# sair-lab/AirSLAM

Measured on AMD Instinct MI355X. Metric: stereo detect+match pairs/sec (2x PLNet @512x512 internal: points + lines, junctions on the left + LightGlue match), higher is better.
Workload: dtype fp16

## Files before the change

### airslam_amd/_lib.py

```python
from __future__ import annotations

import ctypes as C
import os

_HERE = os.path.dirname(os.path.abspath(__file__))
LIB_PATH = os.path.join(_HERE, "libairfe.so")


class Tuning(C.Structure):
    _fields_ = [(n, C.c_int) for n in (
        "fuse_lg_block", "gemm_small_max_m", "gemm8_min_m", "gemmr_min_m", "gemmr_wgs", "qkv_pair", "block_min_m", "lgb_tokens", "sg_kenc_gemm",
        "fold_qkv", "overlap_lines", "kf_graph", "kf_spec_rows", "fuse_dec", "assign_fused", "fold_out_proj", "desc_gather_stream", "copy_wgs")] + [("reserved", C.c_int * 5)]


class Cfg(C.Structure):
    _fields_ = [
        ("device", C.c_int), ("precision", C.c_int), ("max_batch", C.c_int), ("enc_chunk", C.c_int),
        ("max_keypoints", C.c_int), ("keypoint_threshold", C.c_float), ("remove_borders", C.c_int),
        ("nms_radius", C.c_int), ("line_threshold", C.c_float), ("line_length_threshold", C.c_float),
        ("matcher", C.c_int), ("image_width", C.c_int), ("image_height", C.c_int), ("sinkhorn_iters", C.c_int),
        ("superpoint_pack", C.c_char_p), ("plnet_s1_pack", C.c_char_p), ("lightglue_pack", C.c_char_p),
        ("superglue_pack", C.c_char_p), ("matcher_precision", C.c_int), ("line_precision", C.c_int), ("check_launches", C.c_int),
        ("tuning", C.POINTER(Tuning)),
    ]


class Stage0(C.Structure):
    _fields_ = [(n, C.c_void_p) for n in (
        "juncs_pred", "lines_pred", "iskeep", "idx_junc_to_end_min", "idx_junc_to_end_max",
        "loi_features", "loi_features_thin", "loi_features_aux")]


class BowdbFilter(C.Structure):
    _fields_ = [("ratio", C.c_float), ("min_words", C.c_int), ("d_max_index", C.c_void_p), ("d_exclude", C.c_void_p), ("exclude_words", C.c_int)]


class RelocCfg(C.Structure):
    _fields_ = [("ratio", C.c_float), ("min_words", C.c_int), ("K", C.c_int), ("outlier_rejection", C.c_int), ("min_inlier", C.c_int),
                ("pose_refinement", C.c_int), ("cam", C.c_double * 5), ("thr", C.c_double * 2)]


class LoopCfg(C.Structure):
    _fields_ = [("ratio", C.c_float), ("min_words", C.c_int), ("K", C.c_int), ("outlier_rejection", C.c_int), ("distance_rate", C.c_double),
                ("min_matches", C.c_int), ("min_points", C.c_int), ("min_inliers", C.c_int), ("cam", C.c_double * 5), ("thr", C.c_double * 2)]


class SeqPolicy(C.Structure):
    _fields_ = [("min_init_stereo_feature", C.c_int), ("min_num_match", C.c_int), ("max_num_match", C.c_int), ("tracking_point_rate", C.c_float),
                ("tracking_parallax_rate", C.c_float), ("min_x_diff", C.c_double), ("max_x_diff", C.c_double), ("max_y_diff", C.c_double),
                ("image_width", C.c_int), ("image_height", C.c_int)]


class SeqFrame(C.Structure):
    _fields_ = ([(n, C.c_int) for n in ("frame_type", "candidate", "promoted", "dropped", "enough_match", "good_stereo_point", "n_left", "n_right", "n_lines_left",
                                        "n_lines_right", "n_junctions", "n_stereo", "n_matches")] + [("_pad", C.c_int)]
                + [(n, C.c_void_p) for n in ("features_left", "features_right", "lines_left", "lines_right", "junctions", "stereo_idx", "stereo_score", "matches_idx",
                                             "matches_score")])


class DebugLinearArgs(C.Structure):
    _fields_ = ([(n, C.c_int) for n in ("prec", "M", "K", "K1", "N")] + [(n, C.c_void_p) for n in ("x1", "x2", "w", "b")]
                + [("epi", C.c_int), ("act", C.c_int), ("rowidx", C.c_void_p), ("src_rows", C.c_int), ("rot_cos", C.c_void_p), ("rot_sin", C.c_void_p),
                   ("Np", C.c_int), ("H", C.c_int), ("x32", C.c_void_p), ("d2s_hc", C.c_int), ("d2s_wc", C.c_int), ("flag", C.c_void_p),
                   ("kernel", C.c_int), ("gr_wgs", C.c_int), ("out", C.c_void_p), ("out2", C.c_void_p)])


class DebugLgBlockArgs(C.Structure):
    _fields_ = ([("prec", C.c_int), ("M", C.c_int)] + [(n, C.c_void_p) for n in ("attn", "x32", "xb", "wo", "bo", "w1", "b1", "gamma", "beta", "w2", "b2")]
                + [(n, C.c_int) for n in ("relu", "tokens_per_wg", "mixed", "nqk_n")]
                + [(n, C.c_void_p) for n in ("nqk_w", "nqk_b", "nv_w", "nv_b", "rot_cos", "rot_sin")]
                + [("Np", C.c_int)] + [(n, C.c_void_p) for n in ("q", "k", "vt")] + [("rows_past", C.c_int * 5)])


class DebugConvArgs(C.Structure):
    _fields_ = ([(n, C.c_void_p) for n in ("x", "img", "w1a", "b1a", "w", "b")] + [(n, C.c_int) for n in ("cin", "cout", "B", "H", "W", "pool", "out_pad", "relu", "wgs")]
                + [("y_words", C.c_size_t), ("y_raw", C.c_void_p)])


class DebugLgPrepareArgs(C.Structure):
    _fields_ = ([(n, C.c_int) for n in ("prec", "B", "cap", "ld", "kp_off", "normalize")] + [(n, C.c_float) for n in ("cx", "cy", "linv")]
                + [(n, C.c_void_p) for n in ("f0", "f1", "n0", "n1", "wr", "f0x", "f1x")] + [(n, C.c_int) for n in ("n0x", "n1x", "slack_rows", "rows")]
                + [(n, C.c_void_p) for n in ("x32", "xb", "rot_cos", "rot_sin", "lens")] + [("rows_past", C.c_int)])


class DebugLgAssignArgs(C.Structure):
    _fields_ = ([(n, C.c_int) for n in ("prec", "B", "n")] + [(n, C.c_void_p) for n in ("md", "x32", "w")] + [("b", C.c_float), ("lens", C.c_void_p), ("cap", C.c_int),
                ("thr", C.c_float), ("form", C.c_int)]
                + [(n, C.c_void_p) for n in ("pad", "z", "sim", "scores", "rowlse", "collse", "rowval", "rowarg", "colarg", "idx", "score", "nmatch")])


class DebugAttentionArgs(C.Structure):
    _fields_ = ([(n, C.c_int) for n in ("prec", "S", "H", "n", "cross")] + [(n, C.c_void_p) for n in ("q", "k", "v", "lens")]
                + [("canary", C.c_int), ("raw", C.c_int), ("out", C.c_void_p), ("Np", C.c_int), ("rows_past", C.c_int)])


class DebugDetectorTailArgs(C.Structure):
    _fields_ = ([(n, C.c_int) for n in ("B", "Bs", "h", "w", "cap")] + [(n, C.c_void_p) for n in ("heat", "act", "feat", "feat1", "n", "n1", "nms_map", "keep", "cand_cnt")]
                + [("nms_map_written", C.c_int)])


class DebugLinePostArgs(C.Structure):
    _fields_ = ([(n, C.c_int) for n in ("B", "nj", "ld", "h", "w", "capL", "capJ", "from_plane")]
                + [(n, C.c_void_p) for n in ("la", "sc", "m2", "heat", "lines", "nlines", "nfound", "junc", "njunc", "jfound", "jmap")])


class DebugJunctionTailArgs(C.Structure):
    _fields_ = ([(n, C.c_int) for n in ("B", "nj", "ld", "h", "w", "capL", "capJ")]
                + [(n, C.c_void_p) for n in ("la", "sc", "m2", "heat", "act", "lines", "nlines", "nfound", "junc", "njunc", "jfound")] + [("fused", C.c_int)])


class DebugLineMidArgs(C.Structure):
    _fields_ = ([(n, C.c_int) for n in ("B", "j2l", "s1_form", "wgs")]
                + [(n, C.c_void_p) for n in ("juncs_pred", "lines_pred", "thin", "aux", "loi", "iskeep_in", "idx_min_in", "idx_max_in", "iskeep", "idx_min", "idx_max", "counts",
                                             "keep", "pairs", "rep", "head4", "prop4", "ridx", "proj", "lines_adjusted", "scores_line", "table_dirty")])


class DebugS0DecodeArgs(C.Structure):
    _fields_ = ([(n, C.c_int) for n in ("B", "mode", "ld", "off", "want_ta8", "want_loi", "want_jnms", "prec", "wgs")] + [(n, C.c_void_p) for n in ("rows", "x", "w", "b")]
                + [("stage_floats", C.c_size_t)] + [(n, C.c_void_p) for n in ("stage", "jloc", "joff", "jnms", "ta8", "loi", "head_rows")])


SIGNATURES = {
    "airfe_copy_rows_dev": (C.c_int, [C.c_void_p, C.c_int, C.c_void_p, C.c_void_p, C.c_void_p, C.c_void_p, C.c_void_p, C.c_void_p]),
    "airfe_pack_rows_dev": (C.c_int, [C.c_void_p, C.c_int, C.c_void_p, C.c_void_p, C.c_void_p, C.c_void_p, C.c_void_p, C.c_void_p, C.c_void_p]),
    "airfe_seq_default_policy": (None, [C.POINTER(SeqPolicy)]),
    "airfe_seq_add_keyframe_check": (C.c_int, [C.POINTER(SeqPolicy), C.c_void_p, C.c_int, C.c_void_p, C.c_int, C.c_void_p, C.c_int]),
    "airfe_seq_good_stereo_points": (C.c_int, [C.POINTER(SeqPolicy), C.c_void_p, C.c_void_p, C.c_void_p, C.c_int]),
    "airfe_seq_create": (C.c_int, [C.c_void_p, C.c_void_p, C.c_int, C.POINTER(SeqPolicy), C.c_int, C.c_int, C.c_void_p, C.c_void_p, C.c_void_p, C.POINTER(C.c_void_p)]),
    "airfe_seq_destroy": (None, [C.c_void_p]),
    "airfe_seq_last_error": (C.c_char_p, [C.c_void_p]),
    "airfe_seq_begin": (C.c_int, [C.c_void_p, C.c_void_p, C.c_void_p, C.c_int, C.c_int, C.c_int, C.c_size_t]),
    "airfe_seq_end": (C.c_int, [C.c_void_p, C.POINTER(SeqFrame)]),
    "airfe_seq_step": (C.c_int, [C.c_void_p, C.c_void_p, C.c_void_p, C.c_int, C.c_int, C.c_int, C.c_size_t, C.POINTER(SeqFrame)]),
    "airfe_seq_stream": (C.c_void_p, [C.c_void_p]),
    "airfe_seq_set_outlier_rejection": (C.c_int, [C.c_void_p, C.c_int]),
    "airfe_seq_wall_split": (C.c_int, [C.c_void_p, C.POINTER(C.c_double), C.POINTER(C.c_double), C.POINTER(C.c_double), C.POINTER(C.c_int), C.POINTER(C.c_int)]),
    "airfe_default_cfg": (None, [C.POINTER(Cfg)]),
    "airfe_default_tuning": (None, [C.POINTER(Tuning)]),
    "airfe_debug_fail_next_launch": (C.c_int, [C.c_void_p, C.c_int]),
    "airfe_create": (C.c_int, [C.POINTER(Cfg), C.POINTER(C.c_void_p)]),
    "airfe_destroy": (None, [C.c_void_p]),
    "airfe_last_error": (C.c_char_p, [C.c_void_p]),
    "airfe_detect_points": (C.c_int, [C.c_void_p, C.c_void_p, C.c_int, C.c_int, C.c_int, C.c_void_p, C.c_int,
                                      C.POINTER(C.c_int)]),
    "airfe_has_line_branch": (C.c_int, [C.c_void_p]),
    "airfe_detect_plnet": (C.c_int, [C.c_void_p, C.c_void_p, C.c_int, C.c_int, C.c_int, C.POINTER(Stage0), C.c_void_p,
                                     C.c_int, C.POINTER(C.c_int), C.c_void_p, C.c_int, C.POINTER(C.c_int), C.c_void_p,
                                     C.c_int, C.POINTER(C.c_int), C.c_int]),
    "airfe_stereo_keyframe": (C.c_int, [C.c_void_p, C.c_void_p, C.c_void_p, C.c_int, C.c_int, C.c_int, C.c_void_p, C.c_void_p, C.c_int,
                                        C.POINTER(C.c_int), C.POINTER(C.c_int), C.c_void_p, C.c_void_p, C.c_int, C.POINTER(C.c_int),
                                        C.POINTER(C.c_int), C.c_void_p, C.c_int, C.POINTER(C.c_int), C.c_void_p, C.c_void_p, C.c_int,
                                        C.POINTER(C.c_int)]),
    "airfe_stereo_keyframe_tracked": (C.c_int, [C.c_void_p, C.c_void_p, C.c_void_p, C.c_int, C.c_int, C.c_int, C.c_void_p, C.c_void_p, C.c_int,
                                                C.POINTER(C.c_int), C.POINTER(C.c_int), C.c_void_p, C.c_void_p, C.c_int, C.POINTER(C.c_int),
                                                C.POINTER(C.c_int), C.c_void_p, C.c_int, C.POINTER(C.c_int), C.c_void_p, C.c_void_p, C.c_int,
                                                C.POINTER(C.c_int), C.c_void_p, C.c_int, C.c_void_p, C.c_void_p, C.POINTER(C.c_int)]),
    "airfe_track_frame": (C.c_int, [C.c_void_p, C.c_void_p, C.c_int, C.c_int, C.c_int, C.c_void_p, C.c_int, C.c_void_p, C.c_int, C.POINTER(C.c_int),
                                    C.c_void_p, C.c_void_p, C.c_int, C.POINTER(C.c_int)]),
    "airfe_promote_frame": (C.c_int, [C.c_void_p, C.c_void_p, C.c_int, C.c_int, C.c_int, C.c_void_p, C.c_int, C.POINTER(C.c_int), C.c_void_p, C.c_void_p, C.c_int,
# ... 60 lines not shown
    "airfe_bowdb_add_junction_frames_batch_dev": (C.c_int, [C.c_void_p, C.c_void_p, C.c_void_p, C.c_int, C.c_void_p, C.c_void_p] + [C.c_int] * 4 + [C.c_void_p]),
    "airfe_bowdb_query_stored_batch_dev": (C.c_int, [C.c_void_p, C.c_void_p, C.c_int, C.c_float, C.c_int, C.c_int] + [C.c_void_p] * 3 + [C.c_int] +
                                           [C.c_void_p] * 4),
    "airfe_loop_detect_batch_dev": (C.c_int, [C.c_void_p, C.c_void_p, C.POINTER(LoopCfg), C.c_void_p, C.c_int] + [C.c_void_p] * 10 + [C.c_int] +
                                    [C.c_void_p] * 3),
    "airfe_set_rectify_maps": (C.c_int, [C.c_void_p, C.c_int, C.c_void_p, C.c_void_p, C.c_int, C.c_int]),
    "airfe_rectify_detect_points": (C.c_int, [C.c_void_p, C.c_int, C.c_void_p, C.c_int, C.c_int, C.c_int, C.c_void_p, C.c_void_p, C.c_int,
                                              C.POINTER(C.c_int)]),
    "airfe_rectify_batch_dev": (C.c_int, [C.c_void_p, C.c_int, C.c_void_p, C.c_int, C.c_int, C.c_int, C.c_int, C.c_size_t, C.c_void_p,
                                          C.c_int, C.c_size_t, C.c_void_p]),
    "airfe_detect_points_batch_dev": (C.c_int, [C.c_void_p, C.c_void_p, C.c_int, C.c_int, C.c_int, C.c_int, C.c_size_t,
                                                C.c_void_p, C.c_int, C.c_void_p, C.c_void_p]),
    "airfe_match_lightglue_batch_dev": (C.c_int, [C.c_void_p, C.c_void_p, C.c_void_p, C.c_void_p, C.c_void_p, C.c_int,
                                                  C.c_int, C.c_void_p, C.c_void_p, C.c_int, C.c_void_p, C.c_void_p]),
    "airfe_match_superglue_batch_dev": (C.c_int, [C.c_void_p, C.c_void_p, C.c_void_p, C.c_void_p, C.c_void_p, C.c_int, C.c_int,
                                                  C.c_void_p, C.c_void_p, C.c_void_p, C.c_void_p, C.c_void_p]),
    "airfe_stereo_batch_dev": (C.c_int, [C.c_void_p, C.c_void_p, C.c_void_p, C.c_int, C.c_int, C.c_int, C.c_int,
                                         C.c_size_t, C.c_void_p, C.c_void_p, C.c_int, C.c_void_p, C.c_void_p, C.c_void_p,
                                         C.c_void_p, C.c_int, C.c_void_p, C.c_void_p]),
    "airfe_detect_plnet_batch_dev": (C.c_int, [C.c_void_p, C.c_void_p, C.c_int, C.c_int, C.c_int, C.c_int, C.c_size_t, C.c_void_p,
                                               C.c_int, C.c_void_p, C.c_void_p, C.c_int, C.c_void_p, C.c_void_p, C.c_int, C.c_void_p,
                                               C.c_int, C.c_void_p, C.c_void_p]),
    "airfe_stereo_plnet_batch_dev": (C.c_int, [C.c_void_p, C.c_void_p, C.c_void_p, C.c_int, C.c_int, C.c_int, C.c_int, C.c_size_t,
                                               C.c_void_p, C.c_void_p, C.c_int, C.c_void_p, C.c_void_p, C.c_void_p, C.c_int, C.c_void_p,
                                               C.c_void_p, C.c_int, C.c_void_p, C.c_void_p, C.c_void_p, C.c_void_p, C.c_int, C.c_void_p,
                                               C.c_void_p]),
    "airfe_debug_plnet_j2l": (C.c_int, [C.c_void_p, C.c_int, C.c_void_p, C.c_void_p, C.c_void_p]),
    "airfe_assign_points_to_lines_batch_dev": (C.c_int, [C.c_void_p, C.c_void_p, C.c_void_p, C.c_int, C.c_void_p, C.c_void_p, C.c_int, C.c_int,
                                                         C.c_void_p, C.c_void_p, C.c_void_p, C.c_int, C.c_void_p, C.c_void_p]),
    "airfe_match_lines_batch_dev": (C.c_int, [C.c_void_p] + [C.c_void_p] * 8 + [C.c_int, C.c_int, C.c_void_p, C.c_void_p, C.c_int, C.c_int,
                                              C.c_void_p, C.c_void_p, C.c_void_p, C.c_int, C.c_void_p, C.c_void_p]),
    "airfe_fundamental_ransac": (C.c_int, [C.c_void_p, C.c_void_p, C.c_int, C.c_void_p, C.c_int, C.c_void_p, C.c_void_p, C.c_int, C.POINTER(C.c_int)]),
    "airfe_fundamental_ransac_batch_dev": (C.c_int, [C.c_void_p, C.c_void_p, C.c_void_p, C.c_void_p, C.c_void_p, C.c_int, C.c_int, C.c_void_p, C.c_void_p,
                                                     C.c_int, C.c_void_p, C.c_void_p, C.c_void_p]),
    "airfe_set_outlier_rejection": (C.c_int, [C.c_void_p, C.c_int]),
    "airfe_pnp_ransac": (C.c_int, [C.c_void_p, C.c_void_p, C.c_void_p, C.c_int, C.c_void_p, C.c_void_p, C.c_void_p, C.c_void_p, C.POINTER(C.c_int)]),
    "airfe_pnp_ransac_batch_dev": (C.c_int, [C.c_void_p, C.c_void_p, C.c_void_p, C.c_void_p, C.c_int, C.c_int, C.c_void_p, C.c_void_p, C.c_void_p,
                                             C.c_void_p, C.c_void_p, C.c_void_p]),
    "airfe_stereo_points": (C.c_int, [C.c_void_p, C.c_void_p, C.c_void_p, C.c_int, C.c_void_p, C.c_int, C.c_void_p, C.c_int, C.c_void_p, C.c_void_p,
                                      C.c_void_p, C.POINTER(C.c_int)]),
    "airfe_stereo_points_batch_dev": (C.c_int, [C.c_void_p] * 6 + [C.c_int, C.c_int, C.c_void_p, C.c_void_p, C.c_int] + [C.c_void_p] * 5),
    "airfe_stereo_lines": (C.c_int, [C.c_void_p, C.c_void_p, C.c_void_p, C.c_int, C.c_void_p, C.c_int] + [C.c_void_p] * 8),
    "airfe_stereo_lines_batch_dev": (C.c_int, [C.c_void_p] * 6 + [C.c_int, C.c_void_p, C.c_void_p, C.c_int] + [C.c_void_p] * 7),
    "airfe_stereo_line_landmarks_batch_dev": (C.c_int, [C.c_void_p] * 6 + [C.c_int] + [C.c_void_p] * 4 + [C.c_int, C.c_void_p, C.c_void_p, C.c_int,
                                                        C.c_void_p, C.c_int] + [C.c_void_p] * 8 + [C.c_int] + [C.c_void_p] * 8),
    "airfe_track_pose_batch_dev": (C.c_int, [C.c_void_p, C.c_void_p, C.c_void_p, C.c_int, C.c_void_p, C.c_int, C.c_void_p, C.c_void_p, C.c_int, C.c_int,
                                             C.c_void_p, C.c_void_p, C.c_void_p, C.c_void_p, C.c_void_p]),
    "airfe_frame_optimize": (C.c_int, [C.c_void_p, C.c_void_p, C.c_void_p, C.c_int] + [C.c_void_p] * 7 + [C.POINTER(C.c_int)]),
    "airfe_frame_optimize_batch_dev": (C.c_int, [C.c_void_p, C.c_void_p, C.c_void_p, C.c_void_p, C.c_int, C.c_int] + [C.c_void_p] * 9),
    "airfe_track_pose_opt_batch_dev": (C.c_int, [C.c_void_p, C.c_void_p, C.c_void_p, C.c_int, C.c_void_p, C.c_int, C.c_void_p, C.c_int, C.c_void_p,
                                                 C.c_void_p, C.c_int, C.c_int] + [C.c_void_p] * 9),
    "airfe_sync": (C.c_int, [C.c_void_p]),
    "airfe_superglue_status": (C.c_int, [C.c_void_p, C.c_void_p]),
    "airfe_profile_enable": (C.c_int, [C.c_void_p, C.c_int]),
    "airfe_profile_stages": (C.c_int, []),
    "airfe_profile_stage_name": (C.c_char_p, [C.c_int]),
    "airfe_profile_read": (C.c_int, [C.c_void_p, C.c_void_p, C.c_void_p, C.c_void_p, C.c_void_p]),
    "airfe_debug_detector_maps": (C.c_int, [C.c_void_p, C.c_int, C.c_void_p, C.c_void_p, C.c_void_p]),
    "airfe_debug_lightglue_scores": (C.c_int, [C.c_void_p, C.c_void_p, C.c_int, C.c_void_p, C.c_int, C.c_void_p]),
    "airfe_debug_superglue_scores": (C.c_int, [C.c_void_p, C.c_void_p, C.c_int, C.c_void_p, C.c_int, C.c_void_p]),
    "airfe_debug_lg_filter": (C.c_int, [C.c_void_p, C.c_void_p, C.c_int, C.c_int, C.c_void_p, C.c_void_p, C.c_int, C.POINTER(C.c_int)]),
    "airfe_debug_sg_decode": (C.c_int, [C.c_void_p, C.c_void_p, C.c_int, C.c_int, C.c_void_p, C.c_void_p, C.c_void_p, C.c_void_p]),
    "airfe_debug_sg_sinkhorn": (C.c_int, [C.c_void_p, C.c_void_p, C.c_void_p, C.c_int, C.c_int, C.c_float, C.c_int, C.c_int, C.c_void_p, C.POINTER(C.c_int)]),
    "airfe_debug_detector_tail": (C.c_int, [C.c_void_p, C.POINTER(DebugDetectorTailArgs)]),
    "airfe_debug_line_post": (C.c_int, [C.c_void_p, C.POINTER(DebugLinePostArgs)]),
    "airfe_debug_junction_tail": (C.c_int, [C.c_void_p, C.POINTER(DebugJunctionTailArgs)]),
    "airfe_debug_junctions_topk": (C.c_int, [C.c_void_p, C.c_void_p, C.c_void_p, C.c_int, C.c_void_p]),
    "airfe_debug_line_mid": (C.c_int, [C.c_void_p, C.POINTER(DebugLineMidArgs)]),
    "airfe_debug_s0_decode": (C.c_int, [C.c_void_p, C.POINTER(DebugS0DecodeArgs)]),
    "airfe_debug_lg_prepare": (C.c_int, [C.c_void_p, C.POINTER(DebugLgPrepareArgs)]),
    "airfe_debug_lg_assign": (C.c_int, [C.c_void_p, C.POINTER(DebugLgAssignArgs)]),
    "airfe_debug_plnet_stage0": (C.c_int, [C.c_void_p] + [C.c_void_p] * 10),
    "airfe_debug_plnet_s1": (C.c_int, [C.c_void_p, C.POINTER(Stage0), C.c_void_p, C.c_void_p, C.c_int, C.POINTER(C.c_int)]),
    "airfe_debug_plnet_s1_last": (C.c_int, [C.c_void_p, C.c_void_p, C.c_void_p, C.c_int, C.POINTER(C.c_int)]),
    "airfe_debug_preprocess": (C.c_int, [C.c_void_p, C.c_void_p, C.c_int, C.c_int, C.c_int, C.c_void_p]),
    "airfe_debug_conv3x3": (C.c_int, [C.c_void_p, C.c_void_p, C.c_int, C.c_int, C.c_int, C.c_int, C.c_void_p, C.c_void_p,
                                      C.c_int, C.c_int, C.c_void_p]),
    "airfe_debug_conv": (C.c_int, [C.c_void_p, C.POINTER(DebugConvArgs)]),
    "airfe_debug_trace": (C.c_int, [C.c_void_p, C.c_int]),
    "airfe_debug_trace_stop": (C.c_int, [C.c_void_p, C.c_int]),
    "airfe_debug_trace_buffer": (C.c_int, [C.c_void_p, C.c_int, C.c_void_p, C.c_size_t]),
    "airfe_debug_trace_slots": (C.c_int, [C.c_void_p]),
    "airfe_debug_conv_order": (C.c_int, [C.c_int, C.POINTER(C.c_int)]),
    "airfe_debug_trace_slot": (C.c_int, [C.c_void_p, C.c_int, C.c_char_p, C.c_int, C.POINTER(C.c_uint), C.POINTER(C.c_uint), C.POINTER(C.c_uint)]),
    "airfe_debug_trace_read": (C.c_int, [C.c_void_p, C.c_void_p, C.c_void_p, C.c_void_p]),
    "airfe_debug_gemm": (C.c_int, [C.c_void_p, C.c_void_p, C.c_int, C.c_int, C.c_void_p, C.c_void_p, C.c_int, C.c_int,
                                   C.c_void_p]),
    "airfe_debug_linear": (C.c_int, [C.c_void_p, C.POINTER(DebugLinearArgs)]),
    "airfe_debug_qkv": (C.c_int, [C.c_void_p] + [C.c_int] * 3 + [C.c_void_p] * 3 + [C.c_int] + [C.c_void_p] * 4 + [C.c_int] * 2 + [C.c_void_p] * 3),
    "airfe_debug_lg_block": (C.c_int, [C.c_void_p, C.POINTER(DebugLgBlockArgs)]),
    "airfe_debug_ln_gelu": (C.c_int, [C.c_void_p, C.c_int, C.c_void_p, C.c_void_p, C.c_void_p, C.c_int]),
    "airfe_debug_attention_args": (C.c_int, [C.c_void_p, C.POINTER(DebugAttentionArgs)]),
    "airfe_debug_attention": (C.c_int, [C.c_void_p, C.c_void_p, C.c_void_p, C.c_void_p, C.c_void_p, C.c_int, C.c_int, C.c_int, C.c_int, C.c_void_p]),
}

_lib = None


def lib() -> C.CDLL:
    global _lib
    if _lib is None:
        if not os.path.exists(LIB_PATH):
            raise RuntimeError(
                f"{LIB_PATH} is missing: build it with `python -m airslam_amd.build` "
                "(hipcc, gfx950).  airslam_amd has no CPU fallback.")
        try:
            import torch
        except Exception:
            pass
        l = C.CDLL(LIB_PATH)
        for name, (res, args) in SIGNATURES.items():
            fn = getattr(l, name)
            fn.restype = res
            fn.argtypes = args
        _lib = l
    return _lib
```

### airslam_amd/api.py

```python
from __future__ import annotations

import ctypes as C
import os
import tempfile
from typing import Dict, Optional

import numpy as np

from . import _lib, weights as W

FEAT = 259


def _pack_arg(x, tmpfiles) -> Optional[bytes]:
    if x is None:
        return None
    if isinstance(x, (str, bytes, os.PathLike)):
        return os.fsencode(x)
    f = tempfile.NamedTemporaryFile(suffix=".airfe", delete=False)
    f.close()
    W.save_pack(f.name, x)
    tmpfiles.append(f.name)
    return f.name.encode()


class AirfeError(RuntimeError):
    pass


def conv_tile_order(order: int) -> int:
    prev = C.c_int()
    if _lib.lib().airfe_debug_conv_order(int(order), C.byref(prev)) != 0:
        raise AirfeError((_lib.lib().airfe_last_error(None) or b"airfe_debug_conv_order failed").decode())
    return prev.value


class Context:

    def __init__(self, superpoint=None, lightglue=None, superglue=None, plnet_s1=None, tuning=None, **cfg):
        self._l = _lib.lib()
        c = _lib.Cfg()
        self._l.airfe_default_cfg(C.byref(c))
        t = None
        if tuning and "conv_order" in tuning:
            tuning = dict(tuning)
            conv_tile_order(int(tuning.pop("conv_order")))
        if tuning:
            t = _lib.Tuning()
            self._l.airfe_default_tuning(C.byref(t))
            for k, v in tuning.items():
                if k == "reserved" or not hasattr(t, k):
                    raise TypeError(f"unknown airfe_tuning field {k!r}")
                setattr(t, k, int(v))
            c.tuning = C.pointer(t)
        for k, v in cfg.items():
            if not hasattr(c, k):
                raise TypeError(f"unknown airfe_cfg field {k!r}")
            setattr(c, k, v)
        tmp = []
        try:
            c.superpoint_pack = _pack_arg(superpoint, tmp)
            c.lightglue_pack = _pack_arg(lightglue, tmp)
            c.superglue_pack = _pack_arg(superglue, tmp)
            c.plnet_s1_pack = _pack_arg(plnet_s1, tmp)
            h = C.c_void_p()
            rc = self._l.airfe_create(C.byref(c), C.byref(h))
            if rc != 0:
                raise AirfeError((self._l.airfe_last_error(None) or b"airfe_create failed").decode())
        finally:
            for t in tmp:
                os.unlink(t)
        self._h = h
        c.tuning = None
        self.cfg = c
        self.max_keypoints = c.max_keypoints
        self.np_rows = (c.max_keypoints + 15) // 16 * 16

    def close(self):
        if getattr(self, "_h", None):
            self._l.airfe_destroy(self._h)
            self._h = None

    def __del__(self):
        try:
            self.close()
        except Exception:
            pass

    def _chk(self, rc, what):
        if rc != 0:
            raise AirfeError(f"{what}: {(self._l.airfe_last_error(self._h) or b'').decode()}")

    @staticmethod
    def _image(img, wrong_type=None):
        img = np.asarray(img)
        if img.ndim != 2 or img.dtype != np.uint8:
            raise wrong_type if wrong_type is not None else AirfeError("empty image")
        if img.size == 0:
            raise AirfeError("empty image")
        if img.strides[1] != 1 or img.strides[0] < img.shape[1]:
            img = np.ascontiguousarray(img)
        return img

    def detect_points(self, gray: np.ndarray) -> np.ndarray:
        gray = self._image(gray, TypeError("expected a 2-D uint8 image"))
        cap = self.np_rows
        feat = np.empty((cap, FEAT), dtype=np.float32)
        n = C.c_int(0)
        self._chk(self._l.airfe_detect_points(self._h, gray.ctypes.data, gray.shape[0], gray.shape[1], gray.strides[0],
                                              feat.ctypes.data, cap, C.byref(n)), "airfe_detect_points")
        return feat[:n.value].copy()

    def bow_load(self, voc: dict):
        d = np.ascontiguousarray(voc["desc"], np.float32); fc = np.ascontiguousarray(voc["first_child"], np.int32)
        nc = np.ascontiguousarray(voc["n_children"], np.int32); wi = np.ascontiguousarray(voc["word_id"], np.int32)
        w = np.ascontiguousarray(voc["weight"], np.float64)
        self._chk(self._l.airfe_bow_load(self._h, d.ctypes.data, fc.ctypes.data, nc.ctypes.data, wi.ctypes.data, w.ctypes.data, d.shape[0]),
                  "airfe_bow_load")

    def bow_transform(self, feat_rows: np.ndarray):
        f = np.ascontiguousarray(feat_rows, np.float32).reshape(-1, FEAT)
        wid = np.empty((f.shape[0],), np.uint32); w = np.empty((f.shape[0],), np.float64)
        self._chk(self._l.airfe_bow_transform(self._h, f.ctypes.data, f.shape[0], wid.ctypes.data, w.ctypes.data), "airfe_bow_transform")
        return wid, w

    def set_rectify_maps(self, side: int, mapx: np.ndarray, mapy: np.ndarray):
        mx = np.ascontiguousarray(mapx, np.float32); my = np.ascontiguousarray(mapy, np.float32)
        if mx.shape != my.shape or mx.ndim != 2:
            raise TypeError("maps must be two 2-D arrays of one shape")
# ... 355 lines not shown
        for name, x in zip(("iskeep_in", "idx_min_in", "idx_max_in"), ins):
            if x is not None:
                assert x.shape == (b, n)
                setattr(a, name, x.ctypes.data)
        self._chk(self._l.airfe_debug_line_mid(self._h, C.byref(a)), "airfe_debug_line_mid")
        return out

    S0_STAGE = {"lines_pred": (600, 3 * 16384 * 4), "thin": (600 + 7 * 3 * 16384, 4 * 16384), "aux": (600 + 7 * 3 * 16384 + 4 * 16384, 4 * 16384)}
    S0_STAGE_FLOATS = (600 + 7 * 3 * 16384 + 8 * 16384 + 63) // 64 * 64

    def debug_s0_decode(self, rows=None, ld=160, off=128, ta8=True, loi=False, jnms=True, x=None, w=None, b=None, prec=1, wgs=0, two_pass=False):
        f = lambda t: np.ascontiguousarray(t, np.float32)
        npx, sf = 128 * 128, self.S0_STAGE_FLOATS
        a = _lib.DebugS0DecodeArgs(want_ta8=int(bool(ta8)), want_loi=int(bool(loi)), want_jnms=int(bool(jnms)), prec=int(prec), wgs=int(wgs), stage_floats=sf)
        if rows is not None:
            assert x is None and not two_pass
            rows = f(rows)
            bb = rows.shape[0]
            assert rows.shape == (bb, npx, ld)
            a.mode, a.ld, a.off, a.rows = 0, int(ld), int(off), rows.ctypes.data
        else:
            x, w, b = f(x), f(w), f(b)
            bb = x.shape[0] // npx
            assert x.shape == (bb * npx, 128) and w.shape == (17, 128) and b.shape == (17,)
            a.mode, a.x, a.w, a.b = (2 if two_pass else 1), x.ctypes.data, w.ctypes.data, b.ctypes.data
        poison = lambda *shape: np.full(shape, -1, np.int32).view(np.float32)
        out = {"stage": poison(bb, sf), "jloc": poison(bb, 128, 128), "joff": poison(bb, 2, 128, 128), "jnms": poison(bb, 128, 128), "ta8": poison(bb, npx, 8),
               "loi": poison(128, 128, 128)}
        if two_pass:
            out["head_rows"] = poison(bb, npx, 32)
        a.B = bb
        for k, v in out.items():
            setattr(a, k, v.ctypes.data)
        self._chk(self._l.airfe_debug_s0_decode(self._h, C.byref(a)), "airfe_debug_s0_decode")
        for k, (o, n) in self.S0_STAGE.items():
            v = out["stage"][:, o:o + n]
            out[k] = v.reshape(bb, 3 * npx, 4) if k == "lines_pred" else v.reshape(bb, 4, 128, 128)
        return out

    def debug_junctions_topk(self, jloc, joff):
        jloc, joff = np.ascontiguousarray(jloc, np.float32), np.ascontiguousarray(joff, np.float32)
        b = jloc.shape[0]
        assert jloc.shape == (b, 128, 128) and joff.shape == (b, 2, 128, 128)
        out = np.full((b, 300, 2), np.nan, np.float32)
        self._chk(self._l.airfe_debug_junctions_topk(self._h, jloc.ctypes.data, joff.ctypes.data, b, out.ctypes.data), "airfe_debug_junctions_topk")
        return out

    def debug_preprocess(self, gray):
        gray = np.ascontiguousarray(gray, np.uint8)
        out = np.empty((512, 512), np.float32)
        self._chk(self._l.airfe_debug_preprocess(self._h, gray.ctypes.data, gray.shape[0], gray.shape[1], gray.strides[0],
                                                 out.ctypes.data), "airfe_debug_preprocess")
        return out

    def debug_conv3x3(self, x, w, b, pool=False):
        x = np.ascontiguousarray(x, np.float32); w = np.ascontiguousarray(w, np.float32); b = np.ascontiguousarray(b, np.float32)
        bb, cin, hh, ww = x.shape
        cout = w.shape[0]
        ho, wo = (hh // 2, ww // 2) if pool else (hh, ww)
        y = np.empty((bb, cout, ho, wo), np.float32)
        self._chk(self._l.airfe_debug_conv3x3(self._h, x.ctypes.data, bb, cin, hh, ww, w.ctypes.data, b.ctypes.data, cout,
                                              int(pool), y.ctypes.data), "airfe_debug_conv3x3")
        return y

    def debug_conv(self, w, b, prec, x=None, img=None, w1a=None, b1a=None, pool=False, out_pad=1, relu=True, wgs=256):
        f32 = lambda t: None if t is None else np.ascontiguousarray(t, np.float32)
        x, img, w1a, b1a, w, b = map(f32, (x, img, w1a, b1a, w, b))
        src = x if x is not None else img
        bb, hh, ww = src.shape[0], src.shape[-2], src.shape[-1]
        cout, cin = w.shape[0], w.shape[1]
        p = int(out_pad)
        ho, wo = (hh // 2, ww // 2) if pool else (hh, ww)
        guard = (wo + 2 * p) * cout
        words = bb * (ho + 2 * p) * guard
        raw = np.zeros(words + 2 * guard, np.uint16)
        ptr = lambda t: None if t is None else t.ctypes.data
        a = _lib.DebugConvArgs(x=ptr(x), img=ptr(img), w1a=ptr(w1a), b1a=ptr(b1a), w=ptr(w), b=ptr(b), cin=cin, cout=cout, B=bb, H=hh, W=ww, pool=int(pool), out_pad=p,
                               relu=int(relu), wgs=int(wgs), y_words=raw.size, y_raw=ptr(raw))
        self._chk(self._l.airfe_debug_conv(self._h, C.byref(a)), "airfe_debug_conv")
        buf = raw[guard:guard + words].reshape(bb, ho + 2 * p, wo + 2 * p, cout)
        inner = np.ascontiguousarray(buf[:, p:p + ho, p:p + wo, :])
        y = inner.view(np.float16).astype(np.float32) if prec == 1 else (inner.astype(np.uint32) << 16).view(np.float32)
        return {"raw": buf, "guard_lo": raw[:guard], "guard_hi": raw[guard + words:], "y": np.ascontiguousarray(y.transpose(0, 3, 1, 2))}

    def debug_gemm(self, x, w, b, relu=False):
        x = np.ascontiguousarray(x, np.float32); w = np.ascontiguousarray(w, np.float32); b = np.ascontiguousarray(b, np.float32)
        m, k = x.shape
        n = w.shape[0]
        y = np.empty((m, n), np.float32)
        self._chk(self._l.airfe_debug_gemm(self._h, x.ctypes.data, m, k, w.ctypes.data, b.ctypes.data, n, int(relu),
                                           y.ctypes.data), "airfe_debug_gemm")
        return y

    DEBUG_KERNELS = {"dispatch": 0, "small": 1, "tiled": 2, "gemm8": 3, "gemmr": 4, "gemmr_gather": 5, "gemmr_gather128": 6}

    def debug_linear(self, x1, w, b, prec, epi=0, act=0, x2=None, rowidx=None, rot=None, Np=0, x32=None, d2s=None, kernel="dispatch", gr_wgs=0):
        f32 = lambda t: None if t is None else np.ascontiguousarray(t, np.float32)
        x1, w, b, x2, x32 = f32(x1), f32(w), f32(b), f32(x2), (None if x32 is None else np.array(x32, np.float32, copy=True))
        n, k = w.shape
        m = len(rowidx) if rowidx is not None else x1.shape[0]
        a = _lib.DebugLinearArgs(prec=prec, M=m, K=k, K1=x1.shape[1], N=n, x1=x1.ctypes.data, w=w.ctypes.data, b=b.ctypes.data, epi=epi, act=act, Np=Np, H=4,
                                 kernel=self.DEBUG_KERNELS[kernel], gr_wgs=gr_wgs)
        keep = []
        if x2 is not None:
            a.x2 = x2.ctypes.data
        if rowidx is not None:
            ri = np.ascontiguousarray(rowidx, np.int32)
            keep.append(ri)
            a.rowidx, a.src_rows = ri.ctypes.data, x1.shape[0]
        if rot is not None:
            rc, rs = f32(rot[0]), f32(rot[1])
            keep += [rc, rs]
            a.rot_cos, a.rot_sin = rc.ctypes.data, rs.ctypes.data
        if x32 is not None:
            a.x32 = x32.ctypes.data
        flag = np.zeros(1, np.int32)
        out2 = None
        if epi == 5:
            hc, wc = d2s
            a.d2s_hc, a.d2s_wc, a.flag = hc, wc, flag.ctypes.data
            out = np.empty((m // (hc * wc), 8 * hc, 8 * wc), np.float32)
        elif epi in (3, 4):
            s = m // Np
            out = np.empty((s, 4, Np, 64) if epi == 3 else (s, 4, 64, Np), np.float32)
            if epi == 3 and n == 512:
                out2 = np.empty_like(out)
                a.out2 = out2.ctypes.data
        else:
            out = np.empty((m, n), np.float32)
        a.out = out.ctypes.data
        self._chk(self._l.airfe_debug_linear(self._h, C.byref(a)), "airfe_debug_linear")
        if epi == 5:
            return out, int(flag[0])
        if epi == 2:
            return out, x32
        return (out, out2) if out2 is not None else out

    def debug_qkv(self, x, wqk, bqk, wv, bv, prec, Np, rot=None, pair=True, gr_wgs=0):
        f32 = lambda t: np.ascontiguousarray(t, np.float32)
        x, wqk, bqk, wv, bv = f32(x), f32(wqk), f32(bqk), f32(wv), f32(bv)
        m, nqk, s = x.shape[0], wqk.shape[0], x.shape[0] // Np
        q = np.empty((s, 4, Np, 64), np.float32)
        k = np.empty_like(q) if nqk == 512 else None
        vt = np.empty((s, 4, 64, Np), np.float32)
        rc, rs = (f32(rot[0]), f32(rot[1])) if rot is not None else (None, None)
        ptr = lambda t: None if t is None else t.ctypes.data
        self._chk(self._l.airfe_debug_qkv(self._h, prec, m, Np, ptr(x), ptr(wqk), ptr(bqk), nqk, ptr(wv), ptr(bv), ptr(rc), ptr(rs), int(pair), gr_wgs, ptr(q),
                                          ptr(k), ptr(vt)), "airfe_debug_qkv")
        return q, k, vt

    def debug_lg_block(self, attn, x32, w1, b1, w2, b2, prec, gamma=None, beta=None, wo=None, bo=None, relu=False, tokens_per_wg=128, mixed=False,
                       nqk=None, nv=None, rot=None, Np=0):
        f32 = lambda t: None if t is None else np.ascontiguousarray(t, np.float32)
        m = attn.shape[0]
        attn, w1, b1, w2, b2, gamma, beta, wo, bo = map(f32, (attn, w1, b1, w2, b2, gamma, beta, wo, bo))
        x32 = np.array(x32, np.float32, copy=True)
        xb = np.empty_like(x32)
        ptr = lambda t: None if t is None else t.ctypes.data
        a = _lib.DebugLgBlockArgs(prec=prec, M=m, attn=ptr(attn), x32=ptr(x32), xb=ptr(xb), wo=ptr(wo), bo=ptr(bo), w1=ptr(w1), b1=ptr(b1), gamma=ptr(gamma),
                                  beta=ptr(beta), w2=ptr(w2), b2=ptr(b2), relu=int(relu), tokens_per_wg=tokens_per_wg, mixed=int(mixed), Np=Np)
        q = k = vt = None
        keep = []
        if nqk is not None:
            (qw, qb), (vw, vb) = map(lambda p: (f32(p[0]), f32(p[1])), (nqk, nv))
            keep += [qw, qb, vw, vb]
            s = m // Np
# ... 707 lines not shown
```

### airslam_amd/csrc/airfe_debug.hip

```cpp
#include "airfe_host.h"

#include <memory>

struct HookStage {
  enum { OWN_TEXT = 1, SATURATION = 2, DEVICE_WIDE = 4 };
  HookStage(airfe_ctx* c_, const std::string& who_, int pack_prec = 0) : c(c_), who(who_), st(c_->stream) { mem.pack_prec = pack_prec; }
  HookStage(const HookStage&) = delete;
  ~HookStage() {
    if (queued) (void)hipStreamSynchronize(st);
    for (void* p : mem.allocs) (void)hipFree(p);
  }
  int status() const { return rc; }
  hipStream_t stream() { queued = true; return st; }
  int refuse(const std::string& m) { return rc ? rc : rc = fail(c, who + ": " + m); }
  void step(int r) { queued = true; if (r) rc = 1; }
  template <class T> T* fresh(size_t n, int byte) {
    T* p = raw<T>(n);
    fill(p, byte, std::max<size_t>(n, 1) * sizeof(T));
    return p;
  }
  template <class T> T* up(std::vector<T> v) { T* p = raw<T>(v.size()); put(p, std::move(v)); return p; }
  template <class T> T* up(const T* src, size_t n) { return up(std::vector<T>(src, src + n)); }
  bool linear(const float* W, const float* b, int K, int N, LinW& out) { if (!rc && !make_linear(&mem, W, b, K, N, out)) refuse("allocation failed"); return !rc; }
  void fill(void* p, int byte, size_t bytes) { if (!rc && bytes) hip(hipMemsetAsync(p, byte, bytes, stream()), "hipMemsetAsync"); }
// ... 110 lines not shown
  s.wait();
  const std::vector<uint16_t> yo = s.get<uint16_t>(a.Y, ywords);
  for (int bb = 0; bb < B; ++bb)
    for (int co = 0; co < cout; ++co)
      for (int yy = 0; yy < Ho; ++yy)
        for (int xx = 0; xx < Wo; ++xx)
          y[(((size_t)bb * cout + co) * Ho + yy) * Wo + xx] = back2(yo[(((size_t)bb * (Ho + 2) + yy + 1) * (Wo + 2) + xx + 1) * cout + co], prec);
  return s.status();
} AIRFE_CATCH(c)

int airfe_debug_fail_next_launch(airfe_ctx* c, int stage) try {
  AIRFE_ENTER(c);
  if (stage < -1 || stage >= ST_COUNT) return fail(c, "debug_fail_next_launch: no such stage");
  c->fail_stage = stage;
  return 0;
} AIRFE_CATCH(c)

int airfe_debug_gemm(airfe_ctx* c, const float* x, int M, int K, const float* w, const float* b, int N, int relu, float* y) try {
  AIRFE_ENTER(c);
  if (K != 128 && K != 256 && K != 512) return fail(c, "debug_gemm: K must be 128, 256 or 512");
  const int prec = c->prec, Mp = (M + 127) / 128 * 128, Np8 = (N + 7) / 8 * 8;
  HookStage s(c, "debug_gemm", prec);
  LinW lw;
  s.linear(w, b, K, N, lw);
  GemmArgs g;
  g.X1 = s.up(dbg_rows2(x, M, K, Mp, prec)); g.ld1 = K; g.K1 = K; g.Wp = lw.w; g.bias = lw.b; g.M = Mp; g.N = N; g.cb_total = lw.cbt;
  g.epi = EPI_STORE_F32; g.act = relu ? ACT_RELU : ACT_NONE; g.out = s.fresh<float>((size_t)Mp * Np8, 0); g.ldo = Np8;
  dbg_gemm_dispatch(c, g, 0);
  if (s.status()) return 1;
  launch_gemm(prec, K, false, g, s.stream());
  s.wait(HookStage::OWN_TEXT);
  const std::vector<float> yo = s.get<float>(g.out, (size_t)Mp * Np8);
  for (int m = 0; m < M; ++m)
    for (int n = 0; n < N; ++n) y[(size_t)m * N + n] = yo[(size_t)m * Np8 + n];
  return s.status();
} AIRFE_CATCH(c)

int airfe_debug_conv(airfe_ctx* c, airfe_debug_conv_args* a) try {
  AIRFE_ENTER(c);
  if (!a || !a->w || !a->b || !a->y_raw) return fail(c, "debug_conv: null argument");
  const bool fused = a->img != nullptr;
  if (fused == (a->x != nullptr)) return fail(c, "debug_conv: exactly one of x (plain form) and img (fused conv1a -> conv1b) must be given");
  const int cin = a->cin, cout = a->cout, B = a->B, H = a->H, W = a->W, pool = a->pool, opad = a->out_pad, prec = c->prec;
  if (prec != 0 && prec != 1) return fail(c, "debug_conv: the context's precision must be fp16 or bf16");
  if (a->wgs < 1 || a->wgs > 256) return fail(c, "debug_conv: wgs must lie in 1 .. 256");
  if (cin != 64 && cin != 128) return fail(c, "debug_conv: cin must be 64 or 128");
  if (cout < 64 || cout % 64 || (cin == 128 && cout % 128)) return fail(c, "debug_conv: cout must be a multiple of 64 (of 128 when cin is 128)");
  if (B < 1 || H < 16 || W < 16 || H % 16 || W % 16) return fail(c, "debug_conv: B >= 1, H and W multiples of 16");
  if ((pool != 0 && pool != 1) || (opad != 0 && opad != 1) || (a->relu != 0 && a->relu != 1)) return fail(c, "debug_conv: pool, out_pad and relu are 0 or 1");
  if (pool && !opad) return fail(c, "debug_conv: a pooled layer always feeds another conv (out_pad = 1); pool with out_pad = 0 is no form of the arena");
  if (fused && (cin != 64 || cout != 64 || !pool || !opad || !a->relu || !a->w1a || !a->b1a))
    return fail(c, "debug_conv: the fused form is conv1a -> conv1b: cin = cout = 64, pool = 1, out_pad = 1, relu = 1, w1a and b1a given");
  const int Ho = pool ? H / 2 : H, Wo = pool ? W / 2 : W;
  const size_t guard = (size_t)(Wo + 2 * opad) * cout, words = (size_t)B * (Ho + 2 * opad) * guard, total = words + 2 * guard;
  if (a->y_words != total) return fail(c, "debug_conv: y_words must be (B (Ho + 2 out_pad) + 2) (Wo + 2 out_pad) cout");
  HookStage s(c, "debug_conv");
  ConvArgs g;
  if (fused) {
    std::vector<float> im((size_t)B * (H + 2) * (W + 2), 0.f);
    for (int bb = 0; bb < B; ++bb)
      for (int yy = 0; yy < H; ++yy) memcpy(&im[((size_t)bb * (H + 2) + yy + 1) * (W + 2) + 1], a->img + ((size_t)bb * H + yy) * W, (size_t)W * sizeof(float));
    g.img = s.up(std::move(im));
    g.w1a = s.up(a->w1a, (size_t)64 * 9);
    g.b1a = s.up(a->b1a, (size_t)64);
  } else {
    g.X = s.up(dbg_conv_x(a->x, B, cin, H, W, prec));
  }
  g.Wp = s.up(dbg_conv_slabs(a->w, cin, cout, prec));
  g.bias = s.up(a->b, (size_t)cout);
  uint16_t* dy = s.fresh<uint16_t>(total, 0xFF);
  if (s.status()) return 1;
  g.Y = dy + guard;
  g.B = B; g.H = H; g.W = W; g.CIN = cin; g.COUT = cout; g.pool = pool; g.out_pad = opad; g.relu = a->relu; g.wgs = a->wgs;
  if (fused) launch_conv64r(prec, g, s.stream());
  else launch_conv3x3(prec, g, s.stream());
  s.wait(HookStage::OWN_TEXT);
  s.get(a->y_raw, dy, total * 2);
  return s.status();
} AIRFE_CATCH(c)

int airfe_debug_conv_order(int order, int* previous) try {
  if (order < -1 || order > CONV_ORDER_DEFAULT) return fail(nullptr, "debug_conv_order: order must lie in -1 .. 3");
  const int before = conv_tile_order_switch(order);
  if (previous) *previous = before;
  return 0;
} AIRFE_CATCH(nullptr)

int airfe_debug_linear(airfe_ctx* c, const airfe_debug_linear_args* a) try {
  AIRFE_ENTER(c);
  if (!a || !a->x1 || !a->w || !a->b || !a->out) return fail(c, "debug_linear: null argument");
  const int prec = a->prec, M = a->M, K = a->K, N = a->N, epi = a->epi, kern = a->kernel, K1 = a->x2 ? a->K1 : K;
  if ((prec != 0 && prec != 1) || M < 1 || N < 1 || (K != 128 && K != 256 && K != 512) || K1 < 32 || K1 % 32 || K1 > K || (a->x2 && K1 == K) ||
      epi < EPI_STORE || epi > EPI_SOFTMAX_D2S || kern < AIRFE_DEBUG_KERNEL_DISPATCH || kern > AIRFE_DEBUG_KERNEL_GEMMR_GATHER128 || (a->act != ACT_NONE && a->act != ACT_RELU))
    return fail(c, "debug_linear: bad argument");
  const bool trans = epi == EPI_HEADS_T, heads = epi == EPI_HEADS || trans, d2s = epi == EPI_SOFTMAX_D2S;
  if (heads && ((a->H != 4 && a->H != 0) || a->Np < 16 || a->Np % 16 || M % a->Np || (epi == EPI_HEADS ? (N != 256 && N != 512) || (N == 512 && !a->out2) : N != 256)))
    return fail(c, "debug_linear: head layouts need H = 4, M = S * Np with Np a multiple of 16, N = 256 (or 512 with out2 for EPI_HEADS)");
  if ((a->rot_cos || a->rot_sin) && (epi != EPI_HEADS || !a->rot_cos || !a->rot_sin)) return fail(c, "debug_linear: rotary is an EPI_HEADS form");
  if (epi == EPI_RESID && (!a->x32 || N % 64)) return fail(c, "debug_linear: EPI_RESID needs x32 and N a multiple of 64");
  if (d2s && (K != 256 || N != 65 || a->x2 || a->rowidx || a->act || a->d2s_hc < 1 || a->d2s_wc < 1 || M % (a->d2s_hc * a->d2s_wc) || M % 16 ||
              (kern != AIRFE_DEBUG_KERNEL_DISPATCH && kern != AIRFE_DEBUG_KERNEL_GEMM8)))
    return fail(c, "debug_linear: EPI_SOFTMAX_D2S is launch_gemm8's head kernel: K = 256, N = 65, dense rows, M = B * hc * wc, M % 16 == 0");
  if (a->rowidx) {
    if (kern != AIRFE_DEBUG_KERNEL_GEMM8 && kern != AIRFE_DEBUG_KERNEL_GEMMR_GATHER && kern != AIRFE_DEBUG_KERNEL_GEMMR_GATHER128)
      return fail(c, "debug_linear: a row gather runs in gemm8, gemmr_gather or gemmr_gather128 only");
    if (a->src_rows < 1) return fail(c, "debug_linear: rowidx needs src_rows");
    for (int r = 0; r < M; ++r)
      if (a->rowidx[r] < 0 || a->rowidx[r] >= a->src_rows) return fail(c, "debug_linear: rowidx entry outside 0 .. src_rows - 1");
  }
  static const int row_tile[7] = {128, 32, 128, 256, 32, 32, 64};
  const int Mp = d2s ? M : (M + row_tile[kern] - 1) / row_tile[kern] * row_tile[kern];
  const int xrows = a->rowidx ? a->src_rows : Mp;
  const int ldo = (epi == EPI_STORE || epi == EPI_STORE_F32) ? (N + 7) / 8 * 8 : N;
  const int Sg = heads ? (Mp + a->Np - 1) / a->Np : 0, S = heads ? M / a->Np : 0;
  const bool f32 = epi == EPI_STORE_F32 || d2s, two = epi == EPI_HEADS && N == 512;
  const size_t out_elems = d2s ? (size_t)M * 64 : heads ? (size_t)Sg * 4 * a->Np * 64 : (size_t)Mp * ldo, out_bytes = out_elems * (f32 ? 4 : 2);
  HookStage s(c, "debug_linear", prec);
  LinW lw;
  s.linear(a->w, a->b, K, N, lw);
  GemmArgs g;
  g.X1 = s.up(dbg_rows2(a->x1, a->rowidx ? a->src_rows : M, K1, xrows, prec)); g.ld1 = K1; g.K1 = K1;
  if (a->x2) { g.X2 = s.up(dbg_rows2(a->x2, M, K - K1, Mp, prec)); g.ld2 = K - K1; }
  g.Wp = lw.w; g.bias = lw.b; g.M = Mp; g.N = N; g.cb_total = lw.cbt; g.epi = epi; g.act = a->act; g.ldo = ldo; g.Np = a->Np; g.H = 4;
  dbg_gemm_dispatch(c, g, a->gr_wgs);
  if (a->rot_cos) { g.rot_cos = s.up(dbg_rows4(a->rot_cos, M, 32, Mp)); g.rot_sin = s.up(dbg_rows4(a->rot_sin, M, 32, Mp)); }
  if (a->rowidx) { std::vector<int> ri(Mp, 0); memcpy(ri.data(), a->rowidx, (size_t)M * sizeof(int)); g.rowidx = s.up(std::move(ri)); }
  g.out = s.fresh<uint8_t>(out_bytes, 0xFF);
  if (two) g.out2 = s.fresh<uint8_t>(out_bytes, 0xFF);
  if (epi == EPI_RESID) g.x32 = s.up(dbg_rows4(a->x32, M, N, Mp));
  if (d2s) { g.d2s_hc = a->d2s_hc; g.d2s_wc = a->d2s_wc; g.flag = s.fresh<int>(1, 0); }
  if (s.status()) return 1;
  const char* refused = nullptr;
  hipStream_t st = s.stream();
  switch (kern) {
    case AIRFE_DEBUG_KERNEL_DISPATCH:
      if (d2s) launch_gemm8(prec, K, false, g, st);
      else launch_gemm(prec, K, trans, g, st);
      break;
    case AIRFE_DEBUG_KERNEL_SMALL:
      if (d2s || a->rowidx) refused = "gemm_small";
      else { g.small_max = 1 << 30; g.g8_min = 1 << 30; g.gr_min = 1 << 30; launch_gemm(prec, K, trans, g, st); }
      break;
    case AIRFE_DEBUG_KERNEL_TILED:
      if (d2s || a->rowidx || K1 % 64) refused = "gemm_kernel";
      else { g.small_max = -1; g.g8_min = 1 << 30; g.gr_min = 1 << 30; launch_gemm(prec, K, trans, g, st); }
      break;
    case AIRFE_DEBUG_KERNEL_GEMM8:
      if (K1 % 64) refused = "gemm8";
      else launch_gemm8(prec, K, trans, g, st);
      break;
    case AIRFE_DEBUG_KERNEL_GEMMR:
      if (a->rowidx || !gemmr_applicable(K, trans, g)) refused = "gemmr";
      else launch_gemmr(prec, trans, g, st);
      break;
    case AIRFE_DEBUG_KERNEL_GEMMR_GATHER:
      if (!gemmr_gather_applicable(K, g)) refused = "gemmr_gather";
      else launch_gemmr_gather(prec, g, st);
      break;
    default:
      if (!gemmr_gather128_applicable(g)) refused = "gemmr_gather128";
      else launch_gemmr_gather128(prec, g, st);
      break;
  }
  if (refused) return s.refuse(std::string(refused) + " does not apply to this form");
  s.wait(HookStage::OWN_TEXT);
  if (f32) {
// ... 825 lines not shown
```

### airslam_amd/csrc/airfe_detect.hip

```cpp
#include "airfe_host.h"

namespace airfe_host {

int ensure_tables(airfe_ctx* c, int h, int w) {
  if (c->tab_w == w && c->tab_h == h) return 0;
  const auto xt = resize_table(AIRFE_INTERNAL_SIZE, w), yt = resize_table(AIRFE_INTERNAL_SIZE, h);
  if (c->tab_w != -1) HIPCHK(c, hipDeviceSynchronize());
  HIPCHK(c, hipMemcpyAsync(c->xtab, xt.data(), xt.size() * 4, hipMemcpyHostToDevice, c->stream));
  HIPCHK(c, hipMemcpyAsync(c->ytab, yt.data(), yt.size() * 4, hipMemcpyHostToDevice, c->stream));
  HIPCHK(c, hipStreamSynchronize(c->stream));
  c->tab_w = w;
  c->tab_h = h;
  return 0;
}

int run_conv(airfe_ctx* c, const ConvW& w, const uint16_t* x, uint16_t* y, int B, int H, int W, int pool, int out_pad,
             hipStream_t st) {
  ConvArgs a;
  a.X = x; a.Wp = w.w; a.bias = w.b; a.Y = y;
  a.B = B; a.H = H; a.W = W; a.CIN = w.cin; a.COUT = w.cout;
  a.pool = pool; a.out_pad = out_pad; a.relu = 1;
  const double px = (double)B * H * W;
  const double ob = px / (pool ? 4 : 1) * w.cout * 2;
  {
    ProfScope ps(c, w.cin == 64 ? ST_CONV3X3_C64 : ST_CONV3X3_C128, st, 2.0 * px * w.cin * w.cout * 9,
                 px * w.cin * 2 + ob + 9.0 * w.cin * w.cout * 2);
    launch_conv3x3(c->prec, a, st);
  }
  return c->cfg.check_launches ? launch_status(c) : 0;
}

void f32_conv(const airfe_ctx::F32Conv& w, const float* x, float* y, int B, int H, int W, int opad, hipStream_t st) {
  launch_conv3x3_f32(x, w.w, w.b, y, B, H, W, w.cin, w.cout, opad, st);
}
int encode_f32(airfe_ctx* c, const uint8_t* d_gray, int B, int h, int w, int stride, size_t img_stride, hipStream_t st) {
  const int R = AIRFE_INTERNAL_SIZE;
  for (int c0 = 0; c0 < B; c0 += c->f_B) {
    const int cb = std::min(c->f_B, B - c0);
    launch_preprocess(d_gray + (size_t)c0 * img_stride, cb, h, w, stride, img_stride, c->xtab, c->ytab, c->lut, c->img32, R, R, st);
    launch_conv1a_f32(c->img32, c->c1a_w, c->c1a_b, c->f1a, cb, R, R, st);
    f32_conv(c->f_c1b, c->f1a, c->f1b, cb, R, R, 1, st);
    launch_maxpool2_f32(c->f1b, c->fp1, cb, R, R, 64, st);
    f32_conv(c->f_c2a, c->fp1, c->f2a, cb, R / 2, R / 2, 1, st);
    f32_conv(c->f_c2b, c->f2a, c->f2b, cb, R / 2, R / 2, 1, st);
    launch_maxpool2_f32(c->f2b, c->fp2, cb, R / 2, R / 2, 64, st);
    f32_conv(c->f_c3a, c->fp2, c->f3a, cb, R / 4, R / 4, 1, st);
    f32_conv(c->f_c3b, c->f3a, c->f3b, cb, R / 4, R / 4, 1, st);
    launch_maxpool2_f32(c->f3b, c->fp3, cb, R / 4, R / 4, 128, st);
    f32_conv(c->f_c4a, c->fp3, c->f4a, cb, R / 8, R / 8, 1, st);
    f32_conv(c->f_c4b, c->f4a, c->f4b, cb, R / 8, R / 8, 1, st);
    f32_conv(c->f_cPa, c->f4b, c->fPa, cb, R / 8, R / 8, 0, st);
    f32_conv(c->f_cDa, c->f4b, c->fDa, cb, R / 8, R / 8, 0, st);
    const int cells = cb * (R / 8) * (R / 8);
    const size_t cell0 = (size_t)c0 * (R / 8) * (R / 8);
    GemmF32Args g;
    g.X1 = c->fPa; g.ld1 = 256; g.K1 = 256; g.K = 256; g.W = c->f_cPb.w; g.bias = c->f_cPb.b; g.M = cells; g.N = 65;
    g.Y = c->logits + cell0 * 72; g.ldy = 72;
    launch_gemm_f32(g, st);
    g.X1 = c->fDa; g.W = c->f_cDb.w; g.bias = c->f_cDb.b; g.N = 256; g.Y = c->desc + cell0 * 256; g.ldy = 256;
    launch_gemm_f32(g, st);
  }
  launch_softmax_d2s(c->logits, 72, c->heat, B, R / 8, R / 8, st);
  c->desc_normalised = false;
  return launch_status(c);
}

int dense_desc_head(airfe_ctx* c, int B, hipStream_t st) {
  const int R = AIRFE_INTERNAL_SIZE, cells = B * (R / 8) * (R / 8);
  GemmArgs g;
  g.X1 = c->aDa; g.ld1 = 256; g.K1 = 256; g.Wp = c->cDb.w; g.bias = c->cDb.b;
  g.M = cells; g.N = 256; g.cb_total = c->cDb.cbt; g.epi = EPI_STORE_F32; g.out = c->desc; g.ldo = 256;
  g.small_max = c->gemm_small_max; g.g8_min = c->gemm8_min; g.gr_min = c->gemmr_min; g.gr_wgs = c->gemmr_wgs;
  {
    ProfScope ps(c, ST_HEAD_GEMM, st, 2.0 * cells * 256 * 256, (double)cells * (512 + 1024));
    if (c->desc_gather_stream && cells >= c->gemmr_min && gemmr_gather_applicable(256, g)) launch_gemmr_gather(c->prec, g, st);
    else launch_gemm(c->prec, 256, false, g, st);
  }
  c->desc_normalised = false;
  return c->cfg.check_launches ? launch_status(c) : 0;
}

int point_desc_head(airfe_ctx* c, int B, int cap, hipStream_t st, bool& sparse) {
  const int R = AIRFE_INTERNAL_SIZE;
  sparse = B > 2 && cap * 4 <= (R / 8) * (R / 8) && cap <= 1024;
  if (!sparse && dense_desc_head(c, B, st)) return 1;
  c->desc_dense_valid = !sparse;
  c->last_B = B;
  return 0;
}

int detect_tail_dev(airfe_ctx* c, int B, int Bs, bool two, bool sparse_desc, int h, int w, float* d_feat, float* d_feat1, int cap, int* d_n, int* d_n1,
                    hipStream_t st) {
  const int R = AIRFE_INTERNAL_SIZE;
  const int ccap = R * R;
  {
    ProfScope ps(c, ST_NMS, st, 0, (double)B * R * R * 8);
    if (c->cfg.nms_radius == 4) {
      c->nms_map_valid = B <= 2;
      launch_nms512_candidates(c->heat, c->nms_map_valid ? c->heat_nms : nullptr, c->nms_mask, B, c->cfg.keypoint_threshold,
                               c->cfg.remove_borders, c->cand, c->cand_cnt, ccap, st);
    } else if (c->cfg.nms_radius > 0) {
      c->nms_map_valid = true;
      launch_simple_nms(c->heat, c->heat_nms, c->nms_tmp, B, R, R, c->cfg.nms_radius, st);
      launch_candidates(c->heat_nms, B, R, R, c->cfg.keypoint_threshold, c->cfg.remove_borders, c->cand, c->cand_cnt, ccap, st);
    } else {
      launch_candidates(c->heat, B, R, R, c->cfg.keypoint_threshold, c->cfg.remove_borders, c->cand, c->cand_cnt, ccap, st);
    }
  }
  const int M = B * cap * 4, Mp = (M + 255) / 256 * 256;
  {
    ProfScope ps(c, ST_SELECT, st, 0, (double)B * 8192 * 8);
    SelectExtra ex;
    if (two) { ex.feat1 = d_feat1; ex.n_out1 = d_n1; ex.Bs = Bs; }
    if (sparse_desc) { ex.desc_idx = c->desc_idx; ex.HC = R / 8; ex.WC = R / 8; }
    launch_select_list(c->cand, c->cand_cnt, ccap, B, R, c->cfg.max_keypoints, cap, d_feat, d_n, st, &ex);
  }
  bool sampled = false;
  if (sparse_desc) {
    if (Mp > M) HIPCHK(c, hipMemsetAsync(c->desc_idx + M, 0, (size_t)(Mp - M) * 4, st));
    GemmArgs g;
    g.X1 = c->aDa; g.ld1 = 256; g.K1 = 256; g.Wp = c->cDb.w; g.bias = c->cDb.b; g.rowidx = c->desc_idx;
    g.M = Mp; g.N = 256; g.cb_total = c->cDb.cbt; g.epi = EPI_STORE_F32; g.out = c->desc; g.ldo = 256;
    g.gr_wgs = c->gemmr_wgs;
    const bool stream = c->desc_gather_stream && Mp >= c->gemmr_min && gemmr_gather_applicable(256, g);
    if (stream && gemmr_gather_sample_applicable(g)) {
      ProfScope ps(c, ST_HEAD_GEMM, st, 2.0 * Mp * 256 * 256, (double)Mp * 512 + (double)B * c->cfg.max_keypoints * 1036);
      DescSample ds;
      ds.feat = d_feat; ds.n = d_n; ds.feat1 = two ? d_feat1 : nullptr; ds.n1 = two ? d_n1 : nullptr; ds.Bs = two ? Bs : B; ds.B = B; ds.cap = cap;
      ds.HC = R / 8; ds.WC = R / 8; ds.w_scale = (float)w / (float)R; ds.h_scale = (float)h / (float)R; ds.flag = c->sat_flag;
      launch_gemmr_gather_sample(c->prec, g, ds, st);
      sampled = true;
    } else {
      ProfScope ps(c, ST_HEAD_GEMM, st, 2.0 * Mp * 256 * 256, (double)Mp * (512 + 1024));
      if (stream) launch_gemmr_gather(c->prec, g, st);
      else launch_gemm8(c->prec, 256, false, g, st);
    }
  }
  if (!sampled) {
    ProfScope ps(c, ST_SAMPLE, st, 0, (double)B * c->cfg.max_keypoints * (4096 + 1036));
    launch_sample_desc(c->desc, B, R / 8, R / 8, d_feat, d_n, cap, (float)w / (float)R, (float)h / (float)R,
                       sparse_desc ? 1 : (c->desc_normalised ? 0 : 1), st, sparse_desc ? 1 : 0, c->sat_flag, two ? d_feat1 : nullptr, two ? d_n1 : nullptr, Bs);
  }
  return launch_status(c);
}

int detect_dev2(airfe_ctx* c, const uint8_t* d_gray, const uint8_t* d_gray1, int Bs, int h, int w, int stride, size_t img_stride,
                float* d_feat, float* d_feat1, int cap, int* d_n, int* d_n1, hipStream_t st) {
  if (!c->has_sp) return fail(c, "detector weights were not loaded (cfg.superpoint_pack)");
  const int B = d_gray1 ? 2 * Bs : Bs;
  if (Bs < 1 || Bs > c->Bmax || B > c->Dmax) return fail(c, "batch exceeds cfg.max_batch");
  if (h < 1 || w < 1) return fail(c, "empty image");
  if (cap < c->cfg.max_keypoints) return fail(c, "feature capacity < max_keypoints");
  if (ensure_tables(c, h, w)) return 1;
  const int R = AIRFE_INTERNAL_SIZE;
  bool sparse_desc = false;
  if (c->prec == 2) {
    if (d_gray1) return fail(c, "detect_dev2: the fp32 path takes one source");
    if (encode_f32(c, d_gray, B, h, w, stride, img_stride, st)) return 1;
  } else {
    for (int c0 = 0, cb = 0; c0 < B; c0 += cb) {
      cb = std::min(c->chunk, B - c0);
      {
        ProfScope ps(c, ST_PREPROCESS, st, 0, (double)cb * ((double)h * w + (double)R * R * 4));
        const int n0 = std::min(std::max(Bs - c0, 0), cb);
        const uint8_t* s0 = n0 > 0 ? d_gray + (size_t)c0 * img_stride : nullptr;
        const uint8_t* s1 = cb > n0 ? d_gray1 + (size_t)(c0 + n0 - Bs) * img_stride : nullptr;
        launch_preprocess(s0 ? s0 : s1, cb, h, w, stride, img_stride, c->xtab, c->ytab, c->lut, c->img32, R, R, st, s0 ? s1 : nullptr, n0);
      }
      {
        ConvArgs a;
        a.Wp = c->c1b.w; a.bias = c->c1b.b; a.Y = c->a1b; a.B = cb; a.H = R; a.W = R; a.CIN = 64; a.COUT = 64;
        a.pool = 1; a.out_pad = 1; a.relu = 1;
        a.img = c->img32; a.w1a = c->c1a_w; a.b1a = c->c1a_b;
        const double px = (double)cb * R * R;
        ProfScope ps(c, ST_CONV1_FUSED, st, 2.0 * px * 9 * 64 + 2.0 * px * 64 * 64 * 9, px * 4 + px / 4 * 128 + 9.0 * 64 * 64 * 2);
        launch_conv64r(c->prec, a, st);
      }
      if (run_conv(c, c->c2a, c->a1b, c->a2a, cb, R / 2, R / 2, 0, 1, st)) return 1;
      if (run_conv(c, c->c2b, c->a2a, c->a2b + (size_t)c0 * (R / 4 + 2) * (R / 4 + 2) * 64, cb, R / 2, R / 2, 1, 1, st)) return 1;
    }
    if (run_conv(c, c->c3a, c->a2b, c->a3a, B, R / 4, R / 4, 0, 1, st)) return 1;
    if (run_conv(c, c->c3b, c->a3a, c->a3b, B, R / 4, R / 4, 1, 1, st)) return 1;
    if (run_conv(c, c->c4a, c->a3b, c->a4a, B, R / 8, R / 8, 0, 1, st)) return 1;
    if (run_conv(c, c->c4b, c->a4a, c->a4b, B, R / 8, R / 8, 0, 1, st)) return 1;
    if (run_conv(c, c->cPa, c->a4b, c->aPa, B, R / 8, R / 8, 0, 0, st)) return 1;
    if (run_conv(c, c->cDa, c->a4b, c->aDa, B, R / 8, R / 8, 0, 0, st)) return 1;
    const int cells = B * (R / 8) * (R / 8);
    {
      GemmArgs g;
      g.X1 = c->aPa; g.ld1 = 256; g.K1 = 256; g.Wp = c->cPb.w; g.bias = c->cPb.b;
      g.M = cells; g.N = 65; g.cb_total = c->cPb.cbt; g.epi = EPI_STORE_F32; g.out = c->logits; g.ldo = 72;
      g.small_max = c->gemm_small_max; g.g8_min = c->gemm8_min; g.gr_min = c->gemmr_min; g.gr_wgs = c->gemmr_wgs;
      g.epi = EPI_SOFTMAX_D2S; g.out = c->heat; g.d2s_hc = R / 8; g.d2s_wc = R / 8; g.flag = c->sat_flag;
      ProfScope ps(c, ST_HEAD_GEMM, st, 2.0 * cells * 256 * 65, (double)cells * (512 + 256));
      launch_gemm8(c->prec, 256, false, g, st);
    }
    if (point_desc_head(c, B, cap, st, sparse_desc)) return 1;
  }
  return detect_tail_dev(c, B, Bs, d_gray1 != nullptr, sparse_desc, h, w, d_feat, d_feat1, cap, d_n, d_n1, st);
}

int detect_dev(airfe_ctx* c, const uint8_t* d_gray, int B, int h, int w, int stride, size_t img_stride, float* d_feat,
               int cap, int* d_n, hipStream_t st) {
  return detect_dev2(c, d_gray, nullptr, B, h, w, stride, img_stride, d_feat, nullptr, cap, d_n, nullptr, st);
}

}
```

### airslam_amd/csrc/airfe_host.h

```cpp
#pragma once
#include "../../include/airfe.h"
#include "../../include/airfe_debug.h"

#include <hip/hip_runtime.h>

#include <algorithm>
#include <cmath>
#include <cstdio>
#include <cstdlib>
#include <cstring>
#include <functional>
#include <map>
#include <string>
#include <vector>

#include "kernels.h"
#include "common.h"

using namespace airfe;


namespace airfe_host {

extern thread_local std::string g_err;
// ... 235 lines not shown
  ST_PREPROCESS = 0, ST_CONV1_FUSED , ST_CONV3X3_C64, ST_CONV3X3_C128, ST_HEAD_GEMM, ST_HEAD_ELTWISE, ST_NMS, ST_SELECT,
  ST_SAMPLE, ST_LG_PREPARE, ST_LG_GEMM, ST_LG_ATTENTION, ST_LG_LNGELU, ST_LG_ASSIGN, ST_PL_DECODE, ST_PL_STAGE1, ST_PL_FILTER, ST_LINE_ASSOC, ST_RECTIFY, ST_BOW, ST_COUNT
};
static const char* kStageNames[ST_COUNT] = {
  "preprocess", "conv1_fused", "conv3x3_cin64", "conv3x3_cin128", "head_gemm", "head_eltwise", "simple_nms", "select_topk",
  "sample_desc", "lg_prepare", "lg_gemm", "lg_attention", "lg_ln_gelu", "lg_assign", "plnet_s0_decode", "plnet_stage1", "plnet_filter", "line_assoc", "rectify", "bow"};

void note_launch(airfe_ctx* c, int stage);
void fail_launch_now(hipStream_t st);
struct ProfScope {
  airfe_ctx* c; hipStream_t st; bool on; int stage; airfe_ctx::Mark m;
  ProfScope(airfe_ctx* c_, int stage_, hipStream_t st_, double flops, double bytes) : c(c_), st(st_), on((c_->prof_mask >> stage_) & 1u), stage(stage_) {
    if (c->fail_stage == stage) { c->fail_stage = -1; fail_launch_now(st); if (c->cfg.check_launches) note_launch(c, stage); }
    if (!on) return;
    auto get = [&]() {
      hipEvent_t e;
      if (!c->ev_pool.empty()) { e = c->ev_pool.back(); c->ev_pool.pop_back(); }
      else (void)hipEventCreate(&e);
      return e;
    };
    m.stage = stage; m.flops = flops; m.bytes = bytes; m.a = get(); m.b = get();
    (void)hipEventRecord(m.a, st);
  }
  ~ProfScope() {
    if (c->cfg.check_launches) note_launch(c, stage);
    if (!on) return;
    (void)hipEventRecord(m.b, st);
    try { c->marks.push_back(m); } catch (...) { c->ev_pool.clear(); }
  }
};

namespace airfe_host {

#define HIPCHK(ctx, expr)                                                                         \
  do {                                                                                            \
    hipError_t e_ = (expr);                                                                       \
    if (e_ != hipSuccess) {                                                                       \
      (ctx)->err = std::string(#expr) + ": " + hipGetErrorString(e_);                             \
      g_err = (ctx)->err;                                                                         \
      return 1;                                                                                   \
    }                                                                                             \
  } while (0)

int fail(airfe_ctx* c, const std::string& m);
int fail_noexcept(airfe_ctx* c, const char* what, const char* detail) noexcept;
int launch_status(airfe_ctx* c);
int saturation_status(airfe_ctx* c);

template <class T>
T* dalloc(DevAllocs* c, size_t n, bool zero = true) {
  void* p = nullptr;
  if (hipMalloc(&p, std::max<size_t>(n, 1) * sizeof(T)) != hipSuccess) return nullptr;
  if (zero) (void)hipMemset(p, 0, std::max<size_t>(n, 1) * sizeof(T));
  c->allocs.push_back(p);
  return reinterpret_cast<T*>(p);
}
template <class T>
T* dupload(DevAllocs* c, const std::vector<T>& v) {
  T* p = dalloc<T>(c, v.size(), false);
  if (p && !v.empty()) (void)hipMemcpy(p, v.data(), v.size() * sizeof(T), hipMemcpyHostToDevice);
  return p;
}

int load_superpoint(airfe_ctx* c, const char* path);
int load_lightglue(airfe_ctx* c, const char* path);
int load_superglue(airfe_ctx* c, const char* path);
int load_plnet_s1(airfe_ctx* c, const char* path);
std::vector<int> resize_table(int dsize, int ssize);
std::vector<uint16_t> pack_slabs(int cbt, int nslab, int prec, const std::function<float(int, int, int)>& get);
uint16_t f2bf(float f);
uint16_t f2h(float f);
float h2f(uint16_t h);
inline uint16_t cvt2(float f, int prec) { return prec == 1 ? f2h(f) : f2bf(f); }
inline float back2(uint16_t v, int prec) {
  if (prec == 1) return h2f(v);
  uint32_t u = (uint32_t)v << 16;
  float f;
  memcpy(&f, &u, 4);
  return f;
}
bool make_linear(DevAllocs* c, const float* W, const float* bias, int K, int N, LinW& out, float scale = 1.f,
                 const std::function<int(int)>* src_row = nullptr, const std::function<int(int)>* src_col = nullptr);
int ensure_tables(airfe_ctx* c, int h, int w);
int run_conv(airfe_ctx* c, const ConvW& w, const uint16_t* x, uint16_t* y, int B, int H, int W, int pool, int out_pad, hipStream_t st);
int dense_desc_head(airfe_ctx* c, int B, hipStream_t st);
int detect_tail_dev(airfe_ctx* c, int B, int Bs, bool two, bool sparse_desc, int h, int w, float* d_feat, float* d_feat1, int cap, int* d_n, int* d_n1,
                    hipStream_t st);
int detect_dev2(airfe_ctx* c, const uint8_t* d_gray, const uint8_t* d_gray1, int Bs, int h, int w, int stride, size_t img_stride,
                float* d_feat, float* d_feat1, int cap, int* d_n, int* d_n1, hipStream_t st);
int detect_dev(airfe_ctx* c, const uint8_t* d_gray, int B, int h, int w, int stride, size_t img_stride, float* d_feat, int cap, int* d_n, hipStream_t st);
int point_desc_head(airfe_ctx* c, int B, int cap, hipStream_t st, bool& sparse);
void junctions_topk_dev(airfe_ctx* c, int nb, hipStream_t st);
void line_head_gemm(airfe_ctx* c, int nb, bool fused, int prec, const LinW& hw, hipStream_t st);
void line_head_decode(airfe_ctx* c, int nb, int prec, const LinW& hw, float* jnms, int wgs, hipStream_t st);
void line_decode_rows(airfe_ctx* c, int nb, const float* head, int ld, int off, float* jnms, bool ta8, bool loi_chw, hipStream_t st);
void line_match(airfe_ctx* c, int nb, bool exact_all, hipStream_t st);
void line_dedup(airfe_ctx* c, int nb, hipStream_t st);
int line_tap_rows(airfe_ctx* c, int nb, hipStream_t st);
void line_loi_rows(airfe_ctx* c, int nb, hipStream_t st);
enum S1Form { S1_CHW = 0, S1_HEAD = 1, S1_ROWS = 2, S1_ROWS_H = 3, S1_HEAD_H = 4 };
void line_stage1(airfe_ctx* c, int nb, int form, int wgs, hipStream_t st);
void junction_maps_clear(airfe_ctx* c, int nj, hipStream_t st);
void line_filter_maps(airfe_ctx* c, int nb, int nj, int h, int w, double* d_lines, int capL, int* d_nlines, int* d_lfound, hipStream_t st);
int junction_scan_maps(airfe_ctx* c, int i0, int nj, float* d_junc, int capJ, int* d_njunc, int* d_jfound, hipStream_t st);
int junction_desc_sample(airfe_ctx* c, int i0, int nj, int h, int w, float* d_junc, int capJ, const int* d_njunc, hipStream_t st);
int junction_dense_maps(airfe_ctx* c, int nj, int capJ, int phase, hipStream_t st, bool& partial);
int line_branch_dev(airfe_ctx* c, hipStream_t st, int i0, int nb, bool chw);
int line_tail_dev(airfe_ctx* c, int i0, int nb, bool host_s0, int h, int w, double* d_lines, int capL, int* d_nlines, int* d_lfound,
                  float* d_junc, int capJ, int* d_njunc, int* d_jfound, int nj, hipStream_t st, int phase = 3);
bool junction_tail_fused(airfe_ctx* c, int nj, int capJ);
int line_post_dev(airfe_ctx* c, int i0, int nb, int h, int w, double* d_lines, int capL, int* d_nlines, int* d_lfound, float* d_junc, int capJ, int* d_njunc,
                  int* d_jfound, int nj, hipStream_t st, int phase, bool fused);
void trace(airfe_ctx* c, hipStream_t st, const char* what, size_t li, const char* blk, const void* p, size_t words, unsigned unit_words);
int trace_finish(airfe_ctx* c, hipStream_t st);
int run_linear(airfe_ctx* c, const LinW& w, const uint16_t* x1, int ld1, int K1, const uint16_t* x2, int ld2, int M, int epi, int act, void* out,
                int ldo, hipStream_t st, bool trans = false, void* out2 = nullptr, float* x32 = nullptr, const float* rc = nullptr, const float* rs = nullptr);
void reset_slack_rows(airfe_ctx* c, int M, hipStream_t st);
struct LgSecondPair { const float *f0, *f1; const int *n0, *n1; };
int lightglue_dev(airfe_ctx* c, const float* f0, const int* n0, const float* f1, const int* n1, int B, int cap, int ld, int kp_off, int normalize,
                  int32_t* d_idx, float* d_score, int mcap, int* d_nmatch, float* scores_out, hipStream_t st, const LgSecondPair* x2 = nullptr);
int superglue_dev(airfe_ctx* c, const float* f0, const int* n0, const float* f1, const int* n1, int B, int cap, int normalize, hipStream_t st);
int sinkhorn_failed(airfe_ctx* c);

}

#define AIRFE_CATCH(c)                                                                                                   \
  catch (const std::exception& e_) { return airfe_host::fail_noexcept((c), __func__, e_.what()); }                       \
  catch (...) { return airfe_host::fail_noexcept((c), __func__, nullptr); }
inline int enter_device(airfe_ctx* c) {
  int d = -1;
  if (hipGetDevice(&d) == hipSuccess && d == c->cfg.device) return 0;
  if (hipSetDevice(c->cfg.device) != hipSuccess) return fail(c, "hipSetDevice(cfg.device) failed");
  return 0;
}
#define AIRFE_ENTER(c) do { if (!(c)) return 1; if (enter_device(c)) return 1; } while (0)
int ensure_pin(airfe_ctx* c, size_t bytes);
int upload_image(airfe_ctx* c, const uint8_t* gray, int h, int w, int stride);
inline void clear_saturation(airfe_ctx* c) {
  if (c->sat_host) c->sat_host[0] = c->sat_host[1] = 0;
}
struct DrainOnError {
  airfe_ctx* c; bool armed = false, ref_uploaded = false;
  explicit DrainOnError(airfe_ctx* c_, bool armed_ = false) : c(c_), armed(armed_) { clear_saturation(c_); }
  ~DrainOnError() {
    if (!armed) return;
    (void)hipStreamSynchronize(c->stream);
    (void)hipStreamSynchronize(c->stream2);
    if (ref_uploaded) c->ref_n = -1;
  }
};
inline int rows_out(const airfe_ctx* c, int img, float* feat) {
  const int Np = c->cfg.max_keypoints, n = std::min(reinterpret_cast<const int*>(c->pin)[img], Np);
  if (n > 0) memcpy(feat, c->pin + 64 + (size_t)img * Np * AIRFE_FEAT_DIM * 4, (size_t)n * AIRFE_FEAT_DIM * 4);
  return n;
}
inline void matches_out(const airfe_ctx* c, size_t off, size_t stride, int first, int nm, int32_t* idx, float* score) {
  if (nm < 1) return;
  memcpy(idx, c->pin + off + (size_t)first * 8, (size_t)nm * 8);
  memcpy(score, c->pin + off + stride + (size_t)first * 4, (size_t)nm * 4);
}
int upload_reference(airfe_ctx* c, DrainOnError& drain, size_t off, const float* ref_feat, int n_ref, hipStream_t st);
int rows_home(airfe_ctx* c, const DevBlock& blk, size_t bytes, hipStream_t s2);
struct RowsPart { const void* dev; void* host; size_t bytes; };
int rows_second_trip(airfe_ctx* c, std::initializer_list<RowsPart> parts, hipStream_t st);
int upload_stage0(airfe_ctx* c, const airfe_plnet_stage0* s0, hipStream_t st);
int fransac_queue(airfe_ctx* c, const float* d_f0, const float* d_f1, int B, int cap, int32_t* d_idx, float* d_score, int mcap, int* d_nmatch, double* d_F,
                  hipStream_t st);
// ... 8 lines not shown
```

### airslam_amd/csrc/airfe_lines.hip

```cpp
#include "airfe_host.h"

namespace airfe_host {

void junctions_topk_dev(airfe_ctx* c, int nb, hipStream_t st) {
  const int F = 128, ccap = F * F;
  launch_candidates_nms3(c->l_jloc, nb, F, F, 1e-30f, c->l_cand, c->l_cand_cnt, ccap, st);
  SelectExtra jx;
  jx.sort_all = 1;
  launch_select_list(c->l_cand, c->l_cand_cnt, ccap, nb, F, 300, 320, c->l_sel, c->l_nsel, st, &jx);
  launch_s0_juncs(c->l_sel, c->l_nsel, c->l_joff, c->s0_stage + SG_JUNCS, 300, 320, nb, SG_STRIDE, st);
}


void line_head_gemm(airfe_ctx* c, int nb, bool fused, int prec, const LinW& hw, hipStream_t st) {
  const int F = 128;
  GemmArgs g;
  g.X1 = c->l_feat; g.ld1 = 128; g.K1 = 128; g.Wp = hw.w; g.bias = hw.b;
  g.M = nb * F * F; g.N = hw.N; g.cb_total = hw.cbt; g.epi = EPI_STORE_F32; g.out = fused ? c->l_head : c->l_dec; g.ldo = fused ? 160 : 32;
  g.small_max = c->gemm_small_max; g.g8_min = c->gemm8_min; g.gr_min = c->gemmr_min; g.gr_wgs = c->gemmr_wgs;
  if (!fused) g.small_max = 1 << 30;
  ProfScope ps(c, ST_HEAD_GEMM, st, 2.0 * nb * F * F * 128 * hw.N, (double)nb * F * F * (256 + 4.0 * g.ldo));
  launch_gemm(prec, 128, false, g, st);
}

void line_head_decode(airfe_ctx* c, int nb, int prec, const LinW& hw, float* jnms, int wgs, hipStream_t st) {
  const int F = 128;
  ProfScope ps(c, ST_PL_DECODE, st, 2.0 * nb * F * F * 128 * 17, (double)nb * F * F * (256 + 92));
  launch_s0_head_decode(prec, c->l_feat, hw.w, hw.b, c->s0_stage + SG_LP, c->l_jloc, jnms, c->l_joff, c->l_ta8, nb, SG_STRIDE, st, wgs);
}

void line_decode_rows(airfe_ctx* c, int nb, const float* head, int ld, int off, float* jnms, bool ta8, bool loi_chw, hipStream_t st) {
  float* d = c->s0_stage;
  launch_s0_decode(head, ld, off, d + SG_LP, c->l_jloc, jnms, c->l_joff, d + SG_THIN, d + SG_AUX, loi_chw ? c->s0_loi : nullptr, ta8 ? c->l_ta8 : nullptr, nb,
                   SG_STRIDE, st);
}

void line_match(airfe_ctx* c, int nb, bool exact_all, hipStream_t st) {
  float* d = c->s0_stage;
  c->wf_counted = launch_s0_j2l(d + SG_LP, d + SG_JUNCS, 300, KEEP_CAP, 10.0f, d + SG_KEEP, d + SG_MIN, d + SG_MAX, c->wf_counts, nb, SG_STRIDE, exact_all ? 1 : 0, st);
}

void line_dedup(airfe_ctx* c, int nb, hipStream_t st) {
  float* d = c->s0_stage;
  launch_wireframe(d + SG_KEEP, d + SG_MIN, d + SG_MAX, KEEP_CAP, 300, c->wf_table, c->wf_keep, c->wf_pairs, c->wf_rep, KEEP_CAP, LINE_CAP,
                   c->wf_counts, c->wf_counted, d + SG_JUNCS, d + SG_LP, c->s1_la, c->wf_prop, nb, SG_STRIDE, st);
  c->wf_counted = false;
}

int line_tap_rows(airfe_ctx* c, int nb, hipStream_t st) {
  const int M = nb * 1200, Mp = (M + 255) / 256 * 256;
  launch_s1_junc_rows(c->s0_stage + SG_JUNCS, 300, c->l_ridx, nb, SG_STRIDE, st);
  if (Mp > M) HIPCHK(c, hipMemsetAsync(c->l_ridx + M, 0, (size_t)(Mp - M) * 4, st));
  return 0;
}

void line_loi_rows(airfe_ctx* c, int nb, hipStream_t st) {
  const int M = nb * 1200, Mp = (M + 255) / 256 * 256;
  GemmArgs g;
  g.X1 = c->l_feat; g.ld1 = 128; g.K1 = 128; g.Wp = c->cLh_loi.w; g.bias = c->cLh_loi.b; g.rowidx = c->l_ridx;
  g.M = Mp; g.N = 128; g.cb_total = c->cLh_loi.cbt; g.epi = EPI_STORE_F32; g.out = c->l_lrows; g.ldo = 128;
  g.gr_wgs = c->gemmr_wgs;
  if (c->desc_gather_stream && Mp >= c->gemmr_min && c->prec != 2 && gemmr_gather128_applicable(g)) launch_gemmr_gather128(c->prec, g, st);
  else launch_gemm8(c->prec, 128, false, g, st);
}

void line_stage1(airfe_ctx* c, int nb, int form, int wgs, hipStream_t st) {
  float* d = c->s0_stage;
  const bool chw = form == S1_CHW, rows = form == S1_ROWS || form == S1_ROWS_H, pairs = form == S1_ROWS_H || form == S1_HEAD_H;
  if (form == S1_ROWS_H) launch_s1h_junc_proj(d + SG_JUNCS, c->l_lrows, 300, c->s1_wsplit[4], c->s1_wsplit[5], c->s1_jfeat, nb, SG_STRIDE, st);
  else if (!chw)
    launch_s1_junc_proj(d + SG_JUNCS, rows ? nullptr : c->l_head, rows ? 0 : (size_t)128 * 128 * 160, rows ? 0 : 160, rows ? c->l_lrows : nullptr, 300, c->s1_w[0],
                        c->s1_jfeat, nb, SG_STRIDE, st);
  if (pairs)
    launch_plnet_s1h(c->wf_pairs, c->wf_counts, c->s1_jfeat, c->l_ta8, c->s1_wsplit, c->s1_w, c->s1_la, c->wf_prop, c->s1_sc, LINE_CAP, nb, st, wgs);
  else
    launch_plnet_s1(d + SG_JUNCS, d + SG_LP, c->wf_keep, c->wf_pairs, c->wf_rep, c->wf_counts, chw ? c->s0_loi : nullptr, 0, chw ? nullptr : c->s1_jfeat,
                    chw ? nullptr : c->l_ta8, d + SG_THIN, d + SG_AUX, c->s1_w, c->s1_la, c->s1_sc, KEEP_CAP, LINE_CAP, nb, SG_STRIDE, st, wgs);
}

int line_branch_dev(airfe_ctx* c, hipStream_t st, int i0, int nb, bool chw) {
  if (!c->has_s0) return fail(c, "the detector pack carries no line branch (line.* tensors)");
  if (!c->s0_stage) return fail(c, "the line path arena is not allocated (cfg.plnet_s1_pack)");
  if (nb < 1 || nb > c->Lmax || i0 < 0 || i0 + nb > c->Dmax) return fail(c, "line branch: image range outside the arena");
  const int F = 128;
  const bool fused = c->prec == 2 || chw;
  if (fused && (nb != 1 || i0 != 0)) return fail(c, "the fused line head (fp32 mode, inspection hook) runs one image at a time");
  c->line_sparse = !fused;
  bool head_done = false;
  if (c->prec == 2) {
    launch_conv3x3_f32(c->f3a, c->f_cL1.w, c->f_cL1.b, c->fL1, 1, F, F, 128, 128, 0, st);
    GemmF32Args g;
    g.X1 = c->fL1; g.ld1 = 128; g.K1 = 128; g.K = 128; g.W = c->f_cLh.w; g.bias = c->f_cLh.b; g.M = F * F; g.N = 145; g.Y = c->l_head; g.ldy = 160;
    launch_gemm_f32(g, st);
  } else {
    if (run_conv(c, c->cL1, c->a3a + (size_t)i0 * (F + 2) * (F + 2) * 128, c->l_feat, nb, F, F, 0, 0, st)) return 1;
    head_done = !fused && c->fuse_dec;
    if (head_done) line_head_decode(c, nb, c->prec, c->cLh_dec, nullptr, 0, st);
    else line_head_gemm(c, nb, fused, c->prec, fused ? c->cLh : c->cLh_dec, st);
  }
  {
    ProfScope ps(c, ST_PL_DECODE, st, 0, (double)nb * (128.0 * 128 * (17 * 4 + 3 * 16 + 11 * 4) + 3.0 * 49152 * (16 + 12)));
    if (!head_done) line_decode_rows(c, nb, fused ? c->l_head : c->l_dec, fused ? 160 : 32, fused ? 128 : 0, nullptr, true, chw, st);
    junctions_topk_dev(c, nb, st);
    line_match(c, nb, chw, st);
  }
  return launch_status(c);
}

static void junction_gemm_args(airfe_ctx* c, int i0, int nj, float* d_junc, int capJ, const int* d_njunc, int h, int w, GemmArgs& g, DescSample& ds) {
  const int R = AIRFE_INTERNAL_SIZE;
  g.X1 = c->aDa + (size_t)i0 * (R / 8) * (R / 8) * 256; g.ld1 = 256; g.K1 = 256; g.Wp = c->cDb.w; g.bias = c->cDb.b;
  g.M = (capJ + 7) / 8 * nj * 32; g.N = 256; g.cb_total = c->cDb.cbt; g.epi = EPI_STORE_F32; g.out = c->desc; g.ldo = 256;
  g.gr_wgs = c->gemmr_wgs;
  ds.feat = d_junc; ds.n = d_njunc; ds.Bs = nj; ds.B = nj; ds.cap = capJ; ds.HC = R / 8; ds.WC = R / 8;
  ds.w_scale = (float)w / (float)R; ds.h_scale = (float)h / (float)R; ds.flag = nullptr;
  ds.junc = 1;
}
bool junction_tail_fused(airfe_ctx* c, int nj, int capJ) {
  if (nj < 1 || capJ < 1 || c->prec == 2 || c->cfg.nms_radius != 4 || c->nms_map_valid || c->desc_dense_valid || !c->desc_gather_stream) return false;
  GemmArgs g;
  DescSample ds;
  junction_gemm_args(c, 0, nj, nullptr, capJ, nullptr, 1, 1, g, ds);
  return g.M >= c->gemmr_min && gemmr_gather_sample_junc_applicable(g, ds);
}

int line_tail_dev(airfe_ctx* c, int i0, int nb, bool host_s0, int h, int w, double* d_lines, int capL, int* d_nlines, int* d_lfound,
                  float* d_junc, int capJ, int* d_njunc, int* d_jfound, int nj, hipStream_t st, int phase) {
  if (!c->has_s1) return fail(c, "PLNet stage-1 weights were not loaded (cfg.plnet_s1_pack)");
  if (nb < 1 || nb > c->Lmax || nj < 0 || nj > nb) return fail(c, "line path: image range outside the arena");
  const bool fused = phase == 3 && junction_tail_fused(c, nj, capJ);
  if (phase & 1) {
    if (!fused) junction_maps_clear(c, nj, st);
    ProfScope ps(c, ST_PL_STAGE1, st, 0, (double)nb * 49152 * 12);
    line_dedup(c, nb, st);
    const int form = host_s0 ? S1_CHW : c->cfg.line_precision == 3 ? (c->line_sparse ? S1_ROWS_H : S1_HEAD_H) : (c->line_sparse ? S1_ROWS : S1_HEAD);
// ... 82 lines not shown
```

### airslam_amd/csrc/airfe_load.hip

```cpp
#include "airfe_host.h"

namespace airfe_host {

bool load_pack(const char* path, Pack& out, std::string& err) {
  FILE* f = fopen(path, "rb");
  if (!f) { err = std::string("cannot open weight pack ") + path; return false; }
  fseek(f, 0, SEEK_END);
  const long fsize = ftell(f);
  fseek(f, 0, SEEK_SET);
  char magic[8];
  uint32_t count = 0;
  bool ok = fread(magic, 1, 8, f) == 8 && memcmp(magic, "AIRFEPK1", 8) == 0 && fread(&count, 4, 1, f) == 1;
  for (uint32_t i = 0; ok && i < count; ++i) {
    uint32_t nl = 0, nd = 0;
    ok = fread(&nl, 4, 1, f) == 1 && nl < 4096;
    if (!ok) break;
    std::string name(nl, '\0');
    ok = fread(&name[0], 1, nl, f) == nl && fread(&nd, 4, 1, f) == 1 && nd <= 8;
    if (!ok) break;
    Tensor t;
    size_t n = 1;
    for (uint32_t d = 0; d < nd; ++d) {
      uint32_t v = 0;
      ok = ok && fread(&v, 4, 1, f) == 1;
// ... 10 lines not shown
  fclose(f);
  if (!ok) err = std::string("malformed weight pack ") + path;
  return ok;
}

uint16_t f2bf(float f) {
  uint32_t u;
  memcpy(&u, &f, 4);
  if ((u & 0x7F800000u) == 0x7F800000u) return (uint16_t)(u >> 16);
  u += 0x7FFFu + ((u >> 16) & 1u);
  return (uint16_t)(u >> 16);
}
uint16_t f2h(float f) {
  uint32_t x;
  memcpy(&x, &f, 4);
  const uint32_t sign = (x >> 16) & 0x8000u;
  int32_t e = (int32_t)((x >> 23) & 0xFF) - 127 + 15;
  uint32_t m = x & 0x7FFFFFu;
  if (((x >> 23) & 0xFF) == 0xFF) return (uint16_t)(sign | 0x7C00u | (m ? 0x200u : 0));
  if (e >= 31) return (uint16_t)(sign | 0x7C00u);
  if (e <= 0) {
    if (e < -10) return (uint16_t)sign;
    m |= 0x800000u;
    const int shift = 14 - e;
    uint32_t r = m >> shift;
    const uint32_t rem = m & ((1u << shift) - 1u), half = 1u << (shift - 1);
    if (rem > half || (rem == half && (r & 1u))) ++r;
    return (uint16_t)(sign | r);
  }
  uint32_t r = ((uint32_t)e << 10) | (m >> 13);
  const uint32_t rem = m & 0x1FFFu;
  if (rem > 0x1000u || (rem == 0x1000u && (r & 1u))) ++r;
  return (uint16_t)(sign | r);
}
float h2f(uint16_t h) {
  const uint32_t s = (uint32_t)(h & 0x8000u) << 16;
  int e = (h >> 10) & 31;
  uint32_t m = h & 0x3FFu;
  uint32_t u;
  if (e == 0) {
    if (!m) u = s;
    else {
      e = 1;
      while (!(m & 0x400u)) { m <<= 1; --e; }
      m &= 0x3FFu;
      u = s | ((uint32_t)(e + 112) << 23) | (m << 13);
    }
  } else if (e == 31) u = s | 0x7F800000u | (m << 13);
  else u = s | ((uint32_t)(e + 112) << 23) | (m << 13);
  float f;
  memcpy(&f, &u, 4);
  return f;
}

std::vector<uint16_t> pack_slabs(int cbt, int nslab, int prec, const std::function<float(int, int, int)>& get) {
  std::vector<uint16_t> out((size_t)cbt * nslab * 4096, 0);
  for (int cb = 0; cb < cbt; ++cb)
    for (int s = 0; s < nslab; ++s) {
      uint16_t* slab = out.data() + ((size_t)cb * nslab + s) * 4096;
      for (int rr = 0; rr < 64; ++rr) {
        const int feat = cb * 64 + slab_row_to_feature(rr);
        for (int k = 0; k < 64; ++k) {
          const int byte = rr * 128 + ((((k >> 3) ^ ((rr >> 1) & 7))) << 4) + (k & 7) * 2;
          slab[byte >> 1] = cvt2(get(feat, s, k), prec);
        }
      }
    }
  return out;
}

const Tensor* need(const Pack& p, const std::string& name, std::string& err) {
  auto it = p.find(name);
  if (it == p.end()) { err = "weight pack is missing tensor " + name; return nullptr; }
  return &it->second;
}
static bool need_linear(const Pack& p, const std::string& name, int K, int N, const Tensor*& w, const Tensor*& b, std::string& err) {
  w = need(p, name + ".weight", err);
  b = need(p, name + ".bias", err);
  if (!w || !b) return false;
  if ((int)w->data.size() != N * K || (int)b->data.size() != N) { err = name + ": unexpected shape"; return false; }
  return true;
}

bool make_conv(airfe_ctx* c, const Pack& p, const std::string& name, int cin, int cout, ConvW& out, std::string& err) {
  const Tensor* w = need(p, name + ".weight", err);
  const Tensor* b = need(p, name + ".bias", err);
  if (!w || !b) return false;
  if ((int)w->data.size() != cout * cin * 9 || (int)b->data.size() != cout) { err = name + ": unexpected shape"; return false; }
  const int nci = cin / 64;
  const float* wd = w->data.data();
  auto slabs = pack_slabs(cout / 64, 9 * nci, c->prec, [&](int feat, int s, int k) {
    const int tap = s / nci, cc = s % nci, ci = cc * 64 + k;
    return wd[((size_t)feat * cin + ci) * 9 + tap];
  });
  out.w = dupload(c, slabs);
  out.b = dupload(c, b->data);
  out.cin = cin;
  out.cout = cout;
  return out.w && out.b;
}

bool make_linear(DevAllocs* c, const float* W, const float* bias, int K, int N, LinW& out, float scale,
                 const std::function<int(int)>* src_row, const std::function<int(int)>* src_col) {
  const int Kp = (K + 63) / 64 * 64, cbt = (N + 63) / 64;
  const int cbp = (cbt + 3) & ~3;
  auto slabs = pack_slabs(cbp, Kp / 64, c->pack_prec, [&](int feat, int s, int k) {
    const int kk = s * 64 + k;
    if (feat >= N || kk >= K) return 0.f;
    const int r = src_row ? (*src_row)(feat) : feat;
    const int cc = src_col ? (*src_col)(kk) : kk;
    return W[(size_t)r * K + cc] * scale;
  });
  std::vector<float> bp((size_t)cbp * 64, 0.f);
  for (int f = 0; f < N; ++f) bp[f] = bias[src_row ? (*src_row)(f) : f] * scale;
  out.w = dupload(c, slabs);
  out.b = dupload(c, bp);
  out.K = Kp;
  out.N = N;
  out.cbt = cbt;
  {
    const int NS = Kp / 64;
    std::vector<uint16_t> fr(slabs.size());
    for (int T = 0; T < cbp * 4; ++T)
      for (int sl = 0; sl < NS; ++sl) {
        const uint16_t* slab = slabs.data() + ((size_t)(T >> 2) * NS + sl) * (SLAB_BYTES / 2);
        for (int h = 0; h < 2; ++h)
          for (int lane = 0; lane < 64; ++lane) {
            const int l15 = lane & 15, g = lane >> 4, rr = (T & 3) * 16 + l15;
            const int byte = rr * 128 + (((h * 4 + g) ^ ((rr >> 1) & 7)) << 4);
            uint16_t* dst = fr.data() + (((size_t)T * NS + sl) * 2 + h) * 512 + (size_t)lane * 8;
            for (int e = 0; e < 8; ++e) dst[e] = slab[(byte >> 1) + e];
          }
      }
    out.wf = dupload(c, fr);
  }
  return out.w && out.b && out.wf;
}

bool make_linear_named(airfe_ctx* c, const Pack& p, const std::string& name, int K, int N, LinW& out, std::string& err,
                       float scale = 1.f) {
  const Tensor *w, *b;
  return need_linear(p, name, K, N, w, b, err) && make_linear(c, w->data.data(), b->data.data(), K, N, out, scale);
}

bool make_ffn0_folded(airfe_ctx* c, const Tensor& w1, const Tensor& b1, const Tensor& wo, const Tensor& bo, LinW& out, std::string& err,
                      const std::function<int(int)>* wo_col = nullptr) {
  if (w1.data.size() != 512 * 512 || b1.data.size() != 512 || wo.data.size() != 256 * 256 || bo.data.size() != 256) { err = "fold_out_proj: unexpected shape"; return false; }
  std::vector<float> W((size_t)512 * 512), B(512);
  std::vector<double> row(256);
  for (int n = 0; n < 512; ++n) {
    const float* w1n = &w1.data[(size_t)n * 512];
    memcpy(&W[(size_t)n * 512], w1n, 256 * sizeof(float));
    std::fill(row.begin(), row.end(), 0.0);
    double bacc = b1.data[n];
    for (int j = 0; j < 256; ++j) {
      const double m = w1n[256 + j];
      bacc += m * bo.data[j];
      const float* woj = &wo.data[(size_t)j * 256];
      for (int k = 0; k < 256; ++k) row[k] += m * woj[k];
    }
    for (int k = 0; k < 256; ++k) W[(size_t)n * 512 + 256 + k] = (float)row[wo_col ? (*wo_col)(k) : k];
    B[n] = (float)bacc;
  }
  return make_linear(c, W.data(), B.data(), 512, 512, out, 1.f);
}

static const std::function<int(int)> hm = [](int f) { return (f & 63) * 4 + (f >> 6); };
static const std::function<int(int)> qkv_row = [](int f) { const int sel = f >> 8, hd = f & 255; return (hd >> 6) * 192 + (hd & 63) * 3 + sel; };
static const std::function<int(int)> v_row = [](int f) { return qkv_row(512 + f); };
struct BlockNames { std::string out, f0, f3, ln; };
static BlockNames lg_names(int i, const char* half, const char* out) {
  const std::string a = "transformers." + std::to_string(i) + half;
  return {a + out, a + ".ffn.0", a + ".ffn.3", a + ".ffn.1"};
}
static BlockNames sg_names(const std::string& g) { return {g + ".attn.merge", g + ".mlp.0", g + ".mlp.3", ""}; }

static bool load_block_tail(airfe_ctx* c, const Pack& p, const BlockNames& n, const std::function<int(int)>* wo_col, AttnBlock& b, std::string& err) {
  const Tensor *wo, *bo;
  bool ok = need_linear(p, n.out, 256, 256, wo, bo, err) && make_linear(c, wo->data.data(), bo->data.data(), 256, 256, b.out, 1.f, nullptr, wo_col);
  if (c->fold_out) {
    const Tensor *w1 = need(p, n.f0 + ".weight", err), *b1 = need(p, n.f0 + ".bias", err);
    ok = ok && w1 && b1 && make_ffn0_folded(c, *w1, *b1, *wo, *bo, b.ffn0, err, wo_col);
// ... 71 lines not shown
            f32_conv(c, p, "conv2b", 64, 64, c->f_c2b, err) && f32_conv(c, p, "conv3a", 64, 128, c->f_c3a, err) &&
            f32_conv(c, p, "conv3b", 128, 128, c->f_c3b, err) && f32_conv(c, p, "conv4a", 128, 128, c->f_c4a, err) &&
            f32_conv(c, p, "conv4b", 128, 128, c->f_c4b, err) && f32_conv(c, p, "convPa", 128, 256, c->f_cPa, err) &&
            f32_conv(c, p, "convDa", 128, 256, c->f_cDa, err) && f32_lin_named(c, p, "convPb", 256, 65, c->f_cPb, err) &&
            f32_lin_named(c, p, "convDb", 256, 256, c->f_cDb, err);
  if (ok && p.count("line.conv1.weight"))
    ok = f32_conv(c, p, "line.conv1", 128, 128, c->f_cL1, err) && f32_lin_named(c, p, "line.head", 128, 145, c->f_cLh, err);
  if (!ok) return fail(c, err.empty() ? "device allocation failed while loading fp32 detector weights" : err);
  const int R = AIRFE_INTERNAL_SIZE;
  const size_t FB = c->f_B = std::min(c->Bmax, 2);
  auto sq = [](size_t n) { return n * n; };
  c->f1a = dalloc<float>(c, FB * sq(R + 2) * 64); c->f1b = dalloc<float>(c, FB * sq(R + 2) * 64);
  c->fp1 = dalloc<float>(c, FB * sq(R / 2 + 2) * 64); c->f2a = dalloc<float>(c, FB * sq(R / 2 + 2) * 64); c->f2b = dalloc<float>(c, FB * sq(R / 2 + 2) * 64);
  c->fp2 = dalloc<float>(c, FB * sq(R / 4 + 2) * 64); c->f3a = dalloc<float>(c, FB * sq(R / 4 + 2) * 128); c->f3b = dalloc<float>(c, FB * sq(R / 4 + 2) * 128);
  c->fp3 = dalloc<float>(c, FB * sq(R / 8 + 2) * 128); c->f4a = dalloc<float>(c, FB * sq(R / 8 + 2) * 128); c->f4b = dalloc<float>(c, FB * sq(R / 8 + 2) * 128);
  c->fPa = dalloc<float>(c, FB * sq(R / 8) * 256); c->fDa = dalloc<float>(c, FB * sq(R / 8) * 256);
  c->fL1 = dalloc<float>(c, sq(R / 4) * 128);
  if (!c->f1a || !c->f1b || !c->fp1 || !c->f2a || !c->f2b || !c->fp2 || !c->f3a || !c->f3b || !c->fp3 || !c->f4a || !c->f4b || !c->fPa ||
      !c->fDa || !c->fL1)
    return fail(c, "device allocation failed (fp32 detector arena)");
  return 0;
}

int alloc_matcher_arena_f32(airfe_ctx* c);

int load_lightglue_f32(airfe_ctx* c, const Pack& p, int L) {
  std::string err;
  c->f_lg.resize(L);
  bool ok = true;
  for (int i = 0; i < L && ok; ++i) {
    auto& l = c->f_lg[i];
    const std::string s = "transformers." + std::to_string(i) + ".self_attn", x = "transformers." + std::to_string(i) + ".cross_attn";
    ok = f32_lin_named(c, p, s + ".Wqkv", 256, 768, l.self.qk, err, &qkv_row) && f32_block_tail(c, p, lg_names(i, ".self_attn", ".out_proj"), nullptr, l.self, err) &&
         f32_lin_named(c, p, x + ".to_qk", 256, 256, l.cross.qk, err) && f32_lin_named(c, p, x + ".to_v", 256, 256, l.cross.v, err) &&
         f32_block_tail(c, p, lg_names(i, ".cross_attn", ".to_out"), nullptr, l.cross, err);
  }
  ok = ok && f32_lin_named(c, p, "log_assignment." + std::to_string(L - 1) + ".final_proj", 256, 256, c->f_lgfinal, err);
  if (!ok) return fail(c, err.empty() ? "device allocation failed while loading fp32 LightGlue weights" : err);
  return alloc_matcher_arena_f32(c);
}

int alloc_matcher_arena_f32(airfe_ctx* c) {
  if (c->m_qkv) return 0;
  const size_t M = (size_t)(2 * c->Pmax + 2 + 128 / c->Np) * c->Np + 256;
  c->m_qkv = dalloc<float>(c, M * 768); c->m_ctx = dalloc<float>(c, M * 256); c->m_msg = dalloc<float>(c, M * 256);
  c->m_h = dalloc<float>(c, M * 512); c->m_md = dalloc<float>(c, M * 256);
  if (!c->m_qkv || !c->m_ctx || !c->m_msg || !c->m_h || !c->m_md) return fail(c, "device allocation failed (fp32 matcher arena)");
  return 0;
}

int load_superglue_f32(airfe_ctx* c, const Pack& p, int L) {
  std::string err;
  c->f_sg.resize(L);
  bool ok = true;
  for (int i = 0; i < L && ok; ++i) {
    auto& l = c->f_sg[i];
    const std::string g = "gnn.layers." + std::to_string(i);
    std::vector<float> wqkv((size_t)768 * 256), bqkv(768);
    for (int j = 0; j < 3 && ok; ++j) {
      const Tensor *w, *b;
      ok = need_linear(p, g + ".attn.proj." + std::to_string(j), 256, 256, w, b, err);
      for (int f = 0; ok && f < 256; ++f) {
        memcpy(&wqkv[((size_t)j * 256 + f) * 256], &w->data[(size_t)hm(f) * 256], 1024);
        bqkv[j * 256 + f] = b->data[hm(f)];
      }
    }
    ok = ok && f32_lin(c, wqkv.data(), bqkv.data(), 256, 768, l.qk) && f32_block_tail(c, p, sg_names(g), &hm, l, err);
  }
  ok = ok && f32_lin_named(c, p, "final_proj", 256, 256, c->f_sgfinal, err);
  if (!ok) return fail(c, err.empty() ? "SuperGlue (fp32): unexpected shapes or device allocation failed" : err);
  return alloc_matcher_arena_f32(c);
}

int load_superpoint(airfe_ctx* c, const char* path) {
  c->pack_prec = c->prec == 2 ? 1 : c->prec;
  Pack p;
  std::string err;
  if (!load_pack(path, p, err)) return fail(c, err);
  const Tensor* w1 = need(p, "conv1a.weight", err);
  const Tensor* b1 = need(p, "conv1a.bias", err);
  if (!w1 || !b1 || w1->data.size() != 64 * 9) return fail(c, err.empty() ? "conv1a: unexpected shape" : err);
  c->c1a_w = dupload(c, w1->data);
  c->c1a_b = dupload(c, b1->data);
  bool ok = make_conv(c, p, "conv1b", 64, 64, c->c1b, err) && make_conv(c, p, "conv2a", 64, 64, c->c2a, err) &&
            make_conv(c, p, "conv2b", 64, 64, c->c2b, err) && make_conv(c, p, "conv3a", 64, 128, c->c3a, err) &&
            make_conv(c, p, "conv3b", 128, 128, c->c3b, err) && make_conv(c, p, "conv4a", 128, 128, c->c4a, err) &&
            make_conv(c, p, "conv4b", 128, 128, c->c4b, err) && make_conv(c, p, "convPa", 128, 256, c->cPa, err) &&
            make_conv(c, p, "convDa", 128, 256, c->cDa, err) &&
            make_linear_named(c, p, "convPb", 256, 65, c->cPb, err) && make_linear_named(c, p, "convDb", 256, 256, c->cDb, err);
  if (!ok) return fail(c, err.empty() ? "device allocation failed while packing SuperPoint weights" : err);

  const int B = c->Dmax, ch = c->chunk, R = AIRFE_INTERNAL_SIZE;
  c->img32 = dalloc<float>(c, (size_t)ch * (R + 2) * (R + 2));
  c->a1b = dalloc<uint16_t>(c, (size_t)ch * (R / 2 + 2) * (R / 2 + 2) * 64);
  c->a2a = dalloc<uint16_t>(c, (size_t)ch * (R / 2 + 2) * (R / 2 + 2) * 64);
  c->a2b = dalloc<uint16_t>(c, (size_t)B * (R / 4 + 2) * (R / 4 + 2) * 64);
  c->a3a = dalloc<uint16_t>(c, (size_t)B * (R / 4 + 2) * (R / 4 + 2) * 128);
  c->a3b = dalloc<uint16_t>(c, (size_t)B * (R / 8 + 2) * (R / 8 + 2) * 128);
  c->a4a = dalloc<uint16_t>(c, (size_t)B * (R / 8 + 2) * (R / 8 + 2) * 128);
  c->a4b = dalloc<uint16_t>(c, (size_t)B * (R / 8 + 2) * (R / 8 + 2) * 128);
  const size_t cells = (size_t)B * (R / 8) * (R / 8);
  c->aPa = dalloc<uint16_t>(c, cells * 256);
  c->aDa = dalloc<uint16_t>(c, cells * 256);
  c->logits = dalloc<float>(c, cells * 72);
  c->desc = dalloc<float>(c, cells * 256);
  c->desc_idx = dalloc<int>(c, (size_t)B * 1024 * 4 + 256);
  c->heat = dalloc<float>(c, (size_t)B * R * R);
  c->heat_nms = dalloc<float>(c, (size_t)B * R * R);
  c->nms_mask = dalloc<unsigned char>(c, (size_t)2 * B * R * R);
  const bool multipass_nms = c->cfg.nms_radius > 0 && c->cfg.nms_radius != 4;
  c->nms_tmp = dalloc<float>(c, multipass_nms ? (size_t)4 * B * R * R : 1);
  c->cand = dalloc<unsigned long long>(c, (size_t)B * R * R, false);
  c->cand_cnt = dalloc<int>(c, B);
  c->xtab = dalloc<int>(c, (size_t)R * 4);
  c->ytab = dalloc<int>(c, (size_t)R * 4);
  std::vector<float> lut(256);
  for (int i = 0; i < 256; ++i) lut[i] = (float)((double)i / 255.0);
  c->lut = dupload(c, lut);
  if (!c->img32 || !c->a1b || !c->a2a || !c->a2b || !c->a3a || !c->a3b || !c->a4a || !c->a4b || !c->aPa ||
      !c->aDa || !c->logits || !c->desc || !c->heat || !c->heat_nms || !c->nms_tmp || !c->xtab || !c->ytab || !c->lut ||
      !c->cand || !c->cand_cnt)
    return fail(c, "device allocation failed (detector arena)");
  c->has_sp = true;
  if (p.count("line.conv1.weight")) {
    const Tensor *hw = need(p, "line.head.weight", err), *hb = need(p, "line.head.bias", err);
    if (!hw || !hb || hw->data.size() != 145 * 128 || hb->data.size() != 145) return fail(c, err.empty() ? "line.head: unexpected shape" : err);
    std::function<int(int)> dec_row = [](int f) { return 128 + f; };
    if (!make_conv(c, p, "line.conv1", 128, 128, c->cL1, err) || !make_linear(c, hw->data.data(), hb->data.data(), 128, 145, c->cLh) ||
        !make_linear(c, hw->data.data(), hb->data.data(), 128, 128, c->cLh_loi) ||
        !make_linear(c, hw->data.data(), hb->data.data(), 128, 17, c->cLh_dec, 1.f, &dec_row))
      return fail(c, err.empty() ? "device allocation failed while packing the line branch" : err);
    const size_t npx = (size_t)c->Lmax * 128 * 128;
    c->l_feat = dalloc<uint16_t>(c, npx * 128);
    c->l_head = dalloc<float>(c, (size_t)128 * 128 * 160);
    c->l_dec = dalloc<float>(c, npx * 32);
    c->l_ridx = dalloc<int>(c, (size_t)c->Lmax * 1200 + 256);
    c->l_lrows = dalloc<float>(c, ((size_t)c->Lmax * 1200 + 256) * 128);
    c->l_jloc = dalloc<float>(c, npx);
    c->l_joff = dalloc<float>(c, 2 * npx);
    c->l_ta8 = dalloc<float>(c, 8 * npx);
    c->l_sel = dalloc<float>(c, (size_t)c->Lmax * 320 * AIRFE_FEAT_DIM);
    c->l_nsel = dalloc<int>(c, c->Lmax);
    c->l_cand = dalloc<unsigned long long>(c, (size_t)c->Lmax * 128 * 128, false);
    c->l_cand_cnt = dalloc<int>(c, c->Lmax);
    if (!c->l_feat || !c->l_ta8 || !c->l_head || !c->l_dec || !c->l_ridx || !c->l_lrows || !c->l_jloc || !c->l_joff || !c->l_sel || !c->l_nsel || !c->l_cand || !c->l_cand_cnt)
      return fail(c, "device allocation failed (line branch arena)");
    c->has_s0 = true;
  }
  if (c->prec == 2 && load_superpoint_f32(c, p)) return 1;
  return 0;
}

int alloc_matcher_arena(airfe_ctx* c);

int load_lightglue(airfe_ctx* c, const char* path) {
  c->pack_prec = c->mprec == 2 ? 1 : c->mprec;
  Pack p;
  std::string err;
  if (!load_pack(path, p, err)) return fail(c, err);
  int L = 0;
  while (p.count("transformers." + std::to_string(L) + ".self_attn.Wqkv.weight")) ++L;
  if (L == 0) return fail(c, "LightGlue pack has no transformer layers");
  const Tensor* wr = need(p, "posenc.Wr.weight", err);
  if (!wr || wr->data.size() != 64) return fail(c, "posenc.Wr.weight missing or wrong shape");
  c->lg_wr = dupload(c, wr->data);
  c->lg.resize(L);
  bool ok = true;
  for (int i = 0; i < L && ok; ++i) {
    LgLayer& l = c->lg[i];
    const std::string s = "transformers." + std::to_string(i) + ".self_attn", x = "transformers." + std::to_string(i) + ".cross_attn";
    const Tensor *wqkv, *bqkv;
// ... 183 lines not shown
```

### airslam_amd/csrc/kernels.h

```cpp
#pragma once
#include <hip/hip_runtime.h>
#include <stdint.h>

namespace airfe {

enum Epi {
  EPI_STORE = 0,
  EPI_STORE_F32 = 1,
  EPI_RESID = 2,
  EPI_HEADS = 3,
  EPI_HEADS_T = 4,
  EPI_SOFTMAX_D2S = 5
};
enum Act { ACT_NONE = 0, ACT_RELU = 1 };

struct GemmArgs {
  const uint16_t* X1 = nullptr;
  const uint16_t* X2 = nullptr;
  int ld1 = 0, ld2 = 0, K1 = 0;
  const uint16_t* Wp = nullptr;
  const float* bias = nullptr;
  int M = 0;
  int N = 0;
  int cb_total = 0;
  int epi = EPI_STORE;
  int act = ACT_NONE;
  void* out = nullptr;
  void* out2 = nullptr;
  int ldo = 0;
  float* x32 = nullptr;
  const float* rot_cos = nullptr;
  const float* rot_sin = nullptr;
  int Np = 0, H = 4;
  int small_max = 4096, g8_min = 16000;
  int gr_min = 8192;
  int gr_wgs = 256;
  const int* rowidx = nullptr;
  int d2s_hc = 0, d2s_wc = 0;
  int* flag = nullptr;
};

void launch_gemm(int prec, int K, bool trans, const GemmArgs& a, hipStream_t st);
void launch_gemm8(int prec, int K, bool trans, const GemmArgs& a, hipStream_t st);
bool gemmr_applicable(int K, bool trans, const GemmArgs& a);
void launch_gemmr(int prec, bool trans, const GemmArgs& a, hipStream_t st);
bool gemmr_gather_applicable(int K, const GemmArgs& a);
void launch_gemmr_gather(int prec, const GemmArgs& a, hipStream_t st);
bool gemmr_gather128_applicable(const GemmArgs& a);
void launch_gemmr_gather128(int prec, const GemmArgs& a, hipStream_t st);
bool gemmr_pair_applicable(const GemmArgs& a, const GemmArgs& b);
void launch_gemmr_pair(int prec, const GemmArgs& a, const GemmArgs& b, hipStream_t st);

struct LgBlockFArgs {
  const uint16_t* attn;
  uint16_t* xb;
  float* x32;
  const uint16_t *wo, *w1, *w2;
  const float *bo, *b1, *gamma, *beta, *b2;
  int M;
  int tokens_per_wg = 128;
  int mixed = 0, n_cu = 0;
  int relu = 0;
  const uint16_t *nqk_w = nullptr, *nv_w = nullptr;
  const float *nqk_b = nullptr, *nv_b = nullptr, *rot_cos = nullptr, *rot_sin = nullptr;
  int nqk_n = 0, Np = 0, H = 4;
  uint16_t *q_out = nullptr, *k_out = nullptr, *vt_out = nullptr;
};
void launch_lg_blockf(int prec, const LgBlockFArgs& a, hipStream_t st);
bool lg_blockf_frag_weights();

struct ConvArgs {
  const uint16_t* X = nullptr;
  const uint16_t* Wp = nullptr;
  const float* bias = nullptr;
  uint16_t* Y = nullptr;
  int B = 0, H = 0, W = 0, CIN = 0, COUT = 0;
  int pool = 0;
  int out_pad = 1;
  int relu = 1;
  int wgs = 256;
  const float* img = nullptr;
  const float* w1a = nullptr;
  const float* b1a = nullptr;
};
void launch_conv3x3(int prec, const ConvArgs& a, hipStream_t st);
void launch_conv64r(int prec, const ConvArgs& a, hipStream_t st);
void launch_conv128r(int prec, const ConvArgs& a, hipStream_t st);
constexpr int CONV_ORDER_64R = 1, CONV_ORDER_128R = 2, CONV_ORDER_DEFAULT = CONV_ORDER_64R | CONV_ORDER_128R;
int conv_tile_order_switch();
int conv_tile_order_switch(int v);

void launch_preprocess(const uint8_t* src, int B, int h, int w, int stride, size_t img_stride,
                       const int* xtab , const int* ytab , const float* lut ,
                       float* out, int RH, int RW, hipStream_t st, const uint8_t* src1 = nullptr, int n0 = 0);

void launch_remap_linear(const uint8_t* src, int B, int h, int w, int stride, size_t img_stride, const float* mapx, const float* mapy,
                         uint8_t* dst, int dstride, size_t dimg_stride, hipStream_t st);

void launch_softmax_d2s(const float* logits, int ldl, float* heat, int B, int HC, int WC, hipStream_t st);
void launch_l2norm256(float* d, int rows, hipStream_t st);
void launch_simple_nms(const float* heat, float* out, float* tmp, int B, int H, int W, int radius, hipStream_t st);
void launch_nms512_candidates(const float* heat, float* out, void* planes, int B, float thr, int border, unsigned long long* cand,
                              int* cand_cnt, int cand_cap, hipStream_t st);
void launch_candidates(const float* heat, int B, int H, int W, float thr, int border, unsigned long long* cand,
                       int* cand_cnt, int cand_cap, hipStream_t st);
void launch_candidates_nms3(const float* heat, int B, int H, int W, float thr, unsigned long long* cand, int* cand_cnt, int cand_cap, hipStream_t st);
struct SelectExtra {
  float* feat1 = nullptr; int* n_out1 = nullptr; int Bs = 0;
  int* desc_idx = nullptr; int HC = 0, WC = 0;
  int sort_all = 0;
};
void launch_select_list(const unsigned long long* cand, const int* cand_cnt, int cand_cap, int B, int W, int topk, int cap,
                        float* feat, int* n_out, hipStream_t st, const SelectExtra* ex = nullptr);
void launch_sample_desc(const float* desc, int B, int HC, int WC, float* feat, const int* n, int cap,
                        float w_scale, float h_scale, int normalise, hipStream_t st, int compact = 0, int* flag = nullptr,
                        float* feat1 = nullptr, const int* n1 = nullptr, int Bs = 0);
struct DescSample {
  float* feat = nullptr; float* feat1 = nullptr;
  const int* n = nullptr; const int* n1 = nullptr;
  int Bs = 0, B = 0, cap = 0, HC = 0, WC = 0;
  float w_scale = 1.f, h_scale = 1.f;
  int* flag = nullptr;
  float sx = 0.f, bx = 0.f, sy = 0.f, by = 0.f;
  int junc = 0;
};
bool gemmr_gather_sample_applicable(const GemmArgs& a);
void launch_gemmr_gather_sample(int prec, const GemmArgs& a, const DescSample& ds, hipStream_t st);
bool gemmr_gather_sample_junc_applicable(const GemmArgs& a, const DescSample& ds);
void launch_gemmr_gather_sample_junc(int prec, const GemmArgs& a, const DescSample& ds, hipStream_t st);

struct LgPrepArgs {
  const float* f0; const float* f1;
  const int* n0; const int* n1;
  int ld, kp_off;
  int normalize;
  float cx, cy, linv;
  const float* wr;
  int B, cap, Np;
  float* x32; uint16_t* xb;
  float* rot_cos; float* rot_sin;
  int* lens;
  const float *f0x = nullptr, *f1x = nullptr; const int *n0x = nullptr, *n1x = nullptr;
  int slack_rows = 0;
};
void launch_lg_prepare(int prec, const LgPrepArgs& a, hipStream_t st);
void launch_attention32(int prec, const uint16_t* Q, const uint16_t* K, const uint16_t* Vt, uint16_t* O, const int* lens,
                        int S, int H, int Np, int cross, hipStream_t st);
void launch_ln_gelu(int prec, uint16_t* h, const float* gamma, const float* beta, int M, hipStream_t st);
void launch_rowdot256(const float* x32, const float* w, float b, float* z, int M, hipStream_t st);
void launch_sim(int prec, const uint16_t* md, float* sim, int B, int Np, hipStream_t st);
void launch_lg_assign(const float* sim, const float* z, const int* lens, int B, int Np, int cap, float thr,
                      float* rowlse, float* collse, float* scores_out, int* rowarg, float* rowval, int* colarg,
                      int32_t* idx, float* score, int* nmatch, hipStream_t st);

void launch_trace_hash(const void* p, unsigned unit_words, unsigned units, unsigned long long* out, hipStream_t st);
void launch_trace_digest(const unsigned long long* tab, const unsigned* off, int slots, unsigned long long* dig, hipStream_t st);
size_t lg_assign_part_floats(int B, int Np);
void launch_lg_assign_fused(int prec, const uint16_t* md, const float* z, const int* lens, int B, int Np, int cap, float thr, float* part, float* argpart,
                            float* rowlse, float* collse, float* sim_out, float* scores_out, int* rowarg, float* rowval, int* colarg, int32_t* idx,
                            float* score, int* nmatch, hipStream_t st);
void launch_lg_filter_scores(const float* scores, const int* lens, int B, int Np, int cap, float thr, int* rowarg, float* rowval,
                             int* colarg, int32_t* idx, float* score, int* nmatch, hipStream_t st);

constexpr int LINE_CNT_LD = 64;
constexpr int WF_WGS = 48;
void launch_wireframe(const float* iskeep, const float* imin, const float* imax, int n, int jn, int* table, int* keep,
                      int* pairs, int* rep, int cap, int line_cap, int* counts, bool counted, const float* juncs, const float* lines_pred, float* head4,
                      float* prop4, int B, size_t stage_stride, hipStream_t st);
constexpr int S1_WPAD = 128;
void launch_s1_junc_rows(const float* juncs, int jn, int* ridx, int B, size_t stage_stride, hipStream_t st);
void launch_s1_junc_proj(const float* juncs, const float* head, size_t head_img, int ps, const float* lrows, int jn, const float* w0t,
                         float* proj, int B, size_t stage_stride, hipStream_t st);
void launch_plnet_s1(const float* juncs, const float* lines_pred, const int* keep, const int* pairs, const int* rep,
                     const int* counts, const float* loi, size_t loi_img, const float* proj, const float* ta8, const float* thin,
                     const float* aux, const float* const* w, float* lines_adjusted, float* scores_line, int keep_cap, int line_cap, int B,
                     size_t stage_stride, hipStream_t st, int wgs = 0);
void launch_plnet_s1h(const int* pairs, const int* counts, const float* proj, const float* ta8, const uint16_t* const* wsplit, const float* const* w,
                      const float* lines_adjusted, const float* prop4, float* scores_line, int line_cap, int B, hipStream_t st, int wgs = 0);
void launch_s1h_junc_proj(const float* juncs, const float* lrows, int jn, const uint16_t* wa, const uint16_t* wb, float* proj, int B, size_t stage_stride,
                          hipStream_t st);
void launch_line_filter(const float* la, const float* sc, const int* counts, int border, float line_thr, float len_thr,
                        float w_scale, float h_scale, int R, unsigned char* jmap, int nj, double* lines_out, int capL, int* nlines, int* nfound,
                        int line_cap, int B, hipStream_t st);
void launch_zero16(void* p, size_t bytes, hipStream_t st);
void launch_junction_scan(const unsigned char* jmap, const float* heat, int R, int border, float* feat, int cap, int* n_kept, int* n_found,
                          int* wg_counts, int B, hipStream_t st, const unsigned long long* mask = nullptr);
void launch_line_filter_junc(const float* la, const float* sc, const int* counts, int border, float line_thr, float len_thr, float w_scale, float h_scale,
                             double* lines_out, int capL, int* nlines, int* nfound, int line_cap, int B, int nj, const float* heat, const unsigned long long* mask,
                             float* feat, int capJ, int* n_kept, int* n_jfound, hipStream_t st);

struct GemmF32Args {
  const float* X1 = nullptr; int ld1 = 0, K1 = 0;
  const float* X2 = nullptr; int ld2 = 0;
  const float* W = nullptr;
  const float* bias = nullptr;
  float* Y = nullptr; int ldy = 0;
  int M = 0, N = 0, K = 0;
  float scale = 1.f;
  int relu = 0, accumulate = 0;
};
void launch_conv1a_f32(const float* img, const float* w, const float* bias, float* out, int B, int H, int W, hipStream_t st);
void launch_conv3x3_f32(const float* X, const float* Wt, const float* bias, float* Y, int B, int H, int W, int CIN, int COUT, int opad,
                        hipStream_t st);
void launch_maxpool2_f32(const float* X, float* Y, int B, int H, int W, int C, hipStream_t st);
void launch_gemm_f32(const GemmF32Args& a, hipStream_t st);
void launch_rotary_f32(float* qk, int ld, const float* rc, const float* rs, int M, hipStream_t st);
void launch_attention_f32(const float* Q, int ldq, const float* K, int ldk, const float* V, int ldv, float* O, const int* lens, int S, int H,
                          int Np, int cross, float scale, hipStream_t st);
void launch_ln_gelu_f32(float* h, const float* gamma, const float* beta, int M, hipStream_t st);

void launch_s0_decode(const float* head, int ld, int off, float* lines_pred, float* jloc, float* jnms, float* joff, float* thin, float* aux,
                      float* loi, float* ta8, int B, size_t stage_stride, hipStream_t st);
void launch_s0_head_decode(int prec, const uint16_t* X, const uint16_t* Wp, const float* bias, float* lines_pred, float* jloc, float* jnms,
                           float* joff, float* ta8, int B, size_t stage_stride, hipStream_t st, int wgs = 0);
void launch_s0_juncs(const float* sel, const int* n_sel, const float* joff, float* juncs, int jn, int sel_cap, int B, size_t stage_stride,
                     hipStream_t st);
bool launch_s0_j2l(const float* lines_pred, const float* juncs, int jn, int n, float thr, float* iskeep, float* imin, float* imax, int* counts,
                   int B, size_t stage_stride, int exact_all, hipStream_t st);

void launch_sg_prepare(int prec, const float* f0, const float* f1, const int* n0, const int* n1, int ld, int normalize,
                       float cx, float cy, float linv, const float* const* w, int B, int cap, int Np, float* x32,
                       uint16_t* xb, int* lens, uint16_t* h128, hipStream_t st);
void launch_sg_sinkhorn(const float* sim, const int* lens, int B, int Np, int Lz, float alpha, int iters, float* u, float* v,
                        float* Z, unsigned* counters , unsigned* fail_flag , float* xch,
                        hipStream_t st, int form = 0 , int* form_ran = nullptr);
void launch_sg_decode(const float* Z, const int* lens, int B, int Np, int Lz, float thr, int* idx0, float* max0, int* idx1,
                      int32_t* out0, int32_t* out1, float* ms0, float* ms1, hipStream_t st);

void launch_bow_transform(const float* feat, int ld, int off, int N, const float* node_desc, const int* first_child,
                          const int* n_children, const int* word_id, const float* weight, unsigned* out_word, float* out_weight, int* out_node ,
                          hipStream_t st);

struct PlAssignArgs {
  const double* lines = nullptr;
  const int* nlines = nullptr;
  const float* feat = nullptr;
  const int* npts = nullptr;
  int capL = 0, cap = 0, capE = 0;
  int* counts = nullptr;
  int* row_ptr = nullptr;
  int* pt_idx = nullptr;
  double* pt_dist = nullptr;
  int* total = nullptr;
};
void launch_assign_points_to_lines(const PlAssignArgs& a, int B, hipStream_t st);
struct MlArgs {
  const int *row_ptr0 = nullptr, *pt_idx0 = nullptr, *nlines0 = nullptr, *npts0 = nullptr;
  const int *row_ptr1 = nullptr, *pt_idx1 = nullptr, *nlines1 = nullptr, *npts1 = nullptr;
  const int* matches = nullptr;
  const int* nmatch = nullptr;
  int capL = 0, capE = 0, mcap = 0, W = 0, cap = 0;
  int filter_on = 0;
  double min_x_diff = 0, max_x_diff = 0, max_y_diff = 0;
// ... 270 lines not shown
```

### airslam_amd/csrc/kernels_conv128r.hip

```cpp
#include "common.h"
#include "conv_tile_order.h"
#include "kernels.h"

namespace airfe {

typedef __attribute__((address_space(3))) void* las_ptr128r;

__device__ __forceinline__ void c128r_glds16(const void* gsrc, unsigned lds_off) {
  unsigned keep;
  asm volatile("s_mov_b32 %0, m0\n\ts_mov_b32 m0, %2\n\ts_nop 0\n\tglobal_load_lds_dwordx4 %1, off\n\ts_mov_b32 m0, %0"
               : "=&s"(keep)
               : "v"(gsrc), "s"(lds_off)
               : "memory");
}

constexpr int C128R_TILE_BYTES = 10 * 18 * 256;
constexpr int C128R_PIECES = 10 * 18 * 16;
constexpr int C128R_OUT_OFF = 2 * C128R_TILE_BYTES;
constexpr int C128R_LDS = C128R_OUT_OFF + 128 * 256;

template <class P, bool POOL, bool SHIFT>
__global__ __launch_bounds__(512, 1) void conv128r_kernel(ConvArgs a, ConvTileOrder o) {
  extern __shared__ __attribute__((aligned(16))) char smem[];
  const int tid = threadIdx.x, lane = tid & 63, l15 = lane & 15, g = lane >> 4;
  const int wave = __builtin_amdgcn_readfirstlane(tid >> 6);
  int tile, tstep, pass;
  conv_tile_first(o, blockIdx.x, gridDim.x, tile, tstep, pass);
  const int ntiles = o.ntiles, cb0 = 2 * pass;
  const int cb = cb0 + (wave >> 2), t = wave & 3;
  const int H = a.H, W = a.W, COUT = a.COUT;
  const size_t in_row = (size_t)(W + 2) * 256;
  const size_t in_img = (size_t)(H + 2) * in_row;
  const unsigned lds_base = __builtin_amdgcn_readfirstlane((unsigned)(size_t)(las_ptr128r)smem);

  typename P::vec8 wreg[9][2][2];
  {
    const char* wp = reinterpret_cast<const char*>(a.Wp) + (size_t)cb * 18 * SLAB_BYTES;
    const int rr = t * 16 + l15;
#pragma unroll
    for (int tap = 0; tap < 9; ++tap)
#pragma unroll
      for (int cc = 0; cc < 2; ++cc)
#pragma unroll
        for (int ks = 0; ks < 2; ++ks) {
          const uint4 u = *reinterpret_cast<const uint4*>(wp + (tap * 2 + cc) * SLAB_BYTES + rr * 128 + (((ks * 4 + g) ^ swz128(rr)) << 4));
          wreg[tap][cc][ks] = __builtin_bit_cast(typename P::vec8, u);
        }
  }
  const int f0 = (t >> 1) * 32 + g * 8 + (t & 1) * 4;
  const f32x4 bias = *reinterpret_cast<const f32x4*>(a.bias + cb * 64 + f0);

  int goff[6];
#pragma unroll
  for (int j = 0; j < 6; ++j) {
    const int q = min(j * 512 + tid, C128R_PIECES - 1);
    const int p = q >> 4;
    const int pr = p / 18, pc = p - pr * 18;
    const int c = (q & 15) ^ (pc & 15);
    goff[j] = pr * (int)in_row + pc * 256 + c * 16;
  }
  const bool last_piece = 5 * 512 + tid < C128R_PIECES;
  auto stage_tile = [&](int tile, int buf) {
    int b, ty, tx;
    if constexpr (SHIFT) conv_tile_decode_shift(o, tile, b, ty, tx); else conv_tile_decode_div(o, tile, b, ty, tx);
    const char* xin = reinterpret_cast<const char*>(a.X) + (size_t)b * in_img + (size_t)ty * 8 * in_row + (size_t)tx * 16 * 256;
    const unsigned dst = lds_base + buf * C128R_TILE_BYTES + wave * 1024;
#pragma unroll
    for (int j = 0; j < 5; ++j) c128r_glds16(xin + goff[j], dst + j * 8192);
    if (last_piece) c128r_glds16(xin + goff[5], dst + 5 * 8192);
  };
  int cbase[3];
#pragma unroll
  for (int dx = 0; dx < 3; ++dx) cbase[dx] = (l15 + dx) * 256 + ((g ^ ((l15 + dx) & 15)) << 4);

  const int Ho = POOL ? H / 2 : H, Wo = POOL ? W / 2 : W;
  const int opad = a.out_pad;
  const size_t orow = (size_t)(Wo + 2 * opad) * COUT;
  char* ost = smem + C128R_OUT_OFF;

  if (tile < ntiles) stage_tile(tile, 0);
  asm volatile("s_waitcnt vmcnt(0)" ::: "memory");
  __syncthreads();

  for (int i = 0; tile < ntiles; ++i, tile += tstep) {
    const int next = tile + tstep;
    if (next < ntiles) stage_tile(next, (i + 1) & 1);
    const int xoff = (i & 1) * C128R_TILE_BYTES;
    f32x4 acc[8];
#pragma unroll
    for (int m = 0; m < 8; ++m) acc[m] = bias;
#pragma unroll
    for (int c = 0; c < 12; ++c) {
      const int dx = c >> 2, cc = (c >> 1) & 1, ks = c & 1;
      typename P::vec8 bf[10];
      const char* fb = smem + ((cbase[dx] ^ (ks << 6) ^ (cc << 7)) + xoff);
#pragma unroll
      for (int r = 0; r < 10; ++r) bf[r] = lds_frag<P>(fb, r * (18 * 256));
#pragma unroll
      for (int dy = 0; dy < 3; ++dy)
#pragma unroll
        for (int m = 0; m < 8; ++m) acc[m] = P::mfma(wreg[dy * 3 + dx][cc][ks], bf[m + dy], acc[m]);
    }
    asm volatile("s_waitcnt vmcnt(0)" ::: "memory");
    __syncthreads();

    int b, ty, tx;
    if constexpr (SHIFT) conv_tile_decode_shift(o, tile, b, ty, tx); else conv_tile_decode_div(o, tile, b, ty, tx);
    uint16_t* ybase = a.Y + (size_t)b * (Ho + 2 * opad) * orow + cb0 * 64;
    const int fch = (wave >> 2) * 8 + (f0 >> 3);
    uint2 pk[8];
#pragma unroll
    for (int m = 0; m < 8; ++m) pk[m] = uint2{P::pack2(acc[m][0], acc[m][1]), P::pack2(acc[m][2], acc[m][3])};
    if constexpr (!POOL) {
#pragma unroll
      for (int m = 0; m < 8; ++m) {
        const int px = m * 16 + l15;
        uint2 v = pk[m];
        if (a.relu) { v.x = relu_packed(v.x); v.y = relu_packed(v.y); }
        *reinterpret_cast<uint2*>(ost + px * 256 + ((fch ^ (px & 15)) << 4) + (t & 1) * 8) = v;
      }
      __syncthreads();
#pragma unroll
      for (int j = 0; j < 4; ++j) {
        const int q = j * 512 + tid, px = q >> 4, c = q & 15;
        const uint4 v = *reinterpret_cast<const uint4*>(ost + px * 256 + ((c ^ (px & 15)) << 4));
        const int y = ty * 8 + (px >> 4), x = tx * 16 + (px & 15);
        *reinterpret_cast<uint4*>(ybase + (size_t)(y + opad) * orow + (size_t)(x + opad) * COUT + c * 8) = v;
      }
    } else {
#pragma unroll
      for (int mp = 0; mp < 4; ++mp) {
        uint2 v;
        v.x = max_packed_pre_relu(pk[2 * mp].x, pk[2 * mp + 1].x);
        v.y = max_packed_pre_relu(pk[2 * mp].y, pk[2 * mp + 1].y);
        v.x = max_packed_pre_relu(v.x, dpp_xor1(v.x));
        v.y = max_packed_pre_relu(v.y, dpp_xor1(v.y));
        if (a.relu) { v.x = relu_packed(v.x); v.y = relu_packed(v.y); }
        const int px = mp * 8 + (l15 >> 1);
        if (!(l15 & 1)) *reinterpret_cast<uint2*>(ost + px * 256 + ((fch ^ (px & 15)) << 4) + (t & 1) * 8) = v;
      }
      __syncthreads();
      {
        const int q = tid, px = q >> 4, c = q & 15;
        const uint4 v = *reinterpret_cast<const uint4*>(ost + px * 256 + ((c ^ (px & 15)) << 4));
        const int y = ty * 4 + (px >> 3), x = tx * 8 + (px & 7);
        *reinterpret_cast<uint4*>(ybase + (size_t)(y + opad) * orow + (size_t)(x + opad) * COUT + c * 8) = v;
      }
    }
  }
}

template <class P, bool POOL, bool SHIFT>
static void conv128r_launch_k(const ConvArgs& a, ConvTileOrder o, int grid, int launches, hipStream_t st) {
  static PerDeviceOnce attr_once;
  auto kfn = conv128r_kernel<P, POOL, SHIFT>;
  if (auto once_token = attr_once.first()) {
    (void)hipFuncSetAttribute(reinterpret_cast<const void*>(kfn), hipFuncAttributeMaxDynamicSharedMemorySize, C128R_LDS);
  }
  for (; o.pass0 < launches; ++o.pass0) hipLaunchKernelGGL(kfn, dim3(grid), dim3(512), C128R_LDS, st, a, o);
}

template <class P, bool POOL>
static void conv128r_launch_t(const ConvArgs& a, hipStream_t st) {
  const int tiles_x = a.W / 16, tiles_y = a.H / 8;
  const int ntiles = tiles_x * tiles_y * a.B;
  const int grid = ntiles < a.wgs ? ntiles : a.wgs;
  const int passes = a.COUT / 128;
  const ConvTileOrder o = conv_tile_order(conv_tile_order_switch() & CONV_ORDER_128R, grid, tiles_x, tiles_y, a.B, passes, 16, 8);
  const int launches = conv_tile_launches(o, passes);
  if (o.sh_img >= 0) conv128r_launch_k<P, POOL, true>(a, o, grid, launches, st);
  else conv128r_launch_k<P, POOL, false>(a, o, grid, launches, st);
}

void launch_conv128r(int prec, const ConvArgs& a, hipStream_t st) {
  if (prec == 1) {
    if (a.pool) conv128r_launch_t<PF16, true>(a, st); else conv128r_launch_t<PF16, false>(a, st);
  } else {
    if (a.pool) conv128r_launch_t<PBF16, true>(a, st); else conv128r_launch_t<PBF16, false>(a, st);
  }
}

}
```

### airslam_amd/csrc/kernels_ext.hip

```cpp
#include <float.h>
#include <algorithm>
#include <stdlib.h>

#include "common.h"
#include "kernels.h"

namespace airfe {

__device__ __forceinline__ unsigned block_excl_scan_1024(unsigned v, unsigned* wsum , unsigned* total) {
  const int tid = threadIdx.x, lane = tid & 63, wv = tid >> 6;
  unsigned incl = v;
#pragma unroll
  for (int o = 1; o < 64; o <<= 1) {
    const unsigned t = __shfl_up(incl, o);
    if (lane >= o) incl += t;
  }
  __syncthreads();
  if (lane == 63) wsum[wv] = incl;
  __syncthreads();
  unsigned off = 0, tot = 0;
  for (int w = 0; w < 16; ++w) {
    const unsigned t = wsum[w];
    if (w < wv) off += t;
    tot += t;
// ... 230 lines not shown
#pragma unroll
    for (int r = 0; r < 16; ++r) acc[r] = bias[f0 + 8 * (r >> 2) + 4 * kk + (r & 3)];
  }
  float wb[NB][U];
#pragma unroll
  for (int b = 0; b < NB; ++b)
#pragma unroll
    for (int u = 0; u < U; ++u) wb[b][u] = W.ld(lb, (unsigned)(b * 2 * U + 2 * u) * 512u);
#pragma unroll 1
  for (int t0 = 0; t0 < TRIPS; t0 += NB) {
#pragma unroll
    for (int b = 0; b < NB; ++b) {
      const int k0 = (t0 + b) * 2 * U;
      if (k0 < K) {
        float xb[U];
#pragma unroll
        for (int u = 0; u < U; ++u) xb[u] = xp[(k0 + 2 * u) * S1_LP];
#pragma unroll
        for (int u = 0; u < U; ++u) acc = mfma_32x32x2(wb[b][u], xb[u], acc);
        __builtin_amdgcn_sched_barrier(0);
        const unsigned nrow = (unsigned)__builtin_amdgcn_readfirstlane((k0 + NB * 2 * U) * 512);
#pragma unroll
        for (int u = 0; u < U; ++u) wb[b][u] = W.ld(lb, nrow + (unsigned)u * 1024u);
        __builtin_amdgcn_sched_barrier(0);
      }
    }
  }
}

#ifdef S1_TIMING
__device__ unsigned long long s1_dbg[16];
#define S1_T(i) if (tid == 0) { const long long now_ = wall_clock64(); tacc[i] += now_ - tp_; tp_ = now_; }
#else
#define S1_T(i)
#endif

struct S1Weights {
  const float *w0t, *b0, *w2t, *b2, *w4t, *b4, *wrt, *br, *wh, *bh, *tt;
};
struct S1Loi {
  const float* base;
  size_t img;
  int cs, ps;
  const float* jfeat;
  int jn;
  const float* ta8;
};

constexpr int S1_PJ = 8;
__global__ __launch_bounds__(256) void s1_junc_proj_kernel(const float* __restrict__ juncs, const float* __restrict__ head, size_t head_img,
                                                           int ps, const float* __restrict__ lrows, int jn,
                                                           const float* __restrict__ w0t ,
                                                           float* __restrict__ proj , size_t stage_stride) {
  __shared__ float fs[S1_PJ][128];
  const int t = threadIdx.x, n = t & 127, h = t >> 7, j0 = blockIdx.x * S1_PJ;
  const size_t img = blockIdx.y;
  const float* jp = juncs + img * stage_stride;
  for (int q = h; q < S1_PJ; q += 2) {
    const int j = min(j0 + q, jn - 1);
    if (lrows) {
      const BilTap bt = bil_setup(128, 128, jp[j * 2], jp[j * 2 + 1]);
      const float* r = lrows + ((img * jn + j) * 4) * 128 + n;
      fs[q][n] = bil_eval(r[0], r[128], r[256], r[384], bt);
    } else {
      fs[q][n] = bil_plane(head + img * head_img + n, 128, 128, ps, jp[j * 2], jp[j * 2 + 1]);
    }
  }
  __syncthreads();
  float acc[S1_PJ];
#pragma unroll
  for (int q = 0; q < S1_PJ; ++q) acc[q] = 0.f;
  const float* wp = w0t + (size_t)h * 128 * 128 + n;
#pragma unroll 8
  for (int k = 0; k < 128; ++k) {
    const float wv = wp[k * 128];
#pragma unroll
    for (int q = 0; q < S1_PJ; ++q) acc[q] = fmaf(wv, fs[q][k], acc[q]);
  }
#pragma unroll
  for (int q = 0; q < S1_PJ; ++q)
    if (j0 + q < jn) proj[((img * jn + j0 + q) * 2 + h) * 128 + n] = acc[q];
}

__global__ void s1_junc_rows_kernel(const float* __restrict__ juncs, int jn, int* __restrict__ ridx, size_t stage_stride) {
  const int j = blockIdx.x * blockDim.x + threadIdx.x;
  if (j >= jn) return;
  const size_t img = blockIdx.y;
  const float* jp = juncs + img * stage_stride + j * 2;
  const BilTap bt = bil_setup(128, 128, jp[0], jp[1]);
  int* o = ridx + (img * jn + j) * 4;
  const int base = (int)img * 128 * 128;
  o[0] = base + bt.i00; o[1] = base + bt.i10; o[2] = base + bt.i01; o[3] = base + bt.i11;
}
void launch_s1_junc_rows(const float* juncs, int jn, int* ridx, int B, size_t stage_stride, hipStream_t st) {
  hipLaunchKernelGGL(s1_junc_rows_kernel, dim3((jn + 63) / 64, B), dim3(64), 0, st, juncs, jn, ridx, stage_stride);
}
void launch_s1_junc_proj(const float* juncs, const float* head, size_t head_img, int ps, const float* lrows, int jn, const float* w0t,
                         float* proj, int B, size_t stage_stride, hipStream_t st) {
  hipLaunchKernelGGL(s1_junc_proj_kernel, dim3((jn + S1_PJ - 1) / S1_PJ, B), dim3(256), 0, st, juncs, head, head_img, ps, lrows, jn, w0t, proj,
                     stage_stride);
}

template <bool PRE>
__global__ __launch_bounds__(256, PRE ? 4 : 2) void plnet_s1_kernel(const float* __restrict__ juncs, const float* __restrict__ lines_pred,
                                                       const int* __restrict__ keep, const int* __restrict__ pairs,
                                                       const int* __restrict__ rep, const int* __restrict__ counts, S1Loi loi,
                                                       const float* __restrict__ thin, const float* __restrict__ aux, S1Weights w,
                                                       float* __restrict__ lines_adjusted, float* __restrict__ scores_line,
                                                       int keep_cap, int line_cap, size_t stage_stride) {
  constexpr int XR = PRE ? 256 : 496, XT = PRE ? 0 : 256;
  __shared__ float xs[XR * S1_LP];
  __shared__ __attribute__((aligned(16))) float la[S1_LT][4], li[S1_LT][4];
  __shared__ int lj[S1_LT][2];
  __shared__ float zh[S1_LT][2];
  __shared__ float tts[32];
  __shared__ float bs[4][128];
  __shared__ float whs[2][128];
  float* h0 = xs;
  float* h1 = xs + 128 * S1_LP;
  {
    const size_t img = blockIdx.y;
    juncs += img * stage_stride; lines_pred += img * stage_stride; thin += img * stage_stride; aux += img * stage_stride;
    keep += img * keep_cap; pairs += img * line_cap * 2; rep += img * line_cap; counts += img * LINE_CNT_LD;
    lines_adjusted += img * line_cap * 4; scores_line += img * line_cap;
    loi.base += img * loi.img;
    if constexpr (PRE) { loi.jfeat += img * loi.jn * 256; loi.ta8 += img * 128 * 128 * 8; }
  }
  const int m2 = counts[1];
  const int tid = threadIdx.x, n = tid & 127, g0 = (tid >> 7) * (S1_LT / 2);
  const int lane = tid & 63, f0 = (tid >> 6) * 32, col = lane & 31, rb = 4 * (lane >> 5);
  if (tid < 30) tts[tid] = w.tt[tid];
  if (tid < 128) { bs[0][tid] = w.b0[tid]; bs[1][tid] = w.br[tid]; bs[2][tid] = w.b2[tid]; bs[3][tid] = w.b4[tid]; whs[0][tid] = w.wh[tid]; whs[1][tid] = w.wh[128 + tid]; }
#ifdef S1_TIMING
  long long tacc[10] = {0}, tp_ = wall_clock64();
#endif
  const int hl = tid >> 2, hc = tid & 3;
  int h_j = 0, h_k = 0;
  float h_v = 0.f, h_li = 0.f;
  auto header_l1 = [&](int l0n) {
    if (tid < S1_LT * 4 && l0n < m2) {
      const int u = min(l0n + hl, m2 - 1);
      h_j = pairs[u * 2 + (hc >> 1)];
      h_k = rep[u];
    }
  };
  auto header_l2 = [&](int l0n) {
    if (tid < S1_LT * 4 && l0n < m2) {
      h_v = juncs[h_j * 2 + (hc & 1)];
      h_k = keep[h_k];
    }
  };
  auto header_l3 = [&](int l0n) {
    if (tid < S1_LT * 4 && l0n < m2) h_li = lines_pred[(size_t)h_k * 4 + hc];
  };
  auto header_put = [&](int l0n) {
    if (tid < S1_LT * 4 && l0n < m2) {
      la[hl][hc] = h_v;
      li[hl][hc] = h_li;
      if ((hc & 1) == 0) lj[hl][hc >> 1] = h_j;
      if (l0n + hl < m2) lines_adjusted[(size_t)(l0n + hl) * 4 + hc] = h_v;
    }
  };
  const int l_first = blockIdx.x * S1_LT, l_step = gridDim.x * S1_LT;
  header_l1(l_first); header_l2(l_first); header_l3(l_first);
  for (int l0 = l_first; l0 < m2; l0 += l_step) {
    __syncthreads();
    S1_T(0)
    header_put(l0);
    __syncthreads();
    header_l1(l0 + l_step);
    S1_T(1)
    if constexpr (PRE) {
      constexpr int ITEMS = (S1_LT / 2) * 60;
      constexpr int ROUNDS = (ITEMS + S1_SB * 128 - 1) / (S1_SB * 128);
#pragma unroll 1
      for (int rnd = 0; rnd < ROUNDS; ++rnd) {
        BilTap bt[S1_SB];
        float4 a00[S1_SB], a10[S1_SB], a01[S1_SB], a11[S1_SB];
// ... 1343 lines not shown
```

### airslam_amd/csrc/kernels_mm.hip

```cpp
#include <cstdlib>

#include "common.h"
#include "kernels.h"

namespace airfe {

template <int CIN>
__device__ __forceinline__ int swz_pix(int p) {
  if constexpr (CIN == 64) return swz128(p);
  else return swz256(p);
}

template <class P, int CIN, int MR, bool POOL>
__global__ __launch_bounds__(256) void conv3x3_kernel(ConvArgs a, int tiles_x, int tiles_y, int cb_per_block) {
  constexpr int TH = 4 * MR, TW = 16, PH = TH + 2, PW = TW + 2;
  constexpr int PIXB = CIN * 2, CPP = CIN / 8, NS = 9 * (CIN / 64);
  constexpr int TILE_BYTES = PH * PW * PIXB;
  extern __shared__ __attribute__((aligned(16))) char smem[];
  char* xs = smem;
  char* ws = smem + TILE_BYTES;

  const int tid = threadIdx.x, lane = tid & 63, wave = tid >> 6, l15 = lane & 15, g = lane >> 4;
  const int bid = blockIdx.x;
  const int tx = bid % tiles_x, ty = (bid / tiles_x) % tiles_y, b = bid / (tiles_x * tiles_y);
// ... 61 lines not shown
    }
    if (s == NS - 1) {
      const int cb = cb0 + it / NS;
      const size_t orow = (size_t)(Wo + 2 * opad) * COUT;
      uint16_t* ybase = a.Y + (size_t)b * (Ho + 2 * opad) * orow;
#pragma unroll
      for (int tp = 0; tp < 2; ++tp) {
        const int co0 = cb * 64 + tp * 32 + g * 8;
        float bias[8];
#pragma unroll
        for (int e = 0; e < 8; ++e) bias[e] = a.bias[co0 + e];
        if constexpr (!POOL) {
#pragma unroll
          for (int m = 0; m < MR; ++m) {
            float v[8];
#pragma unroll
            for (int e = 0; e < 4; ++e) {
              v[e] = acc[m][2 * tp][e] + bias[e];
              v[4 + e] = acc[m][2 * tp + 1][e] + bias[4 + e];
            }
            if (a.relu) {
#pragma unroll
              for (int e = 0; e < 8; ++e) v[e] = fmaxf(v[e], 0.f);
            }
            const int y = ty * TH + wave * MR + m, x = tx * TW + l15;
            *reinterpret_cast<uint4*>(ybase + (size_t)(y + opad) * orow + (size_t)(x + opad) * COUT + co0) = pack8<P>(v);
          }
        } else {
#pragma unroll
          for (int mp = 0; mp < MR / 2; ++mp) {
            float v[8];
#pragma unroll
            for (int e = 0; e < 4; ++e) {
              v[e] = fmaxf(acc[2 * mp][2 * tp][e], acc[2 * mp + 1][2 * tp][e]);
              v[4 + e] = fmaxf(acc[2 * mp][2 * tp + 1][e], acc[2 * mp + 1][2 * tp + 1][e]);
            }
#pragma unroll
            for (int e = 0; e < 8; ++e) {
              v[e] = fmaxf(v[e], __shfl_xor(v[e], 1));
              v[e] += bias[e];
              if (a.relu) v[e] = fmaxf(v[e], 0.f);
            }
            if ((l15 & 1) == 0) {
              const int y = (ty * TH + wave * MR) / 2 + mp, x = (tx * TW + l15) / 2;
              *reinterpret_cast<uint4*>(ybase + (size_t)(y + opad) * orow + (size_t)(x + opad) * COUT + co0) = pack8<P>(v);
            }
          }
        }
      }
    }
    __syncthreads();
  }
}

template <class P, int CIN, int MR, bool POOL>
static void conv_launch_t(const ConvArgs& a, hipStream_t st) {
  constexpr int TH = 4 * MR;
  constexpr int LDS = (TH + 2) * 18 * CIN * 2 + 2 * SLAB_BYTES;
  static PerDeviceOnce attr_once;
  auto kfn = conv3x3_kernel<P, CIN, MR, POOL>;
  if (auto once_token = attr_once.first()) {
    (void)hipFuncSetAttribute(reinterpret_cast<const void*>(kfn), hipFuncAttributeMaxDynamicSharedMemorySize, LDS);
  }
  const int tiles_x = a.W / 16, tiles_y = a.H / TH;
  const int cbt = a.COUT / 64;
  const long blocks = (long)tiles_x * tiles_y * a.B;
  const int gy = (blocks >= 2048) ? 1 : cbt;
  dim3 grid((unsigned)blocks, (unsigned)gy);
  hipLaunchKernelGGL(kfn, grid, dim3(256), LDS, st, a, tiles_x, tiles_y, cbt / gy);
}

template <class P>
static void conv_launch_p(const ConvArgs& a, hipStream_t st) {
  if (a.CIN == 64) {
    if (a.pool) conv_launch_t<P, 64, 4, true>(a, st); else conv_launch_t<P, 64, 4, false>(a, st);
  } else {
    if (a.pool) conv_launch_t<P, 128, 2, true>(a, st); else conv_launch_t<P, 128, 2, false>(a, st);
  }
}

static std::atomic<int> g_conv_order{CONV_ORDER_DEFAULT};
int conv_tile_order_switch() { return g_conv_order.load(std::memory_order_relaxed); }
int conv_tile_order_switch(int v) { return g_conv_order.exchange(v < 0 ? CONV_ORDER_DEFAULT : (v & CONV_ORDER_DEFAULT), std::memory_order_relaxed); }

void launch_conv3x3(int prec, const ConvArgs& a, hipStream_t st) {
  if (a.CIN == 64 && (a.COUT % 64) == 0 && a.relu && (a.H % 16) == 0 && (a.W % 16) == 0) {
    launch_conv64r(prec, a, st);
    return;
  }
  if (a.CIN == 128 && (a.COUT % 128) == 0 && a.relu && (a.H % 8) == 0 && (a.W % 16) == 0) {
    launch_conv128r(prec, a, st);
    return;
  }
  if (prec == 1) conv_launch_p<PF16>(a, st); else conv_launch_p<PBF16>(a, st);
}

template <class P>
__device__ __forceinline__ void gemm_store_run(const GemmArgs& a, int row, int co0, float* v) {
#pragma unroll
  for (int e = 0; e < 8; ++e) v[e] += a.bias[co0 + e];
  if (a.act == ACT_RELU) {
#pragma unroll
    for (int e = 0; e < 8; ++e) v[e] = fmaxf(v[e], 0.f);
  }
  switch (a.epi) {
    case EPI_STORE: {
      if (co0 < a.ldo)
        *reinterpret_cast<uint4*>(reinterpret_cast<uint16_t*>(a.out) + (size_t)row * a.ldo + co0) = pack8<P>(v);
      break;
    }
    case EPI_STORE_F32: {
      if (co0 < a.ldo) {
        float* o = reinterpret_cast<float*>(a.out) + (size_t)row * a.ldo + co0;
        *reinterpret_cast<float4*>(o) = make_float4(v[0], v[1], v[2], v[3]);
        *reinterpret_cast<float4*>(o + 4) = make_float4(v[4], v[5], v[6], v[7]);
      }
      break;
    }
    case EPI_RESID: {
      float* xr = a.x32 + (size_t)row * a.ldo + co0;
      float4 r0 = *reinterpret_cast<float4*>(xr), r1 = *reinterpret_cast<float4*>(xr + 4);
      v[0] += r0.x; v[1] += r0.y; v[2] += r0.z; v[3] += r0.w;
      v[4] += r1.x; v[5] += r1.y; v[6] += r1.z; v[7] += r1.w;
      *reinterpret_cast<float4*>(xr) = make_float4(v[0], v[1], v[2], v[3]);
      *reinterpret_cast<float4*>(xr + 4) = make_float4(v[4], v[5], v[6], v[7]);
      *reinterpret_cast<uint4*>(reinterpret_cast<uint16_t*>(a.out) + (size_t)row * a.ldo + co0) = pack8<P>(v);
      break;
    }
    case EPI_HEADS: {
      const int s = row / a.Np, n = row - s * a.Np;
      const int sel = co0 >> 8, cw = co0 & 255, h = cw >> 6, d = cw & 63;
      if (a.rot_cos) {
        const f32x4 c = *reinterpret_cast<const f32x4*>(a.rot_cos + (size_t)row * 32 + (d >> 1));
        const f32x4 sn = *reinterpret_cast<const f32x4*>(a.rot_sin + (size_t)row * 32 + (d >> 1));
        rotate_pairs(v, c, sn);
      }
      uint16_t* o = reinterpret_cast<uint16_t*>(sel ? a.out2 : a.out) + (((size_t)s * a.H + h) * a.Np + n) * 64 + d;
      *reinterpret_cast<uint4*>(o) = pack8<P>(v);
      break;
    }
    default: break;
  }
}

template <class P, bool TRANS>
__global__ __launch_bounds__(256, 2) void gemm_kernel(GemmArgs a, int K, int pairs_per_block) {
  constexpr int STAGE = 32768;
  extern __shared__ __attribute__((aligned(16))) char smem[];
  const int tid = threadIdx.x, lane = tid & 63, wave = tid >> 6, l15 = lane & 15, g = lane >> 4;
  const int wm = wave >> 1, wn = wave & 1;
  const int m0 = blockIdx.x * 128;
  const int NS = K >> 6;
  const int pair0 = blockIdx.y * pairs_per_block;
  const int total = pairs_per_block * NS;

  const int xr = tid >> 3, xc = tid & 7;
  const int xdst0 = xr * 128 + ((xc ^ swz128(xr)) << 4);
  const uint16_t* xp1 = a.X1 + (size_t)(m0 + xr) * a.ld1 + xc * 8;
  const uint16_t* xp2 = a.X2 ? a.X2 + (size_t)(m0 + xr) * a.ld2 + xc * 8 : xp1;
  uint4 px0, px1, px2, px3, pw0, pw1, pw2, pw3;
  const int K1 = a.K1, ld1 = a.ld1, ld2 = a.ld2;
  const uint4* wbase = reinterpret_cast<const uint4*>(a.Wp) + tid;
#define AIRFE_LOAD_CHUNK(IT)                                                                                  \
  {                                                                                                           \
    const int pr_ = pair0 + (IT) / NS, s_ = (IT) % NS, k0_ = s_ * 64;                                         \
    const bool first_ = k0_ < K1;                 \
// ... 200 lines not shown
```

### airslam_amd/csrc/kernels_nms512.hip

```cpp
#include "common.h"
#include "kernels.h"

namespace airfe {

typedef unsigned long long u64;

namespace {

constexpr int NR = 512, NBAND = NR / 8;

__device__ __forceinline__ u64 nms_key(float s, int idx) {
  return (1ull << 49) | ((u64)(__float_as_uint(s) & 0x7FFFFFFFu) << 18) | (u64)(0x3FFFF - idx);
}
__device__ __forceinline__ float vmax3f(float a, float b, float c) {
  float r;
  asm("v_max3_f32 %0, %1, %2, %3" : "=v"(r) : "v"(a), "v"(b), "v"(c));
  return r;
}
__device__ __forceinline__ void max9of16(const float* x, float* o) {
  float t[14];
#pragma unroll
  for (int i = 0; i < 14; ++i) t[i] = vmax3f(x[i], x[i + 1], x[i + 2]);
#pragma unroll
  for (int i = 0; i < 8; ++i) o[i] = vmax3f(t[i], t[i + 3], t[i + 6]);
// ... 50 lines not shown
                                                    int* __restrict__ cand_cnt, int cand_cap) {
  const int n = B * NBAND, per = n >> 3;
  int wid = blockIdx.x;
  if ((n & 7) == 0) wid = (wid & 7) * per + (wid >> 3);
  const int b = wid / NBAND, band = wid - b * NBAND, lane = threadIdx.x;
  const float* S = heat + (size_t)b * NR * NR;
  const int y0 = band * 8;

  unsigned D[4] = {0, 0, 0, 0};
  u64 Mc = 0;
  if (MODE >= 1) {
    const u64* Mp = Min + (size_t)b * NBAND * 64 + lane;
    U192 z;
    z.a = band > 0 ? Mp[(band - 1) * 64] : 0ull;
    z.b = Mp[band * 64];
    z.c = band < NBAND - 1 ? Mp[(band + 1) * 64] : 0ull;
    Mc = z.b;
    const U192 a1 = or3(z, shr_rows(z, 1));
    const U192 a2 = or3(a1, shr_rows(a1, 2));
    const U192 a4 = or3(a2, shr_rows(a2, 4));
    const u64 lo = a4.a | z.b, hi = a4.b | z.c;
    unsigned v[4] = {(unsigned)lo, (unsigned)(lo >> 32), (unsigned)hi, (unsigned)(hi >> 32)};
#pragma unroll
    for (int k = 0; k < 4; ++k) D[k] = hdilate4(v[k], lane_left_u(v[k]), lane_right_u(v[k]));
    if (band == 0) D[0] = 0;
    if (band == NBAND - 1) D[3] = 0;
  }

  float x[16][8];
  const float NI = -INFINITY;
  const float* src = S + (size_t)(y0 - 4) * NR + lane * 8;
  if (band > 0 && band < NBAND - 1) {
#pragma unroll
    for (int i = 0; i < 16; ++i) {
      const float4 q0 = *reinterpret_cast<const float4*>(src + (size_t)i * NR);
      const float4 q1 = *reinterpret_cast<const float4*>(src + (size_t)i * NR + 4);
      x[i][0] = q0.x; x[i][1] = q0.y; x[i][2] = q0.z; x[i][3] = q0.w; x[i][4] = q1.x; x[i][5] = q1.y; x[i][6] = q1.z; x[i][7] = q1.w;
    }
  } else {
#pragma unroll
    for (int i = 0; i < 16; ++i) {
      const int y = y0 - 4 + i;
      float4 q0 = make_float4(NI, NI, NI, NI), q1 = q0;
      if (y >= 0 && y < NR) {
        q0 = *reinterpret_cast<const float4*>(S + (size_t)y * NR + lane * 8);
        q1 = *reinterpret_cast<const float4*>(S + (size_t)y * NR + lane * 8 + 4);
      }
      x[i][0] = q0.x; x[i][1] = q0.y; x[i][2] = q0.z; x[i][3] = q0.w; x[i][4] = q1.x; x[i][5] = q1.y; x[i][6] = q1.z; x[i][7] = q1.w;
    }
  }
  if (MODE >= 1) {
#pragma unroll
    for (int i = 0; i < 16; ++i)
#pragma unroll
      for (int j = 0; j < 8; ++j) {
        const int m = __builtin_amdgcn_sbfe((int)D[i >> 2], 8 * (i & 3) + j, 1);
        x[i][j] = __int_as_float(__float_as_int(x[i][j]) & ~m);
      }
  }

  float V[8][8];
#pragma unroll
  for (int j = 0; j < 8; ++j) {
    float col[16], o[8];
#pragma unroll
    for (int i = 0; i < 16; ++i) col[i] = x[i][j];
    max9of16(col, o);
#pragma unroll
    for (int r = 0; r < 8; ++r) V[r][j] = o[r];
  }
  unsigned eq[2] = {0, 0};
#pragma unroll
  for (int r = 0; r < 8; ++r) {
    float o[8];
    hmax9(V[r], o);
    unsigned byte = 0;
#pragma unroll
    for (int j = 0; j < 8; ++j) byte |= (x[r + 4][j] == o[j]) ? (1u << j) : 0u;
    eq[r >> 2] |= byte << (8 * (r & 3));
  }
  u64 M = ((u64)eq[1] << 32) | eq[0];
  if (MODE >= 1) M = Mc | (M & ~(((u64)D[2] << 32) | D[1]));
  Mout[((size_t)b * NBAND + band) * 64 + lane] = M;
  if (MODE <= 1) return;

  const size_t img = (size_t)b * NR * NR;
  if (out) {
    const float4 zf = make_float4(0.f, 0.f, 0.f, 0.f);
#pragma unroll
    for (int r = 0; r < 8; ++r) {
      float* d = out + img + (size_t)(y0 + r) * NR + lane * 8;
      *reinterpret_cast<float4*>(d) = zf;
      *reinterpret_cast<float4*>(d + 4) = zf;
    }
  }
  u64 kept = M;
  while (__builtin_amdgcn_ballot_w64(kept != 0) != 0) {
    float v[4];
    int gi[4];
    bool pass[4];
#pragma unroll
    for (int t = 0; t < 4; ++t) {
      const bool has = kept != 0;
      const int k = has ? __builtin_ctzll(kept) : 0;
      kept &= kept - 1;
      const int gy = y0 + (k >> 3), gx = lane * 8 + (k & 7);
      gi[t] = gy * NR + gx;
      v[t] = has ? S[gi[t]] : 0.f;
      pass[t] = has && !(gx < border || gx > NR - border || gy < border || gy > NR - border);
      if (out && has) out[img + gi[t]] = v[t];
    }
    u64 pm[4];
    int cnt = 0;
#pragma unroll
    for (int t = 0; t < 4; ++t) {
      pass[t] = pass[t] && !(v[t] < thr);
      pm[t] = __builtin_amdgcn_ballot_w64(pass[t]);
      cnt += __builtin_popcountll(pm[t]);
    }
    if (cnt != 0) {
      int base = 0;
      if (lane == 0) base = atomicAdd(&cand_cnt[b], cnt);
      base = __builtin_amdgcn_readfirstlane(base);
      const u64 lt = (1ull << lane) - 1ull;
#pragma unroll
      for (int t = 0; t < 4; ++t) {
        const int pos = base + __builtin_popcountll(pm[t] & lt);
        if (pass[t] && pos < cand_cap) cand[(size_t)b * cand_cap + pos] = nms_key(v[t], gi[t]);
        base += __builtin_popcountll(pm[t]);
      }
    }
  }
}

void launch_nms512_candidates(const float* heat, float* out, void* planes, int B, float thr, int border, u64* cand, int* cand_cnt,
                              int cand_cap, hipStream_t st) {
  u64* P0 = reinterpret_cast<u64*>(planes);
  u64* P1 = P0 + (size_t)B * NBAND * 64;
  (void)hipMemsetAsync(cand_cnt, 0, (size_t)B * sizeof(int), st);
  const dim3 grid(B * NBAND), block(64);
  hipLaunchKernelGGL(nms512_kernel<0>, grid, block, 0, st, heat, (const u64*)nullptr, P0, (float*)nullptr, B, thr, border, cand, cand_cnt, cand_cap);
  hipLaunchKernelGGL(nms512_kernel<1>, grid, block, 0, st, heat, (const u64*)P0, P1, (float*)nullptr, B, thr, border, cand, cand_cnt, cand_cap);
  hipLaunchKernelGGL(nms512_kernel<2>, grid, block, 0, st, heat, (const u64*)P1, P0, out, B, thr, border, cand, cand_cnt, cand_cap);
}

}
```

### airslam_amd/csrc/kernels_sel.hip

```cpp
#include "common.h"
#include "kernels.h"
#include "desc_sample.h"

namespace airfe {

typedef unsigned long long u64;

__device__ __forceinline__ u64 make_key(float s, int idx) {
  return (1ull << 49) | ((u64)(__float_as_uint(s) & 0x7FFFFFFFu) << 18) | (u64)(0x3FFFF - idx);
}
__device__ __forceinline__ bool in_border_box(int x, int y, int W, int H, int border) {
  return !(x < border || x > W - border || y < border || y > H - border);
}

__global__ __launch_bounds__(256) void candidates_kernel(const float* __restrict__ heat, int H, int W, float thr, int border,
                                                         u64* __restrict__ cand, int* __restrict__ cand_cnt, int cand_cap) {
  __shared__ u64 lkeys[1024];
  __shared__ int lcnt[2];
  const int b = blockIdx.y, N = H * W;
  const float* hm = heat + (size_t)b * N;
  for (int s0 = blockIdx.x * 1024; s0 < N; s0 += gridDim.x * 1024) {
    if (threadIdx.x == 0) lcnt[0] = 0;
    __syncthreads();
    const int i0 = s0 + threadIdx.x * 4;
    if (i0 < N) {
      const float4 v4 = *reinterpret_cast<const float4*>(hm + i0);
      const float v[4] = {v4.x, v4.y, v4.z, v4.w};
#pragma unroll
      for (int k = 0; k < 4; ++k) {
        const int i = i0 + k;
        if (i < N && !(v[k] < thr)) {
          const int y = i / W, x = i - y * W;
          if (in_border_box(x, y, W, H, border)) lkeys[atomicAdd(&lcnt[0], 1)] = make_key(v[k], i);
        }
      }
    }
    __syncthreads();
    const int n = lcnt[0];
    if (threadIdx.x == 0 && n > 0) lcnt[1] = atomicAdd(&cand_cnt[b], n);
    __syncthreads();
    const int base = lcnt[1];
    for (int i = threadIdx.x; i < n; i += 256)
      if (base + i < cand_cap) cand[(size_t)b * cand_cap + base + i] = lkeys[i];
    __syncthreads();
  }
}

__global__ __launch_bounds__(256) void candidates_nms3_kernel(const float* __restrict__ heat, int H, int W, float thr, u64* __restrict__ cand,
                                                              int* __restrict__ cand_cnt, int cand_cap) {
  __shared__ u64 lkeys[1024];
  __shared__ int lcnt[2];
  const int b = blockIdx.y, N = H * W;
  const float* hm = heat + (size_t)b * N;
  for (int s0 = blockIdx.x * 1024; s0 < N; s0 += gridDim.x * 1024) {
    if (threadIdx.x == 0) lcnt[0] = 0;
    __syncthreads();
#pragma unroll
    for (int k = 0; k < 4; ++k) {
      const int i = s0 + k * 256 + threadIdx.x;
      if (i < N) {
        const int y = i / W, x = i - y * W;
        const float a = hm[i];
        float m = a;
#pragma unroll
        for (int dy = -1; dy <= 1; ++dy)
#pragma unroll
          for (int dx = -1; dx <= 1; ++dx) {
            const int xx = x + dx, yy = y + dy;
            if (xx >= 0 && xx < W && yy >= 0 && yy < H) m = fmaxf(m, hm[yy * W + xx]);
          }
        const float v = (a == m) ? a : 0.f;
        if (!(v < thr)) lkeys[atomicAdd(&lcnt[0], 1)] = make_key(v, i);
      }
    }
    __syncthreads();
    const int n = lcnt[0];
    if (threadIdx.x == 0 && n > 0) lcnt[1] = atomicAdd(&cand_cnt[b], n);
    __syncthreads();
    const int base = lcnt[1];
    for (int i = threadIdx.x; i < n; i += 256)
      if (base + i < cand_cap) cand[(size_t)b * cand_cap + base + i] = lkeys[i];
    __syncthreads();
  }
}
void launch_candidates_nms3(const float* heat, int B, int H, int W, float thr, u64* cand, int* cand_cnt, int cand_cap, hipStream_t st) {
  (void)hipMemsetAsync(cand_cnt, 0, (size_t)B * sizeof(int), st);
  hipLaunchKernelGGL(candidates_nms3_kernel, dim3(64, B), dim3(256), 0, st, heat, H, W, thr, cand, cand_cnt, cand_cap);
}

void launch_candidates(const float* heat, int B, int H, int W, float thr, int border, u64* cand, int* cand_cnt, int cand_cap,
                       hipStream_t st) {
  (void)hipMemsetAsync(cand_cnt, 0, (size_t)B * sizeof(int), st);
  hipLaunchKernelGGL(candidates_kernel, dim3(64, B), dim3(256), 0, st, heat, H, W, thr, border, cand, cand_cnt, cand_cap);
}

__global__ __launch_bounds__(1024) void select_list_kernel(const u64* __restrict__ cand, const int* __restrict__ cand_cnt,
                                                           int cand_cap, int W, int topk, int cap, float* __restrict__ feat,
                                                           int* __restrict__ n_out, SelectExtra ex, float sx, float bx, float sy, float by) {
  __shared__ unsigned hist[2048];
  __shared__ u64 sk[1024];
  __shared__ unsigned wsum[16];
  __shared__ u64 s_prefix;
  __shared__ unsigned s_remaining, s_cnt, s_done;
  const int tid = threadIdx.x, b = blockIdx.x;
  const int N = min(cand_cnt[b], cand_cap);
  const u64* keys = cand + (size_t)b * cand_cap;

  u64 prefix = 0;
  unsigned remaining = (unsigned)topk;
  const bool take_all = N <= topk && !ex.sort_all;
  if (N > topk) {
    const int shifts[5] = {38, 27, 16, 5, 0};
    const int nbits[5] = {11, 11, 11, 11, 5};
    for (int pass = 0; pass < 5; ++pass) {
      for (int i = tid; i < 2048; i += 1024) hist[i] = 0;
      __syncthreads();
      const int sh = shifts[pass];
      const u64 himask = ~((1ull << (sh + nbits[pass])) - 1ull);
      const unsigned dmask = (1u << nbits[pass]) - 1u;
      const u64 want = (prefix | (1ull << 49)) & himask;
      for (int i = tid; i < N; i += 1024) {
        const u64 k = keys[i];
        if ((k & himask) == want) atomicAdd(&hist[(unsigned)(k >> sh) & dmask], 1u);
      }
      __syncthreads();
      const unsigned h0 = hist[2047 - 2 * tid], h1 = hist[2046 - 2 * tid];
      const unsigned v = h0 + h1;
      unsigned incl = v;
      const int lane = tid & 63, wv = tid >> 6;
#pragma unroll
      for (int o = 1; o < 64; o <<= 1) {
        const unsigned t = __shfl_up(incl, o);
        if (lane >= o) incl += t;
      }
      if (lane == 63) wsum[wv] = incl;
      __syncthreads();
      unsigned woff = 0;
      for (int w2 = 0; w2 < wv; ++w2) woff += wsum[w2];
      incl += woff;
      const unsigned excl = incl - v;
      if (excl < remaining && remaining <= excl + h0) {
        s_prefix = prefix | ((u64)(2047 - 2 * tid) << sh);
        s_remaining = remaining - excl;
        s_done = (h0 == remaining - excl) ? 1u : 0u;
      } else if (excl + h0 < remaining && remaining <= incl) {
        s_prefix = prefix | ((u64)(2046 - 2 * tid) << sh);
        s_remaining = remaining - excl - h0;
        s_done = (h1 == remaining - excl - h0) ? 1u : 0u;
      }
      __syncthreads();
      prefix = s_prefix;
      remaining = s_remaining;
      const bool done = s_done != 0;
      __syncthreads();
      if (done) break;
    }
  }
  const u64 T = prefix | (1ull << 49);
  if (tid == 0) s_cnt = 0;
  sk[tid] = ~0ull;
  __syncthreads();
  for (int i = tid; i < N; i += 1024) {
    const u64 k = keys[i];
    if (take_all || k >= T) {
      const unsigned slot = atomicAdd(&s_cnt, 1u);
      if (slot < 1024) {
        const u64 idx = 0x3FFFFull - (k & 0x3FFFFull);
        sk[slot] = take_all ? ((idx << 32) | ((k >> 18) & 0x7FFFFFFFull)) : ~k;
      }
    }
  }
  __syncthreads();
  const int n = min((int)s_cnt, min(topk, 1024));
  for (int k2 = 2; k2 <= 1024; k2 <<= 1) {
    for (int j = k2 >> 1; j > 0; j >>= 1) {
      const int p = tid ^ j;
      if (p > tid) {
        const u64 a = sk[tid], c = sk[p];
        const bool up = (tid & k2) == 0;
        if ((a > c) == up) { sk[tid] = c; sk[p] = a; }
      }
      __syncthreads();
    }
  }
  int bl = b;
  if (ex.feat1 && b >= ex.Bs) { feat = ex.feat1; n_out = ex.n_out1; bl = b - ex.Bs; }
  int4 rows = make_int4(0, 0, 0, 0);
  if (tid < n) {
    const u64 e = sk[tid];
    int idx;
    unsigned sb;
    if (take_all) { idx = (int)(e >> 32); sb = (unsigned)(e & 0x7FFFFFFFull); }
    else { const u64 k = ~e; idx = 0x3FFFF - (int)(k & 0x3FFFFull); sb = (unsigned)((k >> 18) & 0x7FFFFFFFull); }
    const int y = idx / W, x = idx - y * W;
    float* f = feat + ((size_t)bl * cap + tid) * 259;
    f[0] = __uint_as_float(sb);
    f[1] = (float)x;
    f[2] = (float)y;
    if (ex.desc_idx) {
      const DescTaps t = desc_taps((float)x, (float)y, sx, bx, sy, by, ex.HC, ex.WC);
      const int base = b * ex.HC * ex.WC;
      rows = make_int4(base + t.c[0], base + t.c[1], base + t.c[2], base + t.c[3]);
    }
  }
  if (ex.desc_idx && tid < cap) reinterpret_cast<int4*>(ex.desc_idx)[(size_t)b * cap + tid] = rows;
  if (tid == 0) n_out[bl] = n;
}

void launch_select_list(const u64* cand, const int* cand_cnt, int cand_cap, int B, int W, int topk, int cap, float* feat,
                        int* n_out, hipStream_t st, const SelectExtra* ex) {
  const SelectExtra e = ex ? *ex : SelectExtra();
  float sx = 0.f, bx = 0.f, sy = 0.f, by = 0.f;
  if (e.desc_idx) desc_grid_coeffs(e.HC, e.WC, sx, bx, sy, by);
  hipLaunchKernelGGL(select_list_kernel, dim3(B), dim3(1024), 0, st, cand, cand_cnt, cand_cap, W, topk, cap, feat, n_out, e, sx, bx, sy, by);
}

}
```

### include/airfe_debug.h

```cpp
#ifndef AIRFE_DEBUG_H_
#define AIRFE_DEBUG_H_
#include "airfe.h"
#ifdef __cplusplus
extern "C" {
#endif

int airfe_debug_detector_maps(airfe_ctx* ctx, int B, float* heat_raw, float* heat_nms, float* desc);
int airfe_debug_lightglue_scores(airfe_ctx* ctx, const float* f0, int n0, const float* f1, int n1, float* scores);
int airfe_debug_lg_filter(airfe_ctx* ctx, const float* scores, int n0, int n1, int32_t* idx, float* score, int cap, int* nmatch);
int airfe_debug_sg_decode(airfe_ctx* ctx, const float* Z, int n0, int n1, int32_t* idx0, int32_t* idx1, double* ms0, double* ms1);
int airfe_debug_sg_sinkhorn(airfe_ctx* ctx, const float* sim, const int* lens , int B, int ld ,
                            float alpha, int iters, int form , float* Z , int* form_ran);
int airfe_debug_superglue_scores(airfe_ctx* ctx, const float* f0, int n0, const float* f1, int n1, float* scores);
int airfe_debug_plnet_stage0(airfe_ctx* ctx, float* juncs_pred, float* lines_pred, float* iskeep, float* idx_min, float* idx_max,
                             float* loi, float* thin, float* aux, float* jloc, float* joff);
int airfe_debug_plnet_j2l(airfe_ctx* ctx, int fast, float* iskeep, float* idx_min, float* idx_max);
int airfe_debug_plnet_s1(airfe_ctx* ctx, const airfe_plnet_stage0* stage0, float* lines_adjusted, float* scores_line,
                         int cap, int* m2);
int airfe_debug_plnet_s1_last(airfe_ctx* ctx, float* lines_adjusted, float* scores_line, int cap, int* m2);
int airfe_debug_preprocess(airfe_ctx* ctx, const uint8_t* gray, int h, int w, int stride, float* out);
int airfe_debug_conv3x3(airfe_ctx* ctx, const float* x, int B, int cin, int H, int W, const float* w, const float* b,
                        int cout, int pool, float* y);
int airfe_debug_gemm(airfe_ctx* ctx, const float* x, int M, int K, const float* w, const float* b, int N, int relu, float* y);
typedef struct airfe_debug_conv_args {
  const float* x;
  const float* img;
  const float *w1a, *b1a;
  const float *w, *b;
  int cin, cout, B, H, W;
  int pool, out_pad, relu, wgs;
  size_t y_words;
  uint16_t* y_raw;
} airfe_debug_conv_args;
int airfe_debug_conv(airfe_ctx* ctx, airfe_debug_conv_args* a);
int airfe_debug_conv_order(int order, int* previous);
enum {
  AIRFE_DEBUG_KERNEL_DISPATCH = 0,
  AIRFE_DEBUG_KERNEL_SMALL = 1,
  AIRFE_DEBUG_KERNEL_TILED = 2,
  AIRFE_DEBUG_KERNEL_GEMM8 = 3,
  AIRFE_DEBUG_KERNEL_GEMMR = 4,
  AIRFE_DEBUG_KERNEL_GEMMR_GATHER = 5,
  AIRFE_DEBUG_KERNEL_GEMMR_GATHER128 = 6
};
typedef struct airfe_debug_linear_args {
  int prec, M, K, K1, N;
  const float* x1;
  const float* x2;
  const float* w;
  const float* b;
  int epi, act;
  const int* rowidx;
  int src_rows;
  const float* rot_cos;
  const float* rot_sin;
  int Np, H;
  float* x32;
  int d2s_hc, d2s_wc;
  int* flag;
  int kernel;
  int gr_wgs;
  float* out;
  float* out2;
} airfe_debug_linear_args;
int airfe_debug_linear(airfe_ctx* ctx, const airfe_debug_linear_args* a);
int airfe_debug_qkv(airfe_ctx* ctx, int prec, int M, int Np, const float* x, const float* wqk, const float* bqk, int nqk, const float* wv, const float* bv,
                    const float* rot_cos, const float* rot_sin, int pair, int gr_wgs, float* q, float* k, float* vt);
typedef struct airfe_debug_lg_block_args {
  int prec, M;
  const float* attn;
  float* x32;
  float* xb;
  const float *wo, *bo;
  const float *w1, *b1;
  const float *gamma, *beta;
  const float *w2, *b2;
  int relu;
  int tokens_per_wg, mixed;
  int nqk_n;
  const float *nqk_w, *nqk_b;
  const float *nv_w, *nv_b;
  const float *rot_cos, *rot_sin;
  int Np;
  float *q, *k, *vt;
  int rows_past[5];
} airfe_debug_lg_block_args;
int airfe_debug_lg_block(airfe_ctx* ctx, airfe_debug_lg_block_args* a);
int airfe_debug_ln_gelu(airfe_ctx* ctx, int prec, float* h, const float* gamma, const float* beta, int M);
int airfe_debug_attention(airfe_ctx* ctx, const float* q, const float* k, const float* v, const int* lens, int S, int H, int n, int cross, float* out);
typedef struct airfe_debug_attn_args {
  int prec;
  int S, H, n, cross;
  const float *q, *k, *v;
  const int* lens;
  int canary, raw;
  float* out;
  int Np, rows_past;
} airfe_debug_attn_args;
int airfe_debug_attention_args(airfe_ctx* ctx, airfe_debug_attn_args* a);
typedef struct airfe_debug_lg_prepare_args {
  int prec;
  int B, cap, ld, kp_off;
  int normalize;
  float cx, cy, linv;
  const float *f0, *f1;
  const int *n0, *n1;
  const float* wr;
  const float *f0x, *f1x;
  int n0x, n1x;
  int slack_rows;
  int rows;
  float *x32, *xb;
  float *rot_cos, *rot_sin;
  int* lens;
  int rows_past;
} airfe_debug_lg_prepare_args;
int airfe_debug_lg_prepare(airfe_ctx* ctx, airfe_debug_lg_prepare_args* a);
typedef struct airfe_debug_lg_assign_args {
// ... 104 lines not shown
```

Before: 8092.

## Fuse SuperPoint convPa/convDa head convs into one launch and drop memsets

```diff
diff --git a/airslam_amd/_lib.py b/airslam_amd/_lib.py
--- a/airslam_amd/_lib.py
+++ b/airslam_amd/_lib.py
@@ -75,6 +75,11 @@
 class DebugConvArgs(C.Structure):
     _fields_ = ([(n, C.c_void_p) for n in ("x", "img", "w1a", "b1a", "w", "b")] + [(n, C.c_int) for n in ("cin", "cout", "B", "H", "W", "pool", "out_pad", "relu", "wgs")]
                 + [("y_words", C.c_size_t), ("y_raw", C.c_void_p)])
+
+
+class DebugConvHeadPairArgs(C.Structure):
+    _fields_ = ([(n, C.c_void_p) for n in ("x", "w0", "b0", "w1", "b1")] + [(n, C.c_int) for n in ("cout", "B", "H", "W", "wgs")]
+                + [("y_words", C.c_size_t), ("y0_raw", C.c_void_p), ("y1_raw", C.c_void_p)])
 
 
 class DebugLgPrepareArgs(C.Structure):
@@ -301,6 +306,8 @@
     "airfe_debug_trace_buffer": (C.c_int, [C.c_void_p, C.c_int, C.c_void_p, C.c_size_t]),
     "airfe_debug_trace_slots": (C.c_int, [C.c_void_p]),
     "airfe_debug_conv_order": (C.c_int, [C.c_int, C.POINTER(C.c_int)]),
+    "airfe_debug_conv_head_pair": (C.c_int, [C.c_void_p, C.POINTER(DebugConvHeadPairArgs)]),
+    "airfe_debug_conv_head_pair_mode": (C.c_int, [C.c_int, C.POINTER(C.c_int)]),
     "airfe_debug_trace_slot": (C.c_int, [C.c_void_p, C.c_int, C.c_char_p, C.c_int, C.POINTER(C.c_uint), C.POINTER(C.c_uint), C.POINTER(C.c_uint)]),
     "airfe_debug_trace_read": (C.c_int, [C.c_void_p, C.c_void_p, C.c_void_p, C.c_void_p]),
     "airfe_debug_gemm": (C.c_int, [C.c_void_p, C.c_void_p, C.c_int, C.c_int, C.c_void_p, C.c_void_p, C.c_int, C.c_int,
diff --git a/airslam_amd/api.py b/airslam_amd/api.py
--- a/airslam_amd/api.py
+++ b/airslam_amd/api.py
@@ -35,6 +35,13 @@
     return prev.value
 
 
+def conv_head_pair(mode: int) -> int:
+    prev = C.c_int()
+    if _lib.lib().airfe_debug_conv_head_pair_mode(int(mode), C.byref(prev)) != 0:
+        raise AirfeError((_lib.lib().airfe_last_error(None) or b"airfe_debug_conv_head_pair_mode failed").decode())
+    return prev.value
+
+
 class Context:
 
     def __init__(self, superpoint=None, lightglue=None, superglue=None, plnet_s1=None, tuning=None, **cfg):
@@ -45,6 +52,9 @@
         if tuning and "conv_order" in tuning:
             tuning = dict(tuning)
             conv_tile_order(int(tuning.pop("conv_order")))
+        if tuning and "conv_head_pair" in tuning:
+            tuning = dict(tuning)
+            conv_head_pair(int(tuning.pop("conv_head_pair")))
         if tuning:
             t = _lib.Tuning()
             self._l.airfe_default_tuning(C.byref(t))
@@ -566,6 +576,18 @@
         inner = np.ascontiguousarray(buf[:, p:p + ho, p:p + wo, :])
         y = inner.view(np.float16).astype(np.float32) if prec == 1 else (inner.astype(np.uint32) << 16).view(np.float32)
         return {"raw": buf, "guard_lo": raw[:guard], "guard_hi": raw[guard + words:], "y": np.ascontiguousarray(y.transpose(0, 3, 1, 2))}
+
+    def debug_conv_head_pair(self, x, w0, b0, w1, b1, wgs=256):
+        x, w0, b0, w1, b1 = (np.ascontiguousarray(t, np.float32) for t in (x, w0, b0, w1, b1))
+        bb, hh, ww = x.shape[0], x.shape[-2], x.shape[-1]
+        cout = w0.shape[0]
+        guard = ww * cout
+        words = bb * hh * guard
+        raws = [np.zeros(words + 2 * guard, np.uint16) for _ in range(2)]
+        a = _lib.DebugConvHeadPairArgs(x=x.ctypes.data, w0=w0.ctypes.data, b0=b0.ctypes.data, w1=w1.ctypes.data, b1=b1.ctypes.data, cout=cout, B=bb, H=hh, W=ww,
+                                       wgs=int(wgs), y_words=raws[0].size, y0_raw=raws[0].ctypes.data, y1_raw=raws[1].ctypes.data)
+        self._chk(self._l.airfe_debug_conv_head_pair(self._h, C.byref(a)), "airfe_debug_conv_head_pair")
+        return tuple({"raw": r[guard:guard + words].reshape(bb, hh, ww, cout), "guard_lo": r[:guard], "guard_hi": r[guard + words:]} for r in raws)
 
     def debug_gemm(self, x, w, b, relu=False):
         x = np.ascontiguousarray(x, np.float32); w = np.ascontiguousarray(w, np.float32); b = np.ascontiguousarray(b, np.float32)
diff --git a/airslam_amd/csrc/airfe_debug.hip b/airslam_amd/csrc/airfe_debug.hip
--- a/airslam_amd/csrc/airfe_debug.hip
+++ b/airslam_amd/csrc/airfe_debug.hip
@@ -216,6 +216,44 @@
 int airfe_debug_conv_order(int order, int* previous) try {
   if (order < -1 || order > CONV_ORDER_DEFAULT) return fail(nullptr, "debug_conv_order: order must lie in -1 .. 3");
   const int before = conv_tile_order_switch(order);
+  if (previous) *previous = before;
+  return 0;
+} AIRFE_CATCH(nullptr)
+
+int airfe_debug_conv_head_pair(airfe_ctx* c, airfe_debug_conv_head_pair_args* a) try {
+  AIRFE_ENTER(c);
+  if (!a || !a->x || !a->w0 || !a->b0 || !a->w1 || !a->b1 || !a->y0_raw || !a->y1_raw) return fail(c, "debug_conv_head_pair: null argument");
+  const int cout = a->cout, B = a->B, H = a->H, W = a->W, prec = c->prec;
+  if (prec != 0 && prec != 1) return fail(c, "debug_conv_head_pair: the context's precision must be fp16 or bf16");
+  if (a->wgs < 1 || a->wgs > 256) return fail(c, "debug_conv_head_pair: wgs must lie in 1 .. 256");
+  if (cout < 128 || cout % 128) return fail(c, "debug_conv_head_pair: cout must be a multiple of 128");
+  if (B < 1 || H < 16 || W < 16 || H % 16 || W % 16) return fail(c, "debug_conv_head_pair: B >= 1, H and W multiples of 16");
+  const size_t guard = (size_t)W * cout, words = (size_t)B * H * guard, total = words + 2 * guard;
+  if (a->y_words != total) return fail(c, "debug_conv_head_pair: y_words must be (B H + 2) W cout");
+  HookStage s(c, "debug_conv_head_pair");
+  std::vector<uint16_t> slabs = dbg_conv_slabs(a->w0, 128, cout, prec);
+  const std::vector<uint16_t> half = dbg_conv_slabs(a->w1, 128, cout, prec);
+  slabs.insert(slabs.end(), half.begin(), half.end());
+  std::vector<float> bias(a->b0, a->b0 + cout);
+  bias.insert(bias.end(), a->b1, a->b1 + cout);
+  ConvW w0, w1;
+  w0.w = s.up(std::move(slabs)); w0.b = s.up(std::move(bias));
+  const uint16_t* x = s.up(dbg_conv_x(a->x, B, 128, H, W, prec));
+  uint16_t* dy0 = s.fresh<uint16_t>(total, 0xFF);
+  uint16_t* dy1 = s.fresh<uint16_t>(total, 0xFF);
+  if (s.status()) return 1;
+  w0.cin = w1.cin = 128; w0.cout = w1.cout = cout;
+  w1.w = w0.w + half.size(); w1.b = w0.b + cout;
+  s.step(run_conv_head_pair(c, w0, w1, x, dy0 + guard, dy1 + guard, B, H, W, a->wgs, s.stream()));
+  s.wait(HookStage::OWN_TEXT);
+  s.get(a->y0_raw, dy0, total * 2);
+  s.get(a->y1_raw, dy1, total * 2);
+  return s.status();
+} AIRFE_CATCH(c)
+
+int airfe_debug_conv_head_pair_mode(int mode, int* previous) try {
+  if (mode < -1 || mode > CONV_HEAD_PAIR_ONE) return fail(nullptr, "debug_conv_head_pair_mode: mode must lie in -1 .. 2");
+  const int before = conv_head_pair_switch(mode);
   if (previous) *previous = before;
   return 0;
 } AIRFE_CATCH(nullptr)
diff --git a/airslam_amd/csrc/airfe_detect.hip b/airslam_amd/csrc/airfe_detect.hip
--- a/airslam_amd/csrc/airfe_detect.hip
+++ b/airslam_amd/csrc/airfe_detect.hip
@@ -15,17 +15,38 @@
 }
 
 int run_conv(airfe_ctx* c, const ConvW& w, const uint16_t* x, uint16_t* y, int B, int H, int W, int pool, int out_pad,
-             hipStream_t st) {
+             hipStream_t st, int wgs) {
   ConvArgs a;
   a.X = x; a.Wp = w.w; a.bias = w.b; a.Y = y;
   a.B = B; a.H = H; a.W = W; a.CIN = w.cin; a.COUT = w.cout;
-  a.pool = pool; a.out_pad = out_pad; a.relu = 1;
+  a.pool = pool; a.out_pad = out_pad; a.relu = 1; a.wgs = wgs;
   const double px = (double)B * H * W;
   const double ob = px / (pool ? 4 : 1) * w.cout * 2;
   {
     ProfScope ps(c, w.cin == 64 ? ST_CONV3X3_C64 : ST_CONV3X3_C128, st, 2.0 * px * w.cin * w.cout * 9,
                  px * w.cin * 2 + ob + 9.0 * w.cin * w.cout * 2);
     launch_conv3x3(c->prec, a, st);
+  }
+  return c->cfg.check_launches ? launch_status(c) : 0;
+}
+
+int run_conv_head_pair(airfe_ctx* c, const ConvW& w0, const ConvW& w1, const uint16_t* x, uint16_t* y0, uint16_t* y1, int B, int H, int W, int wgs,
+                       hipStream_t st) {
+  const int mode = conv_head_pair_switch();
+  const bool swap = mode == CONV_HEAD_PAIR_SECOND_FIRST;
+  if (mode != CONV_HEAD_PAIR_ONE)
+    return run_conv(c, swap ? w1 : w0, x, swap ? y1 : y0, B, H, W, 0, 0, st, wgs) || run_conv(c, swap ? w0 : w1, x, swap ? y0 : y1, B, H, W, 0, 0, st, wgs);
+  if (w0.cin != 128 || w1.cin != 128 || w0.cout != w1.cout || w0.cout % 128 || H % 8 || W % 16 || w1.w != w0.w + (size_t)9 * w0.cin * w0.cout ||
+      w1.b != w0.b + w0.cout)
+    return fail(c, "run_conv_head_pair: the one-launch form takes two 128-input layers of one shape whose weights and biases are one pack");
+  ConvArgs a;
+  a.X = x; a.Wp = w0.w; a.bias = w0.b; a.Y = y0; a.Y2 = y1; a.pass2 = w0.cout / 128;
+  a.B = B; a.H = H; a.W = W; a.CIN = 128; a.COUT = w0.cout;
+  a.pool = 0; a.out_pad = 0; a.relu = 1; a.wgs = wgs;
+  const double px = (double)B * H * W;
+  {
+    ProfScope ps(c, ST_CONV3X3_C128, st, 2.0 * (2.0 * px * 128 * w0.cout * 9), 2.0 * (px * 128 * 2 + px * w0.cout * 2 + 9.0 * 128 * w0.cout * 2));
+    launch_conv128r(c->prec, a, st);
   }
   return c->cfg.check_launches ? launch_status(c) : 0;
 }
@@ -112,12 +133,11 @@
     ProfScope ps(c, ST_SELECT, st, 0, (double)B * 8192 * 8);
     SelectExtra ex;
     if (two) { ex.feat1 = d_feat1; ex.n_out1 = d_n1; ex.Bs = Bs; }
-    if (sparse_desc) { ex.desc_idx = c->desc_idx; ex.HC = R / 8; ex.WC = R / 8; }
+    if (sparse_desc) { ex.desc_idx = c->desc_idx; ex.HC = R / 8; ex.WC = R / 8; ex.desc_pad = Mp - M; }
     launch_select_list(c->cand, c->cand_cnt, ccap, B, R, c->cfg.max_keypoints, cap, d_feat, d_n, st, &ex);
   }
   bool sampled = false;
   if (sparse_desc) {
-    if (Mp > M) HIPCHK(c, hipMemsetAsync(c->desc_idx + M, 0, (size_t)(Mp - M) * 4, st));
     GemmArgs g;
     g.X1 = c->aDa; g.ld1 = 256; g.K1 = 256; g.Wp = c->cDb.w; g.bias = c->cDb.b; g.rowidx = c->desc_idx;
     g.M = Mp; g.N = 256; g.cb_total = c->cDb.cbt; g.epi = EPI_STORE_F32; g.out = c->desc; g.ldo = 256;
@@ -183,8 +203,7 @@
     if (run_conv(c, c->c3b, c->a3a, c->a3b, B, R / 4, R / 4, 1, 1, st)) return 1;
     if (run_conv(c, c->c4a, c->a3b, c->a4a, B, R / 8, R / 8, 0, 1, st)) return 1;
     if (run_conv(c, c->c4b, c->a4a, c->a4b, B, R / 8, R / 8, 0, 1, st)) return 1;
-    if (run_conv(c, c->cPa, c->a4b, c->aPa, B, R / 8, R / 8, 0, 0, st)) return 1;
-    if (run_conv(c, c->cDa, c->a4b, c->aDa, B, R / 8, R / 8, 0, 0, st)) return 1;
+    if (run_conv_head_pair(c, c->cPa, c->cDa, c->a4b, c->aPa, c->aDa, B, R / 8, R / 8, 256, st)) return 1;
     const int cells = B * (R / 8) * (R / 8);
     {
       GemmArgs g;
diff --git a/airslam_amd/csrc/airfe_host.h b/airslam_amd/csrc/airfe_host.h
--- a/airslam_amd/csrc/airfe_host.h
+++ b/airslam_amd/csrc/airfe_host.h
@@ -341,7 +341,9 @@
 bool make_linear(DevAllocs* c, const float* W, const float* bias, int K, int N, LinW& out, float scale = 1.f,
                  const std::function<int(int)>* src_row = nullptr, const std::function<int(int)>* src_col = nullptr);
 int ensure_tables(airfe_ctx* c, int h, int w);
-int run_conv(airfe_ctx* c, const ConvW& w, const uint16_t* x, uint16_t* y, int B, int H, int W, int pool, int out_pad, hipStream_t st);
+int run_conv(airfe_ctx* c, const ConvW& w, const uint16_t* x, uint16_t* y, int B, int H, int W, int pool, int out_pad, hipStream_t st, int wgs = 256);
+int run_conv_head_pair(airfe_ctx* c, const ConvW& w0, const ConvW& w1, const uint16_t* x, uint16_t* y0, uint16_t* y1, int B, int H, int W, int wgs,
+                       hipStream_t st);
 int dense_desc_head(airfe_ctx* c, int B, hipStream_t st);
 int detect_tail_dev(airfe_ctx* c, int B, int Bs, bool two, bool sparse_desc, int h, int w, float* d_feat, float* d_feat1, int cap, int* d_n, int* d_n1,
                     hipStream_t st);
diff --git a/airslam_amd/csrc/airfe_lines.hip b/airslam_amd/csrc/airfe_lines.hip
--- a/airslam_amd/csrc/airfe_lines.hip
+++ b/airslam_amd/csrc/airfe_lines.hip
@@ -6,6 +6,7 @@
   const int F = 128, ccap = F * F;
   launch_candidates_nms3(c->l_jloc, nb, F, F, 1e-30f, c->l_cand, c->l_cand_cnt, ccap, st);
   SelectExtra jx;
+  jx.reset_cnt = 1;
   jx.sort_all = 1;
   launch_select_list(c->l_cand, c->l_cand_cnt, ccap, nb, F, 300, 320, c->l_sel, c->l_nsel, st, &jx);
   launch_s0_juncs(c->l_sel, c->l_nsel, c->l_joff, c->s0_stage + SG_JUNCS, 300, 320, nb, SG_STRIDE, st);
@@ -49,8 +50,7 @@
 
 int line_tap_rows(airfe_ctx* c, int nb, hipStream_t st) {
   const int M = nb * 1200, Mp = (M + 255) / 256 * 256;
-  launch_s1_junc_rows(c->s0_stage + SG_JUNCS, 300, c->l_ridx, nb, SG_STRIDE, st);
-  if (Mp > M) HIPCHK(c, hipMemsetAsync(c->l_ridx + M, 0, (size_t)(Mp - M) * 4, st));
+  launch_s1_junc_rows(c->s0_stage + SG_JUNCS, 300, c->l_ridx, nb, SG_STRIDE, st, Mp - M);
   return 0;
 }
 
diff --git a/airslam_amd/csrc/airfe_load.hip b/airslam_amd/csrc/airfe_load.hip
--- a/airslam_amd/csrc/airfe_load.hip
+++ b/airslam_amd/csrc/airfe_load.hip
@@ -116,22 +116,31 @@
   return true;
 }
 
+static bool make_convs(airfe_ctx* c, const Pack& p, const std::vector<std::string>& names, int cin, int cout, ConvW* const* out, std::string& err) {
+  const int nci = cin / 64;
+  std::vector<uint16_t> slabs;
+  std::vector<float> bias;
+  for (const std::string& name : names) {
+    const Tensor* w = need(p, name + ".weight", err);
+    const Tensor* b = need(p, name + ".bias", err);
+    if (!w || !b) return false;
+    if ((int)w->data.size() != cout * cin * 9 || (int)b->data.size() != cout) { err = name + ": unexpected shape"; return false; }
+    const float* wd = w->data.data();
+    const auto one = pack_slabs(cout / 64, 9 * nci, c->prec, [&](int feat, int s, int k) {
+      const int tap = s / nci, cc = s % nci, ci = cc * 64 + k;
+      return wd[((size_t)feat * cin + ci) * 9 + tap];
+    });
+    slabs.insert(slabs.end(), one.begin(), one.end());
+    bias.insert(bias.end(), b->data.begin(), b->data.end());
+  }
+  uint16_t* dw = dupload(c, slabs);
+  float* db = dupload(c, bias);
+  for (size_t k = 0; k < names.size() && dw && db; ++k) *out[k] = ConvW{dw + k * (slabs.size() / names.size()), db + k * cout, cin, cout};
+  return dw && db;
+}
 bool make_conv(airfe_ctx* c, const Pack& p, const std::string& name, int cin, int cout, ConvW& out, std::string& err) {
-  const Tensor* w = need(p, name + ".weight", err);
-  const Tensor* b = need(p, name + ".bias", err);
-  if (!w || !b) return false;
-  if ((int)w->data.size() != cout * cin * 9 || (int)b->data.size() != cout) { err = name + ": unexpected shape"; return false; }
-  const int nci = cin / 64;
-  const float* wd = w->data.data();
-  auto slabs = pack_slabs(cout / 64, 9 * nci, c->prec, [&](int feat, int s, int k) {
-    const int tap = s / nci, cc = s % nci, ci = cc * 64 + k;
-    return wd[((size_t)feat * cin + ci) * 9 + tap];
-  });
-  out.w = dupload(c, slabs);
-  out.b = dupload(c, b->data);
-  out.cin = cin;
-  out.cout = cout;
-  return out.w && out.b;
+  ConvW* const o[1] = {&out};
+  return make_convs(c, p, {name}, cin, cout, o, err);
 }
 
 bool make_linear(DevAllocs* c, const float* W, const float* bias, int K, int N, LinW& out, float scale,
@@ -369,11 +378,11 @@
   if (!w1 || !b1 || w1->data.size() != 64 * 9) return fail(c, err.empty() ? "conv1a: unexpected shape" : err);
   c->c1a_w = dupload(c, w1->data);
   c->c1a_b = dupload(c, b1->data);
+  ConvW* const head_pair[2] = {&c->cPa, &c->cDa};
   bool ok = make_conv(c, p, "conv1b", 64, 64, c->c1b, err) && make_conv(c, p, "conv2a", 64, 64, c->c2a, err) &&
             make_conv(c, p, "conv2b", 64, 64, c->c2b, err) && make_conv(c, p, "conv3a", 64, 128, c->c3a, err) &&
             make_conv(c, p, "conv3b", 128, 128, c->c3b, err) && make_conv(c, p, "conv4a", 128, 128, c->c4a, err) &&
-            make_conv(c, p, "conv4b", 128, 128, c->c4b, err) && make_conv(c, p, "convPa", 128, 256, c->cPa, err) &&
-            make_conv(c, p, "convDa", 128, 256, c->cDa, err) &&
+            make_conv(c, p, "conv4b", 128, 128, c->c4b, err) && make_convs(c, p, {"convPa", "convDa"}, 128, 256, head_pair, err) &&
             make_linear_named(c, p, "convPb", 256, 65, c->cPb, err) && make_linear_named(c, p, "convDb", 256, 256, c->cDb, err);
   if (!ok) return fail(c, err.empty() ? "device allocation failed while packing SuperPoint weights" : err);
 
diff --git a/airslam_amd/csrc/kernels.h b/airslam_amd/csrc/kernels.h
--- a/airslam_amd/csrc/kernels.h
+++ b/airslam_amd/csrc/kernels.h
@@ -78,6 +78,8 @@
   int pool = 0;
   int out_pad = 1;
   int relu = 1;
+  uint16_t* Y2 = nullptr;
+  int pass2 = 0;
   int wgs = 256;
   const float* img = nullptr;
   const float* w1a = nullptr;
@@ -89,6 +91,9 @@
 constexpr int CONV_ORDER_64R = 1, CONV_ORDER_128R = 2, CONV_ORDER_DEFAULT = CONV_ORDER_64R | CONV_ORDER_128R;
 int conv_tile_order_switch();
 int conv_tile_order_switch(int v);
+constexpr int CONV_HEAD_PAIR_SPLIT = 0, CONV_HEAD_PAIR_SECOND_FIRST = 1, CONV_HEAD_PAIR_ONE = 2, CONV_HEAD_PAIR_DEFAULT = CONV_HEAD_PAIR_ONE;
+int conv_head_pair_switch();
+int conv_head_pair_switch(int v);
 
 void launch_preprocess(const uint8_t* src, int B, int h, int w, int stride, size_t img_stride,
                        const int* xtab , const int* ytab , const float* lut ,
@@ -108,9 +113,11 @@
 struct SelectExtra {
   float* feat1 = nullptr; int* n_out1 = nullptr; int Bs = 0;
   int* desc_idx = nullptr; int HC = 0, WC = 0;
+  int desc_pad = 0;
   int sort_all = 0;
-};
-void launch_select_list(const unsigned long long* cand, const int* cand_cnt, int cand_cap, int B, int W, int topk, int cap,
+  int reset_cnt = 0;
+};
+void launch_select_list(const unsigned long long* cand, int* cand_cnt, int cand_cap, int B, int W, int topk, int cap,
                         float* feat, int* n_out, hipStream_t st, const SelectExtra* ex = nullptr);
 void launch_sample_desc(const float* desc, int B, int HC, int WC, float* feat, const int* n, int cap,
                         float w_scale, float h_scale, int normalise, hipStream_t st, int compact = 0, int* flag = nullptr,
@@ -168,7 +175,7 @@
                       int* pairs, int* rep, int cap, int line_cap, int* counts, bool counted, const float* juncs, const float* lines_pred, float* head4,
                       float* prop4, int B, size_t stage_stride, hipStream_t st);
 constexpr int S1_WPAD = 128;
-void launch_s1_junc_rows(const float* juncs, int jn, int* ridx, int B, size_t stage_stride, hipStream_t st);
+void launch_s1_junc_rows(const float* juncs, int jn, int* ridx, int B, size_t stage_stride, hipStream_t st, int pad = 0);
 void launch_s1_junc_proj(const float* juncs, const float* head, size_t head_img, int ps, const float* lrows, int jn, const float* w0t,
                          float* proj, int B, size_t stage_stride, hipStream_t st);
 void launch_plnet_s1(const float* juncs, const float* lines_pred, const int* keep, const int* pairs, const int* rep,
diff --git a/airslam_amd/csrc/kernels_conv128r.hip b/airslam_amd/csrc/kernels_conv128r.hip
--- a/airslam_amd/csrc/kernels_conv128r.hip
+++ b/airslam_amd/csrc/kernels_conv128r.hip
@@ -29,6 +29,8 @@
   const int ntiles = o.ntiles, cb0 = 2 * pass;
   const int cb = cb0 + (wave >> 2), t = wave & 3;
   const int H = a.H, W = a.W, COUT = a.COUT;
+  const bool second = a.Y2 != nullptr && pass >= a.pass2;
+  uint16_t* const yout = (second ? a.Y2 : a.Y) + (second ? pass - a.pass2 : pass) * 128;
   const size_t in_row = (size_t)(W + 2) * 256;
   const size_t in_img = (size_t)(H + 2) * in_row;
   const unsigned lds_base = __builtin_amdgcn_readfirstlane((unsigned)(size_t)(las_ptr128r)smem);
@@ -106,7 +108,7 @@
 
     int b, ty, tx;
     if constexpr (SHIFT) conv_tile_decode_shift(o, tile, b, ty, tx); else conv_tile_decode_div(o, tile, b, ty, tx);
-    uint16_t* ybase = a.Y + (size_t)b * (Ho + 2 * opad) * orow + cb0 * 64;
+    uint16_t* ybase = yout + (size_t)b * (Ho + 2 * opad) * orow;
     const int fch = (wave >> 2) * 8 + (f0 >> 3);
     uint2 pk[8];
 #pragma unroll
@@ -165,7 +167,7 @@
   const int tiles_x = a.W / 16, tiles_y = a.H / 8;
   const int ntiles = tiles_x * tiles_y * a.B;
   const int grid = ntiles < a.wgs ? ntiles : a.wgs;
-  const int passes = a.COUT / 128;
+  const int passes = a.Y2 ? a.pass2 + a.COUT / 128 : a.COUT / 128;
   const ConvTileOrder o = conv_tile_order(conv_tile_order_switch() & CONV_ORDER_128R, grid, tiles_x, tiles_y, a.B, passes, 16, 8);
   const int launches = conv_tile_launches(o, passes);
   if (o.sh_img >= 0) conv128r_launch_k<P, POOL, true>(a, o, grid, launches, st);
diff --git a/airslam_amd/csrc/kernels_ext.hip b/airslam_amd/csrc/kernels_ext.hip
--- a/airslam_amd/csrc/kernels_ext.hip
+++ b/airslam_amd/csrc/kernels_ext.hip
@@ -336,18 +336,19 @@
     if (j0 + q < jn) proj[((img * jn + j0 + q) * 2 + h) * 128 + n] = acc[q];
 }
 
-__global__ void s1_junc_rows_kernel(const float* __restrict__ juncs, int jn, int* __restrict__ ridx, size_t stage_stride) {
+__global__ void s1_junc_rows_kernel(const float* __restrict__ juncs, int jn, int* __restrict__ ridx, size_t stage_stride, int pad) {
   const int j = blockIdx.x * blockDim.x + threadIdx.x;
+  const size_t img = blockIdx.y;
+  if (blockIdx.y == gridDim.y - 1 && j < pad) ridx[(size_t)gridDim.y * jn * 4 + j] = 0;
   if (j >= jn) return;
-  const size_t img = blockIdx.y;
   const float* jp = juncs + img * stage_stride + j * 2;
   const BilTap bt = bil_setup(128, 128, jp[0], jp[1]);
   int* o = ridx + (img * jn + j) * 4;
   const int base = (int)img * 128 * 128;
   o[0] = base + bt.i00; o[1] = base + bt.i10; o[2] = base + bt.i01; o[3] = base + bt.i11;
 }
-void launch_s1_junc_rows(const float* juncs, int jn, int* ridx, int B, size_t stage_stride, hipStream_t st) {
-  hipLaunchKernelGGL(s1_junc_rows_kernel, dim3((jn + 63) / 64, B), dim3(64), 0, st, juncs, jn, ridx, stage_stride);
+void launch_s1_junc_rows(const float* juncs, int jn, int* ridx, int B, size_t stage_stride, hipStream_t st, int pad) {
+  hipLaunchKernelGGL(s1_junc_rows_kernel, dim3((jn + 63) / 64, B), dim3(64), 0, st, juncs, jn, ridx, stage_stride, pad);
 }
 void launch_s1_junc_proj(const float* juncs, const float* head, size_t head_img, int ps, const float* lrows, int jn, const float* w0t,
                          float* proj, int B, size_t stage_stride, hipStream_t st) {
diff --git a/airslam_amd/csrc/kernels_mm.hip b/airslam_amd/csrc/kernels_mm.hip
--- a/airslam_amd/csrc/kernels_mm.hip
+++ b/airslam_amd/csrc/kernels_mm.hip
@@ -167,6 +167,11 @@
 static std::atomic<int> g_conv_order{CONV_ORDER_DEFAULT};
 int conv_tile_order_switch() { return g_conv_order.load(std::memory_order_relaxed); }
 int conv_tile_order_switch(int v) { return g_conv_order.exchange(v < 0 ? CONV_ORDER_DEFAULT : (v & CONV_ORDER_DEFAULT), std::memory_order_relaxed); }
+static std::atomic<int> g_conv_head_pair{CONV_HEAD_PAIR_DEFAULT};
+int conv_head_pair_switch() { return g_conv_head_pair.load(std::memory_order_relaxed); }
+int conv_head_pair_switch(int v) {
+  return g_conv_head_pair.exchange(v < 0 || v > CONV_HEAD_PAIR_ONE ? CONV_HEAD_PAIR_DEFAULT : v, std::memory_order_relaxed);
+}
 
 void launch_conv3x3(int prec, const ConvArgs& a, hipStream_t st) {
   if (a.CIN == 64 && (a.COUT % 64) == 0 && a.relu && (a.H % 16) == 0 && (a.W % 16) == 0) {
diff --git a/airslam_amd/csrc/kernels_nms512.hip b/airslam_amd/csrc/kernels_nms512.hip
--- a/airslam_amd/csrc/kernels_nms512.hip
+++ b/airslam_amd/csrc/kernels_nms512.hip
@@ -156,6 +156,7 @@
   u64 M = ((u64)eq[1] << 32) | eq[0];
   if (MODE >= 1) M = Mc | (M & ~(((u64)D[2] << 32) | D[1]));
   Mout[((size_t)b * NBAND + band) * 64 + lane] = M;
+  if (MODE == 0 && band == 0 && lane == 0) cand_cnt[b] = 0;
   if (MODE <= 1) return;
 
   const size_t img = (size_t)b * NR * NR;
@@ -211,7 +212,6 @@
                               int cand_cap, hipStream_t st) {
   u64* P0 = reinterpret_cast<u64*>(planes);
   u64* P1 = P0 + (size_t)B * NBAND * 64;
-  (void)hipMemsetAsync(cand_cnt, 0, (size_t)B * sizeof(int), st);
   const dim3 grid(B * NBAND), block(64);
   hipLaunchKernelGGL(nms512_kernel<0>, grid, block, 0, st, heat, (const u64*)nullptr, P0, (float*)nullptr, B, thr, border, cand, cand_cnt, cand_cap);
   hipLaunchKernelGGL(nms512_kernel<1>, grid, block, 0, st, heat, (const u64*)P0, P1, (float*)nullptr, B, thr, border, cand, cand_cnt, cand_cap);
diff --git a/airslam_amd/csrc/kernels_sel.hip b/airslam_amd/csrc/kernels_sel.hip
--- a/airslam_amd/csrc/kernels_sel.hip
+++ b/airslam_amd/csrc/kernels_sel.hip
@@ -84,7 +84,6 @@
   }
 }
 void launch_candidates_nms3(const float* heat, int B, int H, int W, float thr, u64* cand, int* cand_cnt, int cand_cap, hipStream_t st) {
-  (void)hipMemsetAsync(cand_cnt, 0, (size_t)B * sizeof(int), st);
   hipLaunchKernelGGL(candidates_nms3_kernel, dim3(64, B), dim3(256), 0, st, heat, H, W, thr, cand, cand_cnt, cand_cap);
 }
 
@@ -94,7 +93,7 @@
   hipLaunchKernelGGL(candidates_kernel, dim3(64, B), dim3(256), 0, st, heat, H, W, thr, border, cand, cand_cnt, cand_cap);
 }
 
-__global__ __launch_bounds__(1024) void select_list_kernel(const u64* __restrict__ cand, const int* __restrict__ cand_cnt,
+__global__ __launch_bounds__(1024) void select_list_kernel(const u64* __restrict__ cand, int* __restrict__ cand_cnt,
                                                            int cand_cap, int W, int topk, int cap, float* __restrict__ feat,
                                                            int* __restrict__ n_out, SelectExtra ex, float sx, float bx, float sy, float by) {
   __shared__ unsigned hist[2048];
@@ -204,10 +203,12 @@
     }
   }
   if (ex.desc_idx && tid < cap) reinterpret_cast<int4*>(ex.desc_idx)[(size_t)b * cap + tid] = rows;
+  if (ex.desc_idx && b == (int)gridDim.x - 1 && tid < ex.desc_pad) ex.desc_idx[(size_t)gridDim.x * cap * 4 + tid] = 0;
   if (tid == 0) n_out[bl] = n;
-}
-
-void launch_select_list(const u64* cand, const int* cand_cnt, int cand_cap, int B, int W, int topk, int cap, float* feat,
+  if (ex.reset_cnt && tid == 0) cand_cnt[b] = 0;
+}
+
+void launch_select_list(const u64* cand, int* cand_cnt, int cand_cap, int B, int W, int topk, int cap, float* feat,
                         int* n_out, hipStream_t st, const SelectExtra* ex) {
   const SelectExtra e = ex ? *ex : SelectExtra();
   float sx = 0.f, bx = 0.f, sy = 0.f, by = 0.f;
diff --git a/include/airfe_debug.h b/include/airfe_debug.h
--- a/include/airfe_debug.h
+++ b/include/airfe_debug.h
@@ -34,6 +34,16 @@
 } airfe_debug_conv_args;
 int airfe_debug_conv(airfe_ctx* ctx, airfe_debug_conv_args* a);
 int airfe_debug_conv_order(int order, int* previous);
+typedef struct airfe_debug_conv_head_pair_args {
+  const float* x;
+  const float *w0, *b0;
+  const float *w1, *b1;
+  int cout, B, H, W, wgs;
+  size_t y_words;
+  uint16_t *y0_raw, *y1_raw;
+} airfe_debug_conv_head_pair_args;
+int airfe_debug_conv_head_pair(airfe_ctx* ctx, airfe_debug_conv_head_pair_args* a);
+int airfe_debug_conv_head_pair_mode(int mode, int* previous);
 enum {
   AIRFE_DEBUG_KERNEL_DISPATCH = 0,
   AIRFE_DEBUG_KERNEL_SMALL = 1,
```

Result: slower. 7879 (-2.6%).
